# shaunlebron/blinky

Measured on AMD Instinct MI355X. Metric: warped Mpixels/s (lensmap apply), higher is better.
Workload: dtype u8; 1 GPU; 3840x2160 cube/panini f_fov 180, 64 frames/step from a resident ring of 64 distinct globes (1.80 GB, advanced every step), one lensmap; value / ms_per_step = the job with steps alternating between 2 HIP stream(s), value_one_stream = the same on one stream, roofline.kernel_ms_per_launch = the kernel alone under HIP events; 64 frames/step since r5 (r1-r4 ran 16: compare those with value_at_16_frames; ring_globes=64, parallelism=row-stripes x1, streams=2

## Files before the change

### blinky_amd/csrc/bk_api.cpp

```cpp
#include "bk_internal.h"

#include <algorithm>
#include <cstdlib>
#include <cstring>
#include <ctime>
#include <vector>

#include <dlfcn.h>

static thread_local std::string g_create_error;

static bool g_hwq_late = false;
__attribute__((constructor)) static void bk_more_hardware_queues()
{
    const char *keep = getenv("BLINKY_HIP_KEEP_HW_QUEUES");
    if (keep && *keep && *keep != '0') return;
    if (getenv("GPU_MAX_HW_QUEUES")) return;
    if (void *h = dlopen("libamdhip64.so", RTLD_NOW | RTLD_NOLOAD)) { g_hwq_late = true; (void)dlclose(h); }
    (void)setenv("GPU_MAX_HW_QUEUES", "16", 0);
}
void bk::hw_queue_note()
{
    static bool said = false;
    if (said) return;
// ... 238 lines not shown
    if (int r = alloc_maps(ctx)) return fail_empty(r);
    if (int r = alloc_globe(ctx)) return fail_empty(r);
    return BK_OK;
}

extern "C" int bk_set_rows(bk_ctx *ctx, int row0, int row1)
{
    if (!ctx) return BK_E_INVALID;
    if (row0 < 0 || row1 > ctx->H || row0 > row1)
        return ctx->fail(BK_E_INVALID, "bk_set_rows: [%d,%d) outside 0..%d", row0, row1, ctx->H);
    if (ctx->device < 0) {
        ctx->row0 = row0; ctx->row1 = row1;
        return BK_OK;
    }
    if (int r = ensure_device(ctx)) return r;
    if (row0 == ctx->row0 && row1 == ctx->row1) return BK_OK;
    ctx->row0 = row0; ctx->row1 = row1;
    ctx->lensmap_valid = false;
    ctx->spans_valid = false;
    bk::footprint_invalidate(ctx);
    return alloc_maps(ctx);
}

extern "C" int bk_set_frames(bk_ctx *ctx, int nframes)
{
    if (!ctx || nframes < 1) return BK_E_INVALID;
    if (int r = ensure_device(ctx)) return r;
    ctx->nframes = nframes;
    if (!ctx->ps) return BK_OK;
    return alloc_globe(ctx);
}

extern "C" int bk_get_size(const bk_ctx *ctx, int *width, int *height, int *platesize, int *row0, int *row1)
{
    if (!ctx) return BK_E_INVALID;
    if (width) *width = ctx->W;
    if (height) *height = ctx->H;
    if (platesize) *platesize = ctx->ps;
    if (row0) *row0 = ctx->row0;
    if (row1) *row1 = ctx->row1;
    return BK_OK;
}

extern "C" int bk_set_rubixgrid(bk_ctx *ctx, int numcells, double cell_size, double pad_size)
{
    if (!ctx) return BK_E_INVALID;
    ctx->rubix.numcells = numcells; ctx->rubix.cell = cell_size; ctx->rubix.pad = pad_size;
    return BK_OK;
}

extern "C" int bk_set_zoom(bk_ctx *ctx, int zoom_type, int fov_degrees)
{
    if (!ctx || zoom_type < BK_ZOOM_NONE || zoom_type > BK_ZOOM_CONTAIN) return BK_E_INVALID;
    ctx->zoom_type = zoom_type;
    ctx->zoom_fov = (zoom_type == BK_ZOOM_FOV || zoom_type == BK_ZOOM_VFOV) ? fov_degrees : 0;
    return BK_OK;
}

extern "C" int bk_set_apply_variant(bk_ctx *ctx, int variant)
{
    if (!ctx) return BK_E_INVALID;
    ctx->apply_variant = variant;
    return BK_OK;
}

extern "C" int bk_set_blockmap_tuning(bk_ctx *ctx, int measured)
{
    if (!ctx) return BK_E_INVALID;
    ctx->blockmap_tuning = measured != 0;
    bk::coopmap_invalidate(ctx);
    return BK_OK;
}

bk::DebugOptions bk::g_debug;
#if BK_DEBUG_API
extern "C" int bk_debug_set_option(const char *name, int value)
{
    if (!name) return BK_E_INVALID;
    if (!strcmp(name, "no_memcache")) bk::g_debug.no_memcache = value;
    else if (!strcmp(name, "libm_rel_log2")) bk::g_debug.libm_rel_log2 = value;
    else if (!strcmp(name, "print_model")) bk::g_debug.print_model = value;
    else if (!strcmp(name, "host_module")) bk::g_debug.host_module = value;
    else if (!strcmp(name, "no_direct_submit")) bk::g_debug.no_direct_submit = value;
    else if (!strcmp(name, "forward_careful")) bk::g_debug.forward_careful = value;
    else return BK_E_INVALID;
    return BK_OK;
}
#endif
#if BK_DEBUG_API
extern "C" int bk_debug_set_ablation(bk_ctx *ctx, int bits)
{
    if (!ctx) return BK_E_INVALID;
    ctx->apply_flags = bits;
    return BK_OK;
}
#endif

#if BK_DEBUG_API
extern "C" int bk_debug_set_tile_shape(bk_ctx *ctx, int lw)
{
    if (!ctx) return BK_E_INVALID;
    if (lw >= 600) { ctx->apply_block_cost = lw == 600 ? -1 : lw - 601; bk::coopmap_invalidate(ctx); return BK_OK; }
    if (lw >= 400) { ctx->apply_lds_kb = lw - 400; bk::coopmap_invalidate(ctx); return BK_OK; }
    if (lw >= 300) { ctx->apply_fchunk = lw - 300; return BK_OK; }
    if (lw >= 100) { ctx->apply_wgs_per_cu = lw - 100; return BK_OK; }
    if (lw != 0 && lw != 1 && lw != 2 && lw != 4) return BK_E_INVALID;
    ctx->tile_shape = lw;
    bk::coopmap_invalidate(ctx);
    return BK_OK;
}
#endif

#if BK_DEBUG_API
extern "C" int bk_debug_tile_stats(bk_ctx *ctx, int out[6])
{
    if (!ctx || !out) return BK_E_INVALID;
    if (!ctx->lensmap_valid) return ctx->fail(BK_E_STATE, "no lensmap");
    if (int r = ensure_device(ctx)) return r;
    return bk::coopmap_stats(ctx, out);
}
#endif

#if BK_DEBUG_API
extern "C" int bk_debug_traffic_model(bk_ctx *ctx, uint64_t out[8])
{
    if (!ctx || !out) return BK_E_INVALID;
    if (!ctx->lensmap_valid) return ctx->fail(BK_E_STATE, "no lensmap");
    if (int r = ensure_device(ctx)) return r;
    return bk::coopmap_traffic_model(ctx, out);
}
#endif

#if BK_DEBUG_API
extern "C" int bk_debug_band_balance(bk_ctx *ctx, uint32_t out[18])
{
    if (!ctx || !out) return BK_E_INVALID;
    if (!ctx->lensmap_valid) return ctx->fail(BK_E_STATE, "no lensmap");
    if (int r = ensure_device(ctx)) return r;
    return bk::coopmap_band_balance(ctx, out);
}
#endif

#if BK_DEBUG_API
extern "C" int bk_debug_xcd_of_workgroups(bk_ctx *ctx, int *out, int nworkgroups)
{
    if (!ctx || !out || nworkgroups < 1) return BK_E_INVALID;
    if (int r = ensure_device(ctx)) return r;
    return bk::coopmap_xcd_probe(ctx, out, nworkgroups);
}
#endif

extern "C" double bk_last_build_ms(const bk_ctx *ctx) { return ctx ? ctx->last_build_ms : 0; }


extern "C" int bk_set_lensmap(bk_ctx *ctx, const uint32_t *offsets, const uint8_t *tints)
{
    if (!ctx || !offsets) return BK_E_INVALID;
    if (!ctx->d_offsets) return ctx->fail(BK_E_STATE, "bk_set_lensmap: call bk_resize first");
    if (int r = ensure_device(ctx)) return r;
    const size_t px = (size_t)ctx->W * ctx->rows();
    BK_HIP(ctx, hipMemcpyAsync(ctx->d_offsets, offsets, px * 4, hipMemcpyHostToDevice, ctx->stream));
    if (int r = bk::launch_convert_offsets(ctx, ctx->d_offsets, px, 1)) return r;
    if (tints) BK_HIP(ctx, hipMemcpyAsync(ctx->d_tints, tints, px, hipMemcpyHostToDevice, ctx->stream));
    else BK_HIP(ctx, hipMemsetAsync(ctx->d_tints, 255, px, ctx->stream));
    BK_HIP(ctx, hipStreamSynchronize(ctx->stream));
    ctx->lensmap_valid = true;
// ... 618 lines not shown
```

### blinky_amd/csrc/bk_build.cpp

```cpp
#include <algorithm>
#include <chrono>
#include <cstring>
#include <memory>

#include "bk_build_params.h"
#include "bk_emit.h"
#include "bk_hostpool.h"
#include "bk_lens_priv.h"
#include "bkm.h"

using namespace bklua;
using bk::LensProgram;


static void fill_params(bk_ctx *ctx, BkBuildParams *bp)
{
    memset(bp, 0, sizeof *bp);
    bp->W = ctx->W; bp->H = ctx->H;
    bp->row0 = ctx->row0; bp->rows = ctx->rows();
    bp->ps = ctx->ps; bp->gp = ctx->gp; bp->ph = ctx->ph;
    bp->numplates = ctx->numplates;
    bp->has_globe_plate = ctx->prog->globe_plate.is_function();
    bp->scale = ctx->scale;
    bp->inv_scale_up = 1.0 / __builtin_fabs(ctx->scale) * (1.0 + 0x1p-50);
// ... 519 lines not shown
    bk::EmitRequest rq;
    rq.interp = &P->interp; rq.lens_inverse = P->lens_inverse; rq.lens_forward = P->lens_forward; rq.globe_plate = P->globe_plate;
    std::string which;
    bool carries = true;
    try { carries = bk::callbacks_carry_state(rq, &which); } catch (const LuaError &) { carries = true; which = "(callbacks not analysable)"; }
    const bool sequential = ctx->sequential_build >= 2 || (ctx->sequential_build == 1 && carries);
    ctx->last_build_path = sequential ? 2 : 1;
    ctx->last_build_why = why + (sequential ? (carries ? "; state carried in '" + which + "': one sequential scan on the host" : "; one sequential scan on the host (bk_set_sequential_build 2)")
                                            : "; callbacks carry no state: evaluated on the host's worker pool");
    if (P->info.map_type == BK_MAP_INVERSE) {
        if (!P->lens_inverse.is_function()) return ctx->fail(BK_E_STATE, "lens has no lens_inverse (map = \"lens_inverse\" without the function)");
        return sequential ? build_sequential(ctx, P, std::string(), bp, display_out) : build_inverse_pool(ctx, P, bp, display_out);
    }
    if (!P->lens_forward.is_function()) return ctx->fail(BK_E_STATE, "lens has no lens_forward");
    return build_forward_host(ctx, P, bp, sequential, display_out);
}

extern "C" int bk_last_build_path(const bk_ctx *ctx, char *why, size_t cap)
{
    if (!ctx) return BK_E_INVALID;
    if (why && cap) snprintf(why, cap, "%s", ctx->last_build_why.c_str());
    return ctx->last_build_path;
}

#if BK_DEBUG_API
extern "C" int bk_debug_host_build(bk_ctx *ctx, int mode, uint32_t *offsets, uint8_t *tints, int display_out[BK_MAX_PLATES], double *scale_out)
{
    if (!ctx || !offsets || !tints || mode < 0 || mode > 2) return BK_E_INVALID;
    LensProgram *P = ctx->prog;
    if (!P || !P->lens_valid) return ctx->fail(BK_E_STATE, "not a valid lens");
    if (!ctx->globe_valid) return ctx->fail(BK_E_STATE, "not a valid globe");
    if (ctx->W <= 0 || ctx->rows() <= 0) return ctx->fail(BK_E_STATE, "bk_debug_host_build: call bk_resize first");
    const size_t px = (size_t)ctx->W * ctx->rows();
    memset(offsets, 0xFF, px * 4);
    memset(tints, 255, px);
    for (int i = 0; i < BK_MAX_PLATES; ++i) { ctx->display[i] = 0; if (display_out) display_out[i] = 0; }
    ctx->last_bad_key = 0;
    if (int r = bk_calc_zoom(ctx, scale_out)) return r;
    if (P->info.map_type == BK_MAP_NONE) return ctx->fail(BK_E_STATE, "no inverse or forward map being used");
    BkBuildParams bp;
    fill_params(ctx, &bp);
    ctx->host_sink_off = offsets; ctx->host_sink_tint = tints;
    int rc;
    if (mode == 0) rc = build_on_host(ctx, P, "bk_debug_host_build", display_out);
    else if (P->info.map_type == BK_MAP_INVERSE) {
        if (!P->lens_inverse.is_function()) rc = ctx->fail(BK_E_STATE, "lens has no lens_inverse");
        else rc = mode == 2 ? build_sequential(ctx, P, std::string(), bp, display_out) : build_inverse_pool(ctx, P, bp, display_out);
    } else {
        if (!P->lens_forward.is_function()) rc = ctx->fail(BK_E_STATE, "lens has no lens_forward");
        else rc = build_forward_host(ctx, P, bp, mode == 2, display_out);
    }
    ctx->host_sink_off = nullptr; ctx->host_sink_tint = nullptr;
    for (size_t i = 0; i < px; ++i) {
        if (offsets[i] == BK_NULL_OFFSET) continue;
        unsigned plate, x, y;
        bk_texel_coords((unsigned)ctx->gp, (unsigned)ctx->ph, offsets[i], &plate, &x, &y);
        offsets[i] = plate * (unsigned)(ctx->ps * ctx->ps) + y * (unsigned)ctx->ps + x;
    }
    return rc;
}
#endif

extern "C" int bk_set_sequential_build(bk_ctx *ctx, int mode)
{
    if (!ctx || mode < 0 || mode > 2) return BK_E_INVALID;
    ctx->sequential_build = mode;
    return BK_OK;
}

extern "C" int bk_lens_carries_state(bk_ctx *ctx, char *global_name, size_t cap)
{
    if (!ctx) return BK_E_INVALID;
    LensProgram *P = ctx->prog;
    if (!P || !P->lens_valid) return ctx->fail(BK_E_STATE, "not a valid lens");
    bk::EmitRequest rq;
    rq.interp = &P->interp; rq.lens_inverse = P->lens_inverse; rq.lens_forward = P->lens_forward; rq.globe_plate = P->globe_plate;
    std::string which;
    bool carries = false;
    try { carries = bk::callbacks_carry_state(rq, &which); } catch (const LuaError &e) { return ctx->fail(BK_E_SCRIPT, "%s", e.what()); }
    if (global_name && cap) snprintf(global_name, cap, "%s", which.c_str());
    return carries ? 1 : 0;
}

struct HipFree { void operator()(void *p) const { (void)hipFree(p); } };
using DeviceMem = std::unique_ptr<void, HipFree>;

static int build_inverse_device(bk_ctx *ctx, LensProgram *P, const std::string &src, BkBuildParams &bp, int counters[kNumCounters])
{
    if (!P->k_inverse) return ctx->fail(BK_E_STATE, "lens has no lens_inverse (map = \"lens_inverse\" without the function)");
    for (int k = 0; k < 4; ++k) {
        (void)hipFree(ctx->fwd_scratch[k]);
        ctx->fwd_scratch[k] = nullptr; ctx->fwd_scratch_bytes[k] = 0;
    }
    void *args[] = {&bp};
    BK_HIP(ctx, hipEventRecord(ctx->build_time_ev[0], ctx->stream));
    const auto tk0 = std::chrono::steady_clock::now();
    std::vector<uint32_t> flagged;
    if (int r = flagged_pass(ctx, "bk_build_inverse launch", bp, false, [&] {
            return hipModuleLaunchKernel(P->k_inverse, (unsigned)((ctx->W + 255) / 256), (unsigned)ctx->rows(), 1, 256, 1, 1, 0, ctx->stream, args, nullptr);
        }, counters, &flagged, &ctx->last_kernel_retries)) return r;
    ctx->last_kernel_wall_ms = std::chrono::duration<double, std::milli>(std::chrono::steady_clock::now() - tk0).count();
    const size_t nfl = flagged.size() / 4;
    std::vector<uint32_t> roff(nfl);
    std::vector<uint8_t> rtint(nfl);
    std::vector<int> rshown(nfl), rerr(nfl, 0);
    rederive(ctx, P, src, flagged.data(), 4, nfl, true,
             [&](const HostModule &hm, const uint32_t *id, int stride, unsigned long cnt, size_t i) { hm.inverse(&bp, id, stride, cnt, &roff[i], &rtint[i], &rshown[i], &rerr[i]); },
             [&](HostEval &E, uint32_t id, size_t i) { h_inverse_entry(E, bp, id, &roff[i], &rtint[i], &rshown[i], &rerr[i]); });
    unsigned int bad_key = (unsigned)counters[BK_MAX_PLATES + 2];
    for (size_t i = 0; i < nfl; ++i) {
        counters[BK_MAX_PLATES] |= rerr[i];
        if (rerr[i] & BK_ERR_RESULT) {
            const uint32_t o = flagged[4 * i], lyl = o / (uint32_t)ctx->W, lx = o - lyl * (uint32_t)ctx->W;
            bad_key = std::max(bad_key, (uint32_t)(((uint32_t)ctx->row0 + lyl) * (uint32_t)ctx->W + ((uint32_t)ctx->W - 1u - lx)) + 1u);
        }
        if (rshown[i] >= 0) counters[rshown[i]] |= 1;
    }
    counters[BK_MAX_PLATES + 2] = (int)bad_key;
    if (int r = patch_changed(ctx, flagged, {roff.data()}, rtint.data(), ctx->d_offsets, ctx->d_tints)) return r;
    BK_HIP(ctx, hipEventRecord(ctx->build_time_ev[1], ctx->stream));
    return BK_OK;
}

static int build_forward_device(bk_ctx *ctx, LensProgram *P, const std::string &src, BkBuildParams &bp, int counters[kNumCounters])
{
    if (!P->k_corners || !P->k_quads || !P->k_resolve) return ctx->fail(BK_E_STATE, "lens has no lens_forward");
    const size_t px = (size_t)ctx->W * ctx->rows();
    const size_t n1 = (size_t)ctx->ps + 1;
    const size_t ncorner = (size_t)ctx->numplates * n1 * n1;
    const bool given = ctx->debug_corners_set();
    (void)given;
#if BK_DEBUG_API
    if (given && ctx->dbg_corner_ok.size() != ncorner)
        return ctx->fail(BK_E_INVALID, "bk_debug_set_forward_corners: the table has %zu corners, this build has %zu (plates * (platesize + 1)^2)", ctx->dbg_corner_ok.size(), ncorner);
#endif
    const size_t want[4] = {ncorner * 2 * sizeof(int), ncorner, px * 4, px * 4};
    for (int k = 0; k < 4; ++k)
        if (ctx->fwd_scratch_bytes[k] < want[k]) {
            (void)hipFree(ctx->fwd_scratch[k]);
            ctx->fwd_scratch[k] = nullptr; ctx->fwd_scratch_bytes[k] = 0;
            BK_HIP(ctx, hipMalloc(&ctx->fwd_scratch[k], want[k]));
            ctx->fwd_scratch_bytes[k] = want[k];
        }
    bp.corner_xy = (int *)ctx->fwd_scratch[0];
    bp.corner_ok = (unsigned char *)ctx->fwd_scratch[1];
    bp.fwd_key_px = (unsigned int *)ctx->fwd_scratch[2];
    bp.fwd_key_tint = (unsigned int *)ctx->fwd_scratch[3];
    constexpr size_t NQ = 21 * 21;
    const size_t ntile = ((size_t)ctx->ps + 15) / 16;
    if (ctx->fwd_tables_ps != ctx->ps) {
        (void)hipFree(ctx->fwd_tables);
        ctx->fwd_tables = nullptr; ctx->fwd_tables_ps = -1;
        std::vector<double> q(NQ, 0.0);
        for (int a = 0; a <= 20; ++a)
            for (int d = 1; d <= 20; ++d) q[(size_t)a * 21 + d] = (double)a / (double)d;
        std::vector<float> uv(2 * n1);
        for (size_t i = 0; i < n1; ++i) {
            uv[i] = (float)(((double)i - 0.5) / ctx->ps - 0.5);
            uv[n1 + i] = (float)((double)i / ctx->ps - 0.5);
        }
        BK_HIP(ctx, hipMalloc(&ctx->fwd_tables, NQ * sizeof(double) + uv.size() * sizeof(float) + (size_t)BK_MAX_PLATES * ntile * ntile));
        BK_HIP(ctx, hipMemcpy(ctx->fwd_tables, q.data(), NQ * sizeof(double), hipMemcpyHostToDevice));
        BK_HIP(ctx, hipMemcpy((char *)ctx->fwd_tables + NQ * sizeof(double), uv.data(), uv.size() * sizeof(float), hipMemcpyHostToDevice));
        ctx->fwd_tables_ps = ctx->ps;
    }
    bp.fwd_quot = (const double *)ctx->fwd_tables;
    bp.fwd_uv = (const float *)((const char *)ctx->fwd_tables + NQ * sizeof(double));
    unsigned char *const tile_own = (unsigned char *)ctx->fwd_tables + NQ * sizeof(double) + 2 * n1 * sizeof(float);
    const hipEvent_t e0 = ctx->build_time_ev[0], e1 = ctx->build_time_ev[1];
    void *args[] = {&bp};
    const auto clear_keys = [&](hipStream_t st) -> hipError_t {
        hipError_t e = hipMemsetAsync(ctx->fwd_scratch[2], 0, px * 4, st);
        return e == hipSuccess ? hipMemsetAsync(ctx->fwd_scratch[3], 0, px * 4, st) : e;
    };
    const auto launch_corners = [&]() -> hipError_t {
#if BK_DEBUG_API
        if (given) {
            hipError_t e = hipMemcpyAsync(bp.corner_xy, ctx->dbg_corner_xy.data(), ncorner * 2 * sizeof(int), hipMemcpyHostToDevice, ctx->stream);
            return e == hipSuccess ? hipMemcpyAsync(bp.corner_ok, ctx->dbg_corner_ok.data(), ncorner, hipMemcpyHostToDevice, ctx->stream) : e;
        }
#endif
// ... 473 lines not shown
```

### blinky_amd/csrc/bk_build_kernels.h

```cpp

BK_DEV void bk_state_init(BkState &S, const BkBuildParams *P)
{
    S.P = P;
    S.err = 0;
    S.steps = 0;
    S.flag = 0;
    BK_INIT_GLOBALS(S)
}

BK_DEV int bk_ray_to_plate_index(BkState &S, const float *ray)
{
    const BkBuildParams &P = *S.P;
#ifdef BK_HAS_GLOBE_PLATE
    bkv a[3] = {bk_num((double)ray[0]), bk_num((double)ray[1]), bk_num((double)ray[2])};
    bkv r[BK_MAXRET];
    int n = LF_globe_plate(S, a, 3, r);
    if (n < 1 || !bk_isnum(r[n - 1])) return -1;
    double d = r[n - 1].n;
    if (r[n - 1].e != 0.0 && !(bkm_rint(d - r[n - 1].e) == bkm_rint(d + r[n - 1].e))) S.flag = 1;
    if (!(d > -2147483648.0 && d < 2147483647.0)) return -1;
    int plate = (int)bkm_rint(d);
    if (plate < 0 || plate >= P.numplates) return -1;
    return plate;
#else
    int plate_index = 0;
    float max_dp = -2.0f;
#pragma unroll
    for (int i = 0; i < 6; ++i) {
        if (i < P.numplates) {
            const float dp = bk_dot3(ray, P.plates[i].forward);
            if (dp > max_dp) { max_dp = dp; plate_index = i; }
        }
    }
    return plate_index;
#endif
}

BK_DEV bool bk_offgrid(const BkBuildParams &P, int px, int py)
{
    if (P.grid_n)
        return !(((P.grid_bits[px >> 5] >> (px & 31)) | (P.grid_bits[py >> 5] >> (py & 31))) & 1u);
    double ux = (double)px / P.rubix_unit_px;
    double uy = (double)py / P.rubix_unit_px;
    bool ongrid = bkm_fmod(ux, P.rubix_block) < P.rubix_pad || bkm_fmod(uy, P.rubix_block) < P.rubix_pad;
    return !ongrid;
}

BK_DEV unsigned int bk_padded_offset(const BkBuildParams &P, int plate, int px, int py)
{
    return bk_texel_offset((unsigned int)P.gp, (unsigned int)P.ph, (unsigned int)plate, (unsigned int)px, (unsigned int)py);
}

#ifndef BK_HOST_MODULE
__device__ __forceinline__ void bk_push_flagged(const BkBuildParams &P, unsigned int id, unsigned int a, unsigned int b, unsigned int c)
{
    const unsigned int k = atomicAdd(P.flag_count, 1u);
    if (k < P.flag_cap) {
        P.flag_list[4 * k] = id; P.flag_list[4 * k + 1] = a; P.flag_list[4 * k + 2] = b; P.flag_list[4 * k + 3] = c;
    }
}

__device__ __forceinline__ void bk_push_flagged_wave(const BkBuildParams &P, bool flag, unsigned int id, unsigned int a, unsigned int b, unsigned int c)
{
    const unsigned long long m = __ballot(flag);
    if (!m) return;
    const int lane = (int)(threadIdx.x & 63u), leader = __ffsll((long long)m) - 1;
    unsigned int base = 0;
    if (lane == leader) base = atomicAdd(P.flag_count, (unsigned int)__popcll(m));
    base = (unsigned int)__shfl((int)base, leader);
    if (flag) {
        const unsigned int k = base + (unsigned int)__popcll(m & ((1ull << lane) - 1ull));
        if (k < P.flag_cap) {
            P.flag_list[4 * k] = id; P.flag_list[4 * k + 1] = a; P.flag_list[4 * k + 2] = b; P.flag_list[4 * k + 3] = c;
        }
    }
}

__device__ __forceinline__ void bk_publish_flags(const int *s_disp, int *display, int serr, int *err)
{
    if (threadIdx.x < 6 && s_disp[threadIdx.x]) {
        if (__hip_atomic_load(&display[threadIdx.x], __ATOMIC_RELAXED, __HIP_MEMORY_SCOPE_AGENT) == 0)
            atomicOr(&display[threadIdx.x], 1);
    }
    if (serr) atomicOr(err, serr);
}
#endif

#ifdef BK_HAS_INVERSE
BK_DEV void bk_inverse_entry(const BkBuildParams &P, BkState &S, int lx, int ly, unsigned int *off_out, unsigned char *tint_out, int *plate_out)
{
    unsigned int off = 0xFFFFFFFFu;
    unsigned char tint = 255;
    int shown = -1;
    const double y = (double)(-(ly - P.H / 2)) * P.scale;
    const double x = (double)(lx - P.W / 2) * P.scale;
    bkv a[2] = {bk_num(x), bk_num(y)};
    bkv r[BK_MAXRET];
    const int n = LF_lens_inverse(S, a, 2, r);
    if (n == 3 && bk_isnum(r[0]) && bk_isnum(r[1]) && bk_isnum(r[2])) {
        float ray[3] = {bk_narrow(S, r[0].n, r[0].e), bk_narrow(S, r[1].n, r[1].e), bk_narrow(S, r[2].n, r[2].e)};
        bk_vector_normalize(ray);
        const int plate = bk_ray_to_plate_index(S, ray);
        if (plate >= 0) {
            const BkPlateDev &p = P.plates[plate];
            const double px_ = (double)bk_dot3(p.right, ray);
            const double py_ = (double)bk_dot3(p.up, ray);
            const double pz_ = (double)bk_dot3(p.forward, ray);
            const double u = px_ / pz_ * p.dist64 + 0.5;
            const double v = -py_ / pz_ * p.dist64 + 0.5;
            if (u >= 0 && u <= 1 && v >= 0 && v <= 1) {
                const int px = bk_trunc_to_int(u * P.ps);
                const int py = bk_trunc_to_int(v * P.ps);
                if (px >= 0 && px < P.ps && py >= 0 && py < P.ps) {
                    shown = plate;
                    off = bk_padded_offset(P, plate, px, py);
                    if (bk_offgrid(P, px, py)) tint = (unsigned char)plate;
                }
            }
        }
    } else if (!(n == 1 && r[0].t == BK_TNIL)) {
        S.err |= BK_ERR_RESULT;
    }
    *off_out = off;
    *tint_out = tint;
    *plate_out = shown;
}

#ifndef BK_HOST_MODULE
extern "C" __global__ __launch_bounds__(256) void bk_build_inverse(BkBuildParams P)
{
    __shared__ int s_disp[6];
    if (threadIdx.x < 6) s_disp[threadIdx.x] = 0;
    __syncthreads();
    const int lx = blockIdx.x * blockDim.x + threadIdx.x;
    const int lyl = blockIdx.y;
    const int ly = P.row0 + lyl;
    int err = 0;
    bool flagged = false;
    unsigned int off = 0xFFFFFFFFu;
    unsigned char tint = 255;
    const size_t o = (size_t)lyl * P.W + lx;
    if (lx < P.W) {
        int plate;
        BkState S;
        bk_state_init(S, &P);
        bk_inverse_entry(P, S, lx, ly, &off, &tint, &plate);
        if (plate >= 0 && !S.flag) s_disp[plate] = 1;
        err = S.err;
        P.offsets[o] = off;
        P.tints[o] = tint;
        flagged = S.flag != 0;
        if ((err & BK_ERR_RESULT) && P.first_bad) atomicMax(P.first_bad, (unsigned int)(ly * P.W + (P.W - 1 - lx)) + 1u);
    }
    bk_push_flagged_wave(P, flagged, (unsigned int)o, off, tint, 0u);
    __syncthreads();
    bk_publish_flags(s_disp, P.display, err, P.err);
}
#endif
#endif

#ifdef BK_HAS_FORWARD
BK_DEV int bk_to_screen(const BkBuildParams &P, BkState &S, double v, double e, int half)
{
#ifndef BK_HOST_MODULE
    {
        const double fa = __builtin_fma(v, P.inv_scale_up, (double)half);
        const double ea = __builtin_fma(__builtin_fma(bk_abs(v), P.inv_scale_up, (double)half), 0x1p-47, e * P.inv_scale_up);
        const double lo = bkm_trunc(fa - ea);
        if (lo == bkm_trunc(fa + ea) && lo > -2147483649.0 && lo < 2147483648.0) return (int)lo;
    }
#endif
    const double f = v / P.scale + (double)half;
    bk_need_same_trunc(S, f, bk_eop(S, f, e * P.inv_scale_up));
    return bk_trunc_to_int(f);
}

BK_DEV void bk_corner_at(const BkBuildParams &P, BkState &S, int plate, int j, int i, int *sx_out, int *sy_out, unsigned char *ok_out)
{
    float ray[3];
#ifdef BK_HOST_MODULE
    const double u = ((double)i - 0.5) / P.ps;
    const double v = ((double)j - 0.5) / P.ps;
    bk_plate_uv_to_ray(P, plate, u, v, ray);
#else
    bk_plate_fuv_to_ray(P, plate, P.fwd_uv[i], -P.fwd_uv[j], ray);
#endif
    bkv a[3] = {bk_num((double)ray[0]), bk_num((double)ray[1]), bk_num((double)ray[2])};
    bkv r[BK_MAXRET];
    const int n = LF_lens_forward(S, a, 3, r);
    unsigned char ok = 0;
    int sx = 0, sy = 0;
    if (n == 2 && bk_isnum(r[0]) && bk_isnum(r[1])) {
        sx = bk_to_screen(P, S, r[0].n, r[0].e, P.W / 2);
        sy = bk_to_screen(P, S, -r[1].n, r[1].e, P.H / 2);
        ok = 1;
    } else if (!(n == 1 && r[0].t == BK_TNIL)) {
        S.err |= BK_ERR_RESULT;
    }
    *sx_out = sx;
    *sy_out = sy;
    *ok_out = ok;
}
BK_DEV void bk_corner_entry(const BkBuildParams &P, BkState &S, long long id, int *sx_out, int *sy_out, unsigned char *ok_out)
{
    const int n1 = P.ps + 1;
    const int plate = (int)(id / ((long long)n1 * n1));
    const int rem = (int)(id - (long long)plate * n1 * n1);
    const int j = rem / n1, i = rem - j * n1;
    bk_corner_at(P, S, plate, j, i, sx_out, sy_out, ok_out);
}

BK_DEV bool bk_texel_owns_at(const BkBuildParams &P, BkState &S, int plate, int py, int px)
{
    float ray[3];
#ifdef BK_HOST_MODULE
    bk_plate_uv_to_ray(P, plate, (double)px / P.ps, (double)py / P.ps, ray);
#else
    bk_plate_fuv_to_ray(P, plate, P.fwd_uv[P.ps + 1 + px], -P.fwd_uv[P.ps + 1 + py], ray);
#endif
    return plate == bk_ray_to_plate_index(S, ray);
}
BK_DEV bool bk_texel_owns(const BkBuildParams &P, BkState &S, long long id)
{
    const int plate = (int)(id / ((long long)P.ps * P.ps));
    const int rem = (int)(id - (long long)plate * P.ps * P.ps);
    const int py = rem / P.ps, px = rem - py * P.ps;
    return bk_texel_owns_at(P, S, plate, py, px);
}

#endif

#ifndef BK_HOST_MODULE
#ifdef BK_HAS_FORWARD
extern "C" __global__ __launch_bounds__(256) void bk_forward_corners(BkBuildParams P)
{
    const int n1 = P.ps + 1;
    const int i = (int)(blockIdx.x * blockDim.x + threadIdx.x), j = (int)blockIdx.y, plate = (int)blockIdx.z;
    const bool live = i < n1;
    const unsigned int id = ((unsigned int)plate * (unsigned int)n1 + (unsigned int)j) * (unsigned int)n1 + (unsigned int)i;
    BkState S;
// ... 324 lines not shown
```

### blinky_amd/csrc/bk_device_rt.h

```cpp
typedef struct { double n; double e; int t; } bkv;
#define BK_TNIL 0
#define BK_TFALSE 1
#define BK_TTRUE 2
#define BK_TNUM 3
#define BK_TSTR 4
#define BK_MAXRET 8
#define BK_LOOP_BUDGET (1 << 22)
#define BK_DEV static __device__ __forceinline__
#ifndef BK_LIBM_REL
#define BK_LIBM_REL 0x1p-50
#endif
#define BK_ROUND_REL 0x1p-51
#define BK_TINY 0x1p-960

struct BkState {
    const BkBuildParams *P;
    int err;
    int steps;
    int flag;
    BK_MUTABLE_GLOBALS
};

BK_DEV bkv bk_num(double d) { bkv v; v.n = d; v.e = 0.0; v.t = BK_TNUM; return v; }
BK_DEV bkv bk_nume(double d, double e) { bkv v; v.n = d; v.e = e; v.t = BK_TNUM; return v; }
// ... 201 lines not shown
BK_DEV double bk_e_log(BkState &S, double x, double e)
{
    if (e == 0.0) return 0.0;
    if (!(x - 2.0 * e > 0.0)) { S.flag = 1; return 0.0; }
    return e / (x - e);
}
BK_DEV bkv bk_f_log(BkState &S, bkv a) { const double x = bk_tonum(S, a), z = bkm_log(x); return bk_nume(z, bk_elibm(S, z, bk_e_log(S, x, a.e))); }
BK_DEV bkv bk_f_log10(BkState &S, bkv a) { const double x = bk_tonum(S, a), z = bkm_log10(x); return bk_nume(z, bk_elibm(S, z, bk_e_log(S, x, a.e))); }
BK_DEV bkv bk_f_sqrt(BkState &S, bkv a)
{
    const double x = bk_tonum(S, a), z = bkm_sqrt(x);
    if (a.e == 0.0) return bk_num(z);
    if (!(x - 2.0 * a.e > 0.0)) { S.flag = 1; return bk_num(z); }
    return bk_nume(z, bk_eop_inexact(S, z, a.e / (2.0 * bkm_sqrt(x - a.e))));
}
BK_DEV bkv bk_f_abs(BkState &S, bkv a) { return bk_nume(bkm_fabs(bk_tonum(S, a)), a.e); }
BK_DEV bkv bk_f_floor(BkState &S, bkv a) { const double x = bk_tonum(S, a); bk_need_same_floor(S, x, a.e); return bk_num(bkm_floor(x)); }
BK_DEV bkv bk_f_ceil(BkState &S, bkv a) { const double x = bk_tonum(S, a); bk_need_same_floor(S, -x, a.e); return bk_num(bkm_ceil(x)); }
BK_DEV double bk_e_atan2(BkState &S, double y, double ey, double x, double ex)
{
    if (ex == 0.0 && ey == 0.0) return 0.0;
    const double d = x * x + y * y, w = bk_eprod(S, bk_abs(x), ey) + bk_eprod(S, bk_abs(y), ex), s = ex + ey;
    if (!(d > 16.0 * s * s) || (x < 0.0 && !(bk_abs(y) > ey)) || !(d >= 0x1p-1022 && d < BKM_INF)) { S.flag = 1; return 0.0; }
    return 2.0 * w / d;
}
BK_DEV bkv bk_f_atan2(BkState &S, bkv a, bkv b)
{
    const double y = bk_tonum(S, a), x = bk_tonum(S, b), z = bkm_atan2(y, x);
    if (a.e == 0.0 && b.e == 0.0 && (x == 0.0 || y == 0.0)) return bk_num(z);
    return bk_nume(z, bk_elibm(S, z, bk_e_atan2(S, y, a.e, x, b.e)));
}
BK_DEV bkv bk_f_fmod(BkState &S, bkv a, bkv b)
{
    const double x = bk_tonum(S, a), y = bk_tonum(S, b), z = bkm_fmod(x, y);
    if (a.e == 0.0 && b.e == 0.0) return bk_num(z);
    const double q = x / y;
    bk_need_same_trunc(S, q, bk_ediv(S, x, a.e, y, b.e, q));
    return bk_nume(z, bk_eop_inexact(S, z, a.e + bk_abs(bkm_trunc(q)) * b.e));
}
BK_DEV bkv bk_f_scale(BkState &S, bkv a, double c, bool divide)
{
    const double x = bk_tonum(S, a), z = divide ? x / c : x * c;
    return bk_nume(z, bk_eop(S, z, divide ? a.e / c : a.e * c));
}
BK_DEV bkv bk_f_logb(BkState &S, bkv a, bkv b)
{
    if (b.t == BK_TNIL) return bk_f_log(S, a);
    bk_need_exact(S, b);
    if (bk_tonum(S, b) == 10.0) return bk_f_log10(S, a);
    return bk_div(S, bk_f_log(S, a), bk_f_log(S, b));
}
BK_DEV bkv bk_f_pick(BkState &S, bkv m, bkv d, bool want_max)
{
    const double dn = bk_tonum(S, d);
    const bool take = want_max ? dn > m.n : dn < m.n;
    return bk_nume(take ? dn : m.n, m.e > d.e ? m.e : d.e);
}
BK_DEV void bk_f_modf(BkState &S, bkv a, bkv *r)
{
    const double x = bk_tonum(S, a), ip = bkm_trunc(x);
    bk_need_same_trunc(S, x, a.e);
    r[0] = bk_num(ip);
    r[1] = bk_nume(bkm_copysign(bkm_isinf(x) ? 0.0 : x - ip, x), a.e);
}

BK_DEV float bk_dot3(const float *a, const float *b) { return a[0] * b[0] + a[1] * b[1] + a[2] * b[2]; }
BK_DEV void bk_vector_ma(const float *a, float scale, const float *b, float *c)
{
    c[0] = a[0] + scale * b[0];
    c[1] = a[1] + scale * b[1];
    c[2] = a[2] + scale * b[2];
}
BK_DEV void bk_vector_normalize(float *v)
{
    float length = v[0] * v[0] + v[1] * v[1] + v[2] * v[2];
    length = (float)__builtin_sqrt((double)length);
    if (length) {
        float ilength = 1 / length;
        v[0] *= ilength;
        v[1] *= ilength;
        v[2] *= ilength;
    }
}
BK_DEV void bk_latlon_to_ray(BkState &S, double lat, double elat, double lon, double elon, float *ray)
{
    double slat, clat, slon, clon;
    bkm_sincos(lat, &slat, &clat);
    bkm_sincos(lon, &slon, &clon);
    const double ec = bk_elibm(S, clat, elat), es = bk_elibm(S, slon, elon), ek = bk_elibm(S, clon, elon);
    const double p0 = slon * clat, p2 = clon * clat;
    ray[0] = bk_narrow(S, p0, bk_eop(S, p0, bk_abs(slon) * ec + bk_abs(clat) * es + ec * es));
    ray[1] = bk_narrow(S, slat, bk_elibm(S, slat, elat));
    ray[2] = bk_narrow(S, p2, bk_eop(S, p2, bk_abs(clon) * ec + bk_abs(clat) * ek + ec * ek));
}
BK_DEV void bk_plate_fuv_to_ray(const BkBuildParams &P, int plate, float fu, float fv, float *ray)
{
    const BkPlateDev &p = P.plates[plate];
    ray[0] = ray[1] = ray[2] = 0;
    bk_vector_ma(ray, p.dist, p.forward, ray);
    bk_vector_ma(ray, fu, p.right, ray);
    bk_vector_ma(ray, fv, p.up, ray);
    bk_vector_normalize(ray);
}
BK_DEV void bk_plate_uv_to_ray(const BkBuildParams &P, int plate, double u, double v, float *ray)
{
    u -= 0.5;
    v -= 0.5;
    v = -v;
    bk_plate_fuv_to_ray(P, plate, (float)u, (float)v, ray);
}
BK_DEV int bk_trunc_to_int(double v)
{
    if (!(v > -2147483649.0 && v < 2147483648.0)) return (int)0x80000000;
    return (int)v;
}

BK_DEV int bk_host_latlon_to_ray(BkState &S, bkv lat, bkv lon, bkv *r)
{
    float ray[3];
    bk_latlon_to_ray(S, bk_tonum(S, lat), lat.e, bk_tonum(S, lon), lon.e, ray);
    r[0] = bk_num((double)ray[0]); r[1] = bk_num((double)ray[1]); r[2] = bk_num((double)ray[2]);
    return 3;
}
BK_DEV int bk_host_ray_to_latlon(BkState &S, bkv x, bkv y, bkv z, bkv *r)
{
    const float ray[3] = {bk_narrow(S, bk_tonum(S, x), x.e), bk_narrow(S, bk_tonum(S, y), y.e), bk_narrow(S, bk_tonum(S, z), z.e)};
    const double lon = bkm_atan2((double)ray[0], (double)ray[2]);
    const double lat = bkm_atan2((double)ray[1], bkm_sqrt((double)(ray[0] * ray[0] + ray[2] * ray[2])));
    r[0] = bk_nume(lat, bk_elibm(S, lat, 0.0)); r[1] = bk_nume(lon, bk_elibm(S, lon, 0.0));
    return 2;
}
BK_DEV int bk_host_plate_to_ray(BkState &S, bkv plate, bkv u, bkv v, bkv *r)
{
    bk_need_same_trunc(S, bk_tonum(S, plate), plate.e);
    int pi = bk_trunc_to_int(bk_tonum(S, plate));
    float ray[3];
    if (pi < 0 || pi >= S.P->numplates) { r[0] = bk_nil(); return 1; }
    (void)bk_narrow(S, bk_tonum(S, u) - 0.5, u.e);
    (void)bk_narrow(S, -(bk_tonum(S, v) - 0.5), v.e);
    bk_plate_uv_to_ray(*S.P, pi, u.n, v.n, ray);
    r[0] = bk_num((double)ray[0]); r[1] = bk_num((double)ray[1]); r[2] = bk_num((double)ray[2]);
    return 3;
}
```

### blinky_amd/csrc/bk_emit.cpp

```cpp
#include "bk_emit.h"

#include <cmath>
#include <cstdio>
#include <map>
#include <set>
#include <sstream>

namespace bk {
using namespace bklua;

namespace {

[[noreturn]] void unsupported(const std::string &chunk, int line, const std::string &what)
{
    throw LuaError(chunk + ":" + std::to_string(line) + ": not supported in a GPU callback: " + what);
}

std::string sanitize(const std::string &s)
{
    std::string o;
    for (char c : s) o += (isalnum((unsigned char)c) ? c : '_');
    return o;
}

std::string num_literal(double d)
{
    if (d != d) return "bk_num(__builtin_nan(\"\"))";
    if (std::isinf(d)) return d > 0 ? "bk_num(__builtin_inf())" : "bk_num(-__builtin_inf())";
    char buf[64];
    snprintf(buf, sizeof buf, "bk_num(%a)", d);
    return buf;
}

struct FnInfo {
    const FuncProto *proto = nullptr;
    const Closure *cl = nullptr;
    std::string cname;
    bool emitting = false, done = false;
};

struct Emitter {
    Interp &I;
    std::map<std::pair<const FuncProto *, std::string>, FnInfo> fns;
    std::vector<std::string> fn_code;
    std::set<std::string> mutable_globals;
    std::map<const Table *, std::pair<std::string, int>> const_tables;
    std::ostringstream table_code;
    int uid = 0;
    struct SinCos { std::string s, c; long epoch; };
    std::map<std::string, SinCos> sincos;
    long epoch = 0;
    struct Pure { std::string name; long epoch; };
    std::map<std::string, Pure> pure;
    std::string last_single, last_single_of;
    static bool is_name(const std::string &v)
    {
        if (v.empty() || (v[0] >= '0' && v[0] <= '9')) return false;
        for (char c : v) if (!(c == '_' || c == '.' || (c >= '0' && c <= '9') || (c >= 'a' && c <= 'z') || (c >= 'A' && c <= 'Z'))) return false;
        return true;
    }
    static bool mentions(const std::string &key, const std::string &var)
    {
        auto word = [](char c) { return c == '_' || c == '.' || (c >= '0' && c <= '9') || (c >= 'a' && c <= 'z') || (c >= 'A' && c <= 'Z'); };
        for (size_t at = key.find(var); at != std::string::npos; at = key.find(var, at + 1)) {
            const bool left = at == 0 || !word(key[at - 1]), right = at + var.size() >= key.size() || !word(key[at + var.size()]);
            if (left && right) return true;
        }
        return false;
    }
    void forget(const std::string &var)
    {
        sincos.erase(var);
        for (auto it = pure.begin(); it != pure.end();) it = mentions(it->first, var) ? pure.erase(it) : std::next(it);
    }
    std::map<std::string, int> strings{{"nil", 1}, {"boolean", 2}, {"number", 3}, {"string", 4}};
    std::string str_literal(const std::string &v)
    {
        auto it = strings.find(v);
        if (it == strings.end()) it = strings.emplace(v, (int)strings.size() + 1).first;
        return "bk_str(" + std::to_string(it->second) + ")";
    }

    explicit Emitter(Interp &i) : I(i) {}

    struct Scope {
        const FuncProto *proto = nullptr;
        const Closure *cl = nullptr;
        const Scope *parent = nullptr;
    };
    struct Fn : Scope {
        std::ostringstream out;
        int indent = 1;
        std::map<int, int> array_slots;
        std::map<int, std::string> fn_slots;
        std::set<int> fn_open;
        std::map<int, Value> static_slots;
        std::map<int, std::vector<std::string>> record_slots;
        std::map<int, std::pair<int, int>> matrix_slots;
        std::string lp = "l", ap = "A", rp = "R";
        std::string field_var(int slot, const std::string &name) const { return rp + std::to_string(slot) + "_" + name; }
        bool is_table(int slot) const { return array_slots.count(slot) || record_slots.count(slot) || matrix_slots.count(slot); }
        std::string chunk;
    };
    static const Value *upvalue_of(const Scope *s, int idx, const Scope **owner, int *slot)
    {
        while (!s->cl) {
            const UpvalDesc &d = s->proto->upvals[(size_t)idx];
            if (d.from_parent_local) { *owner = s->parent; *slot = d.index; return nullptr; }
            idx = d.index;
            s = s->parent;
        }
        *owner = nullptr;
        return s->cl->upvals[(size_t)idx].get();
    }
    bool ad_active = false;
    Fn *ad_fn = nullptr;
    std::map<int, std::string> ad_slot;
    std::map<std::string, std::string> ad_d;
    std::string ad_call;
    std::string d_of(const std::string &v) const { auto it = ad_d.find(v); return it == ad_d.end() ? std::string("0.0") : it->second; }
    void ad_note(Fn &f, const std::string &value, const std::string &dexpr)
    {
        const std::string dn = tmp("dd");
        line(f, "const double " + dn + " = " + dexpr + ";");
        ad_d[value] = dn;
    }
    static Fn *local_of(Fn &f, const Expr &e, int *slot)
    {
        if (e.kind != Expr::Name) return nullptr;
        if (e.var == VarKind::Local) { *slot = e.slot; return &f; }
        if (e.var == VarKind::Upvalue) {
            const Scope *owner = nullptr;
            if (!upvalue_of(&f, e.slot, &owner, slot)) return const_cast<Fn *>(static_cast<const Fn *>(owner));
        }
        return nullptr;
    }
    std::vector<std::pair<const Value *, std::string>> mutable_cells;
    const std::string *cell_field(const Value *cell) const
    {
        for (auto &c : mutable_cells) if (c.first == cell) return &c.second;
        return nullptr;
    }
    std::string tmp(const char *p = "t") { return std::string(p) + std::to_string(++uid); }
    static void line(Fn &f, const std::string &s) { f.out << std::string((size_t)f.indent * 4, ' ') << s << "\n"; }
    std::string pure_value(Fn &f, const std::string &call)
    {
        auto hit = pure.find(call);
        if (hit != pure.end() && hit->second.epoch == epoch) return hit->second.name;
        const std::string t = tmp();
        line(f, "bkv " + t + " = " + call + ";");
        pure.insert_or_assign(call, Pure{t, epoch});
        return t;
    }

    static Value static_field(const Value &t, const Value &key)
    {
        Value cur = t;
        for (int depth = 0; depth < 32 && cur.t == Value::TABLE; ++depth) {
            Value v = cur.tab()->get(key);
            if (v.t != Value::NIL || !cur.tab()->meta) return v;
            cur = cur.tab()->meta->get(Value::string("__index"));
        }
        return Value();
    }

    bool static_value(Fn &f, const Expr &e, Value *v)
    {
        if (e.kind == Expr::Name) {
            int lslot = 0;
            if (Fn *o = local_of(f, e, &lslot)) {
                auto it = o->static_slots.find(lslot);
                if (it == o->static_slots.end()) return false;
                *v = it->second;
                return true;
            }
            if (e.var == VarKind::Global) {
                if (mutable_globals.count(e.str)) return false;
                *v = I.get_global(e.str);
                return true;
            }
            if (e.var == VarKind::Upvalue) {
                const Scope *owner = nullptr;
                int slot = 0;
                const Value *cell = upvalue_of(&f, e.slot, &owner, &slot);
                if (!cell || cell_field(cell)) return false;
                *v = *cell;
                return true;
            }
            return false;
        }
        if (e.kind == Expr::Index && e.b->kind == Expr::String) {
            Value o;
            if (static_value(f, *e.a, &o) && o.t == Value::TABLE) { *v = static_field(o, Value::string(e.b->str)); return true; }
        }
        return false;
    }

    static bool assigned_in(const Block &b, int slot)
    {
        for (const StmtP &sp : b) {
            const Stmt &s = *sp;
            for (auto &t : s.targets) if (t->kind == Expr::Name && t->var == VarKind::Local && t->slot == slot) return true;
            if (assigned_in(s.body, slot)) return true;
            for (auto &c : s.clauses) if (assigned_in(c.second, slot)) return true;
        }
        return false;
    }
    static bool slot_is_constant(const FuncProto *p, int slot) { return !p->is_captured(slot) && !assigned_in(p->body, slot); }

    void scan_closure(const Closure *cl, std::set<const FuncProto *> &seen)
    {
        Scope sc;
        sc.proto = cl->proto;
        sc.cl = cl;
        scan_block(cl->proto->body, sc, seen);
    }
    void scan_block(const Block &b, const Scope &sc, std::set<const FuncProto *> &seen)
    {
        for (const StmtP &s : b) scan_stmt(*s, sc, seen);
    }
    void scan_expr(const Expr *e, const Scope &sc, std::set<const FuncProto *> &seen)
    {
        if (!e) return;
        if (e->kind == Expr::Call && e->str.empty()) {
            Value callee;
            bool known = false;
            if (e->a->kind == Expr::Name && e->a->var == VarKind::Global) { callee = I.get_global(e->a->str); known = true; }
            else if (e->a->kind == Expr::Name && e->a->var == VarKind::Upvalue) {
                const Scope *owner = nullptr;
                int slot = 0;
                if (const Value *cell = upvalue_of(&sc, e->a->slot, &owner, &slot)) { callee = *cell; known = true; }
            }
            if (known && callee.t == Value::FUNC && !seen.count(callee.fn()->proto)) {
                seen.insert(callee.fn()->proto);
                scan_closure(callee.fn(), seen);
            }
        }
        if (e->kind == Expr::Call && !e->str.empty() && e->a->kind == Expr::Name) {
            Value obj;
            if (e->a->var == VarKind::Global) obj = I.get_global(e->a->str);
            else if (e->a->var == VarKind::Upvalue) {
                const Scope *owner = nullptr;
                int slot = 0;
                if (const Value *cell = upvalue_of(&sc, e->a->slot, &owner, &slot)) obj = *cell;
            }
            const Value m = static_field(obj, Value::string(e->str));
            if (m.t == Value::FUNC && !seen.count(m.fn()->proto)) {
                seen.insert(m.fn()->proto);
                scan_closure(m.fn(), seen);
            }
        }
        if (e->kind == Expr::Function && e->proto) {
            Scope inner;
            inner.proto = e->proto;
            inner.parent = &sc;
            scan_block(e->proto->body, inner, seen);
        }
        scan_expr(e->a.get(), sc, seen);
        scan_expr(e->b.get(), sc, seen);
        for (auto &x : e->args) scan_expr(x.get(), sc, seen);
        for (auto &x : e->fields) { scan_expr(x.first.get(), sc, seen); scan_expr(x.second.get(), sc, seen); }
    }
    void scan_stmt(const Stmt &s, const Scope &sc, std::set<const FuncProto *> &seen)
    {
        for (auto &t : s.targets) {
            if (t->kind == Expr::Name && t->var == VarKind::Global) mutable_globals.insert(t->str);
            if (t->kind == Expr::Name && t->var == VarKind::Upvalue) {
                const Scope *owner = nullptr;
                int slot = 0;
                const Value *cell = upvalue_of(&sc, t->slot, &owner, &slot);
                if (cell && !cell_field(cell)) mutable_cells.emplace_back(cell, "u" + std::to_string(mutable_cells.size() + 1) + "_" + sanitize(t->str));
            }
            scan_expr(t.get(), sc, seen);
        }
        for (auto &x : s.exprs) scan_expr(x.get(), sc, seen);
        scan_expr(s.call.get(), sc, seen);
        scan_expr(s.cond.get(), sc, seen);
        scan_block(s.body, sc, seen);
        for (auto &c : s.clauses) { scan_expr(c.first.get(), sc, seen); scan_block(c.second, sc, seen); }
    }

    std::pair<std::string, int> const_table(Fn &f, const Expr &at, const std::shared_ptr<Table> &t, const std::string &hint)
    {
        auto it = const_tables.find(t.get());
        if (it != const_tables.end()) return it->second;
        if (!t->nhash.empty() || !t->shash.empty())
            unsupported(f.chunk, at.line, "table '" + hint + "' with non-array keys");
        std::string name = "GT" + std::to_string(++uid) + "_" + sanitize(hint);
        int n = (int)t->arr.size();
        table_code << "static __device__ const bkv " << name << "[" << n + 1 << "] = {{0.0, 0.0, BK_TNIL}";
        for (const Value &v : t->arr) {
            char buf[80];
            switch (v.t) {
            case Value::NUM:
                if (v.n != v.n || std::isinf(v.n)) unsupported(f.chunk, at.line, "non-finite number in table '" + hint + "'");
                snprintf(buf, sizeof buf, ", {%a, 0.0, BK_TNUM}", v.n);
                break;
            case Value::BOOL: snprintf(buf, sizeof buf, ", {0.0, 0.0, %s}", v.b ? "BK_TTRUE" : "BK_TFALSE"); break;
            case Value::NIL: snprintf(buf, sizeof buf, ", {0.0, 0.0, BK_TNIL}"); break;
            case Value::STR: {
                const std::string lit = str_literal(v.str());
                snprintf(buf, sizeof buf, ", {%s.0, 0.0, BK_TSTR}", lit.substr(7, lit.size() - 8).c_str());
                break;
            }
            default: unsupported(f.chunk, at.line, std::string("table '") + hint + "' holding a " + v.type_name());
            }
            table_code << buf;
        }
        table_code << "};\n";
        return const_tables[t.get()] = {name, n};
    }

    std::string const_value(Fn &f, const Expr &e, const Value &v, const std::string &what)
    {
        switch (v.t) {
        case Value::NIL: return "bk_nil()";
        case Value::BOOL: return v.b ? "bk_bool(true)" : "bk_bool(false)";
        case Value::NUM: return num_literal(v.n);
        case Value::STR: return str_literal(v.str());
        default: unsupported(f.chunk, e.line, what + " (a " + v.type_name() + ") used as a value");
        }
    }

    std::string emit_expr(Fn &f, const Expr &e)
    {
        switch (e.kind) {
        case Expr::Nil: return "bk_nil()";
        case Expr::True: return "bk_bool(true)";
        case Expr::False: return "bk_bool(false)";
        case Expr::Number: return num_literal(e.num);
        case Expr::String: return str_literal(e.str);
        case Expr::Vararg: {
            const std::string np = std::to_string(f.proto->nparams);
            return "(na > " + np + " ? a[" + np + "] : bk_nil())";
        }
        case Expr::Function: unsupported(f.chunk, e.line, "function values / closures");
        case Expr::Table: unsupported(f.chunk, e.line, "table constructors other than 'local t = {a, b, ...}'");
        case Expr::Name: {
            int slot = 0;
            if (Fn *o = local_of(f, e, &slot)) {
                if (o->is_table(slot)) unsupported(f.chunk, e.line, "table '" + e.str + "' used as a value");
                if (o->fn_slots.count(slot)) unsupported(f.chunk, e.line, "function '" + e.str + "' used as a value (a function defined inside a callback can only be called)");
                if (o->static_slots.count(slot))
                    unsupported(f.chunk, e.line, std::string(o->static_slots[slot].t == Value::TABLE ? "table" : "function") + " '" + e.str +
                                                     "' used as a value (it can be " + (o->static_slots[slot].t == Value::TABLE ? "indexed" : "called") + ", and passed on to script functions)");
                return o->lp + std::to_string(slot);
            }
            if (e.var == VarKind::Global && mutable_globals.count(e.str)) return "S.g_" + sanitize(e.str);
            if (e.var == VarKind::Upvalue) {
                const Scope *owner = nullptr;
                if (const std::string *field = cell_field(upvalue_of(&f, e.slot, &owner, &slot))) return "S." + *field;
            }
            {
                Value v;
                static_value(f, e, &v);
                return const_value(f, e, v, "'" + e.str + "'");
            }
        }
        case Expr::Index: {
            int aslot = 0;
            Fn *ao = local_of(f, *e.a, &aslot);
            if (ao && ao->record_slots.count(aslot)) {
                if (e.b->kind != Expr::String) unsupported(f.chunk, e.line, "indexing record '" + e.a->str + "' with a computed key");
                const auto &names = ao->record_slots[aslot];
                for (const std::string &n : names) if (n == e.b->str) return ao->field_var(aslot, n);
                return "bk_nil()";
            }
            if (ao && ao->matrix_slots.count(aslot)) unsupported(f.chunk, e.line, "a row of table '" + e.a->str + "' used as a value");
            if (e.a->kind == Expr::Index) {
                int mslot = 0;
                Fn *mo = local_of(f, *e.a->a, &mslot);
                if (mo && mo->matrix_slots.count(mslot)) {
                    const std::string row = matrix_row(f, *mo, mslot, *e.a->b);
                    const std::string k = emit_expr(f, *e.b), t = tmp();
                    line(f, "bkv " + t + " = bk_aget(S, " + row + ", " + std::to_string(mo->matrix_slots[mslot].second) + ", " + k + ");");
                    return t;
                }
            }
            if (ao && ao->array_slots.count(aslot)) {
                std::string k = emit_expr(f, *e.b), t = tmp();
                line(f, "bkv " + t + " = bk_aget(S, " + ao->ap + std::to_string(aslot) + ", " + std::to_string(ao->array_slots[aslot]) + ", " + k + ");");
                return t;
            }
            Value sv;
            if (static_value(f, e, &sv)) return const_value(f, e, sv, "field '" + e.b->str + "'");
            Value o;
            if (static_value(f, *e.a, &o) && o.t == Value::TABLE) {
                auto ct = const_table(f, e, o.tab_ptr(), e.a->kind == Expr::Name ? e.a->str : "table");
                std::string k = emit_expr(f, *e.b), t = tmp();
                line(f, "bkv " + t + " = bk_aget(S, " + ct.first + ", " + std::to_string(ct.second) + ", " + k + ");");
                return t;
            }
            unsupported(f.chunk, e.line, "indexing this expression");
        }
        case Expr::Call: {
            std::string arr, cnt;
            emit_call(f, e, &arr, &cnt);
            if (!ad_active && last_single_of == arr && is_name(last_single)) return last_single;
            std::string t = tmp();
            line(f, "bkv " + t + " = " + cnt + " > 0 ? " + arr + "[0] : bk_nil();");
            if (ad_active && !ad_call.empty()) ad_note(f, t, ad_call);
            ad_call.clear();
            return t;
        }
        case Expr::Unop: {
            if (e.str == "()") return emit_expr(f, *e.a);
            if (e.str == "#") {
                int aslot = 0;
                Fn *ao = local_of(f, *e.a, &aslot);
                if (ao && ao->array_slots.count(aslot)) return num_literal((double)ao->array_slots[aslot]);
                if (ao && ao->matrix_slots.count(aslot)) return num_literal((double)ao->matrix_slots[aslot].first);
                if (ao && ao->record_slots.count(aslot)) return num_literal(0.0);
                if (e.a->kind == Expr::Index) {
                    int mslot = 0;
                    Fn *mo = local_of(f, *e.a->a, &mslot);
                    if (mo && mo->matrix_slots.count(mslot)) { (void)matrix_row(f, *mo, mslot, *e.a->b); return num_literal((double)mo->matrix_slots[mslot].second); }
                }
                Value sv;
                if (static_value(f, *e.a, &sv) && sv.t == Value::TABLE && sv.tab()->nhash.empty() && sv.tab()->shash.empty() && !sv.tab()->meta)
                    return num_literal((double)sv.tab()->length());
                if (static_value(f, *e.a, &sv) && sv.t == Value::STR) return num_literal((double)sv.str().size());
                if (e.a->kind == Expr::String) return num_literal((double)e.a->str.size());
                unsupported(f.chunk, e.line, "the length operator on this expression");
            }
            std::string a = emit_expr(f, *e.a), t = tmp();
            if (e.str == "not") line(f, "bkv " + t + " = bk_not(" + a + ");");
            else {
                line(f, "bkv " + t + " = bk_unm(S, " + a + ");");
                if (ad_active && d_of(a) != "0.0") ad_note(f, t, "-" + d_of(a));
            }
            return t;
        }
        case Expr::Binop: {
            const std::string &op = e.str;
            if (op == "and" || op == "or") {
                std::string a = emit_expr(f, *e.a), t = tmp();
                line(f, "bkv " + t + " = " + a + ";");
                line(f, std::string("if (") + (op == "and" ? "" : "!") + "bk_truthy(" + t + ")) {");
                f.indent++;
                ++epoch;
                std::string b = emit_expr(f, *e.b);
                line(f, t + " = " + b + ";");
                f.indent--;
                line(f, "}");
                ++epoch;
                return t;
            }
            if (op == "..") unsupported(f.chunk, e.line, "string concatenation");
            std::string a = emit_expr(f, *e.a);
            std::string b = emit_expr(f, *e.b);
            std::string t = tmp(), call;
            if (op == "+") call = "bk_add(S, " + a + ", " + b + ")";
            else if (op == "-") call = "bk_sub(S, " + a + ", " + b + ")";
            else if (op == "*") call = "bk_mul(S, " + a + ", " + b + ")";
            else if (op == "/") call = "bk_div(S, " + a + ", " + b + ")";
            else if (op == "%") call = "bk_mod(S, " + a + ", " + b + ")";
            else if (op == "^") call = "bk_pow(S, " + a + ", " + b + ")";
            else if (op == "==") call = "bk_eq(S, " + a + ", " + b + ")";
            else if (op == "~=") call = "bk_ne(S, " + a + ", " + b + ")";
            else if (op == "<") call = "bk_lt(S, " + a + ", " + b + ")";
            else if (op == "<=") call = "bk_le(S, " + a + ", " + b + ")";
            else if (op == ">") call = "bk_lt(S, " + b + ", " + a + ")";
            else if (op == ">=") call = "bk_le(S, " + b + ", " + a + ")";
            else unsupported(f.chunk, e.line, "operator '" + op + "'");
            if (!ad_active) return pure_value(f, call);
            line(f, "bkv " + t + " = " + call + ";");
            if (ad_active && (d_of(a) != "0.0" || d_of(b) != "0.0")) {
                const std::string da = d_of(a), db = d_of(b);
                const bool za = da == "0.0", zb = db == "0.0";
                if (op == "+") ad_note(f, t, za ? db : zb ? da : da + " + " + db);
                else if (op == "-") ad_note(f, t, za ? "-" + db : zb ? da : da + " - " + db);
                else if (op == "*") ad_note(f, t, za ? a + ".n * " + db : zb ? b + ".n * " + da : a + ".n * " + db + " + " + b + ".n * " + da);
                else if (op == "/") ad_note(f, t, zb ? da + " / " + b + ".n" : za ? "-" + t + ".n * " + db + " / " + b + ".n" : "(" + da + " - " + t + ".n * " + db + ") / " + b + ".n");
            }
            return t;
        }
        }
        return "bk_nil()";
    }

    struct Args {
        std::vector<std::string> fixed;
        bool multi = false;
        std::string marr, mcnt;
    };
    Args emit_args(Fn &f, const std::vector<ExprP> &list)
    {
        std::vector<const Expr *> ptrs;
        for (const ExprP &x : list) ptrs.push_back(x.get());
        return emit_args(f, ptrs);
    }
    Args emit_args(Fn &f, const std::vector<const Expr *> &list)
    {
        Args a;
        for (size_t i = 0; i < list.size(); ++i) {
            const Expr &x = *list[i];
            if (i + 1 == list.size() && x.kind == Expr::Call && !(ad_active && single_valued_call(f, x))) {
                a.multi = true;
                emit_call(f, x, &a.marr, &a.mcnt);
                if (!ad_active && last_single_of == a.marr && is_name(last_single)) {
                    a.multi = false;
                    a.fixed.push_back(last_single);
                    a.marr.clear(); a.mcnt.clear();
                }
            } else if (i + 1 == list.size() && x.kind == Expr::Vararg) {
                const std::string np = std::to_string(f.proto->nparams), vc = tmp("va");
                line(f, "int " + vc + " = na > " + np + " ? na - " + np + " : 0;");
                line(f, "if (" + vc + " > BK_MAXRET) { S.err |= BK_ERR_INDEX; " + vc + " = BK_MAXRET; }");
                a.multi = true;
                a.marr = "(a + " + np + ")";
                a.mcnt = vc;
            } else a.fixed.push_back(emit_expr(f, x));
        }
        return a;
    }
    static std::string arg_at(const Args &a, size_t i)
    {
        if (i < a.fixed.size()) return a.fixed[i];
        if (a.multi) {
            size_t k = i - a.fixed.size();
            return "(" + a.mcnt + " > " + std::to_string(k) + " ? " + a.marr + "[" + std::to_string(k) + "] : bk_nil())";
        }
        return "bk_nil()";
    }
    std::pair<std::string, std::string> pack(Fn &f, const Args &a, int min_size)
    {
        std::string arr = tmp("v"), cnt = tmp("n");
        int cap = (int)a.fixed.size() + (a.multi ? 8 : 0);
        if (cap < min_size) cap = min_size;
        if (cap < 1) cap = 1;
        line(f, "bkv " + arr + "[" + std::to_string(cap) + "];");
        for (size_t i = 0; i < a.fixed.size(); ++i) line(f, arr + "[" + std::to_string(i) + "] = " + a.fixed[i] + ";");
        if (a.multi) {
            line(f, "int " + cnt + " = " + std::to_string(a.fixed.size()) + " + " + a.mcnt + ";");
            line(f, "for (int q = 0; q < " + a.mcnt + "; ++q) " + arr + "[" + std::to_string(a.fixed.size()) + " + q] = " + a.marr + "[q];");
        } else {
            line(f, "const int " + cnt + " = " + std::to_string(a.fixed.size()) + ";");
        }
        return {arr, cnt};
    }

    bool single_valued_call(Fn &f, const Expr &e)
    {
        Value callee;
        if (e.kind != Expr::Call || !e.str.empty() || !static_value(f, *e.a, &callee) || callee.t != Value::BUILTIN) return false;
        const std::string &bn = callee.bi()->name;
        return bn.compare(0, 5, "math.") == 0 && bn != "math.modf" && bn != "math.frexp";
    }
// ... 2 lines not shown
    {
        ad_call.clear();
        Value callee, self_obj;
        const bool method = !e.str.empty();
        if (method) {
            if (!static_value(f, *e.a, &self_obj) || self_obj.t != Value::TABLE)
                unsupported(f.chunk, e.line, "method calls (a:" + e.str + "(..)) on a value that is not a constant table of the script");
            callee = static_field(self_obj, Value::string(e.str));
            if (callee.t != Value::FUNC) unsupported(f.chunk, e.line, "method '" + e.str + "' is not a script function");
        } else {
            int slot = 0;
            Fn *o = local_of(f, *e.a, &slot);
            if (o && o->fn_slots.count(slot)) {
                if (o->fn_open.count(slot)) unsupported(f.chunk, e.line, "recursion ('" + e.a->str + "')");
                *arr = tmp("r");
                *cnt = tmp("n");
                Args a = emit_args(f, e.args);
                auto packed = pack(f, a, 1);
                line(f, "bkv " + *arr + "[BK_MAXRET];");
                line(f, "const int " + *cnt + " = " + o->fn_slots[slot] + "(" + packed.first + ", " + packed.second + ", " + *arr + ");");
                ++epoch;
                return;
            }
        }
        if (!method && !static_value(f, *e.a, &callee)) {
            std::string n = e.a->kind == Expr::Name ? "'" + e.a->str + "'" : "this expression";
            unsupported(f.chunk, e.line, "calling " + n + " (callee must be a script function or builtin known at build time)");
        }
        *arr = tmp("r");
        *cnt = tmp("n");
        if (callee.t == Value::FUNC) {
            std::vector<std::pair<int, Value>> bound;
            std::vector<const Expr *> plain;
            static const Expr nil_expr = [] { Expr x; x.kind = Expr::Nil; return x; }();
            const int shift = method ? 1 : 0;
            if (method) {
                if (callee.fn()->proto->nparams < 1) unsupported(f.chunk, e.line, "method '" + e.str + "' takes no self");
                bound.emplace_back(0, self_obj);
                plain.push_back(&nil_expr);
            }
            for (size_t i = 0; i < e.args.size(); ++i) {
                Value av;
                const Expr &x = *e.args[i];
                if ((int)i + shift < callee.fn()->proto->nparams && (x.kind == Expr::Name || x.kind == Expr::Index) && static_value(f, x, &av) &&
                    (av.is_function() || av.t == Value::TABLE)) {
                    bound.emplace_back((int)i + shift, av);
                    plain.push_back(&nil_expr);
                } else plain.push_back(&x);
            }
            const FnInfo &fi = ensure_function(callee.fn(), e.line, f.chunk, bound);
            Args a = emit_args(f, plain);
            auto packed = pack(f, a, 1);
            line(f, "bkv " + *arr + "[BK_MAXRET];");
            line(f, "const int " + *cnt + " = " + fi.cname + "(S, " + packed.first + ", " + packed.second + ", " + *arr + ");");
            ++epoch;
            return;
        }
        if (callee.t != Value::BUILTIN) {
            std::string n = e.a->kind == Expr::Name ? e.a->str : "?";
            unsupported(f.chunk, e.line, "attempt to call '" + n + "' (a " + callee.type_name() + " value)");
        }
        const std::string &bn = callee.bi()->name;
        if (bn == "print") {
            line(f, "bkv " + *arr + "[1]; const int " + *cnt + " = 0; (void)" + *arr + ";");
            return;
        }
        Args a = emit_args(f, e.args);
        auto A = [&](size_t i) { return arg_at(a, i); };
        auto single = [&](const std::string &expr) {
            line(f, "bkv " + *arr + "[1] = {" + expr + "}; const int " + *cnt + " = 1;");
            last_single = expr;
            last_single_of = *arr;
        };
        static const std::map<std::string, std::string> unary = {
            {"math.sin", "bk_f_sin"}, {"math.cos", "bk_f_cos"}, {"math.tan", "bk_f_tan"}, {"math.asin", "bk_f_asin"},
            {"math.acos", "bk_f_acos"}, {"math.atan", "bk_f_atan"}, {"math.sinh", "bk_f_sinh"}, {"math.cosh", "bk_f_cosh"},
            {"math.tanh", "bk_f_tanh"}, {"math.exp", "bk_f_exp"}, {"math.log10", "bk_f_log10"}, {"math.sqrt", "bk_f_sqrt"},
            {"math.abs", "bk_f_abs"}, {"math.floor", "bk_f_floor"}, {"math.ceil", "bk_f_ceil"}};
        if (bn == "math.sin" || bn == "math.cos") {
            const std::string operand = A(0);
            auto hit = sincos.find(operand);
            if (hit == sincos.end() || hit->second.epoch != epoch) {
                SinCos sc{tmp("sn"), tmp("cs"), epoch};
                line(f, "bkv " + sc.s + ", " + sc.c + "; bk_f_sincos(S, " + operand + ", &" + sc.s + ", &" + sc.c + ");");
                hit = sincos.insert_or_assign(operand, sc).first;
            }
            single(bn == "math.sin" ? hit->second.s : hit->second.c);
            if (ad_active && d_of(operand) != "0.0")
                ad_call = bn == "math.sin" ? hit->second.c + ".n * " + d_of(operand) : "-" + hit->second.s + ".n * " + d_of(operand);
            return;
        }
        auto u = unary.find(bn);
        if (u != unary.end()) {
            if (!ad_active) { single(pure_value(f, u->second + "(S, " + A(0) + ")")); return; }
            single(u->second + "(S, " + A(0) + ")");
            if (ad_active && d_of(A(0)) != "0.0") {
                const std::string x = A(0) + ".n", r = *arr + "[0].n", d = d_of(A(0));
                if (bn == "math.tan") ad_call = "(1.0 + " + r + " * " + r + ") * " + d;
                else if (bn == "math.asin") ad_call = d + " / bkm_sqrt((1.0 - " + x + ") * (1.0 + " + x + "))";
                else if (bn == "math.acos") ad_call = "-" + d + " / bkm_sqrt((1.0 - " + x + ") * (1.0 + " + x + "))";
                else if (bn == "math.atan") ad_call = d + " / (1.0 + " + x + " * " + x + ")";
                else if (bn == "math.sqrt") ad_call = d + " / (2.0 * " + r + ")";
                else if (bn == "math.exp") ad_call = r + " * " + d;
                else if (bn == "math.tanh") ad_call = "(1.0 - " + r + " * " + r + ") * " + d;
                else if (bn == "math.sinh") ad_call = "bkm_cosh(" + x + ") * " + d;
                else if (bn == "math.cosh") ad_call = "bkm_sinh(" + x + ") * " + d;
            }
            return;
        }
        if (bn == "math.atan2") {
            if (!ad_active) { single(pure_value(f, "bk_f_atan2(S, " + A(0) + ", " + A(1) + ")")); return; }
            single("bk_f_atan2(S, " + A(0) + ", " + A(1) + ")");
            if (ad_active && (d_of(A(0)) != "0.0" || d_of(A(1)) != "0.0")) {
                const std::string y = A(0) + ".n", x = A(1) + ".n";
                ad_call = "(" + x + " * " + d_of(A(0)) + " - " + y + " * " + d_of(A(1)) + ") / (" + x + " * " + x + " + " + y + " * " + y + ")";
            }
            return;
        }
        if (bn == "math.pow") { single("bk_powv(S, " + A(0) + ", " + A(1) + ")"); return; }
        if (bn == "math.fmod") { single("bk_f_fmod(S, " + A(0) + ", " + A(1) + ")"); return; }
        if (bn == "math.deg") { single("bk_f_scale(S, " + A(0) + ", 0x1.921fb54442d18p+1 / 180.0, true)"); return; }
        if (bn == "math.rad") { single("bk_f_scale(S, " + A(0) + ", 0x1.921fb54442d18p+1 / 180.0, false)"); return; }
        if (bn == "math.log") {
            if (a.fixed.size() < 2 && !a.multi) { single("bk_f_log(S, " + A(0) + ")"); return; }
            single("bk_f_logb(S, " + A(0) + ", " + A(1) + ")");
            return;
        }
        if (bn == "math.max" || bn == "math.min") {
            if (a.fixed.empty() && !a.multi) unsupported(f.chunk, e.line, bn + " without arguments");
            const std::string want = bn == "math.max" ? "true" : "false";
            std::string m = tmp("m");
            line(f, "bkv " + m + " = " + A(0) + "; (void)bk_tonum(S, " + m + ");");
            for (size_t i = 1; i < a.fixed.size(); ++i) line(f, m + " = bk_f_pick(S, " + m + ", " + A(i) + ", " + want + ");");
            if (a.multi)
                line(f, "for (int q = " + std::string(a.fixed.empty() ? "1" : "0") + "; q < " + a.mcnt + "; ++q) " + m + " = bk_f_pick(S, " + m + ", " +
                            a.marr + "[q], " + want + ");");
            single(m);
            return;
        }
        if (bn == "math.modf") {
            line(f, "bkv " + *arr + "[2]; bk_f_modf(S, " + A(0) + ", " + *arr + "); const int " + *cnt + " = 2;");
            return;
        }
        if (bn == "select") {
            if (e.args.empty()) unsupported(f.chunk, e.line, "select without arguments");
            std::vector<const Expr *> rest;
            for (size_t i = 1; i < e.args.size(); ++i) rest.push_back(e.args[i].get());
            Args ra = emit_args(f, rest);
            auto packed = pack(f, ra, 1);
            if (e.args[0]->kind == Expr::String && e.args[0]->str == "#") {
                line(f, "bkv " + *arr + "[1] = {bk_num((double)" + packed.second + ")}; const int " + *cnt + " = 1; (void)" + packed.first + ";");
                return;
            }
            const std::string n = emit_expr(f, *e.args[0]), tn = tmp(), k = tmp("k");
            line(f, "const bkv " + tn + " = " + n + "; bk_need_exact(S, " + tn + ");");
            line(f, "int " + k + " = (" + tn + ".t == BK_TNUM && " + tn + ".n > -65.0 && " + tn + ".n < 65.0) ? (int)" + tn + ".n : 0;");
            line(f, "if (" + k + " < 0) " + k + " = " + packed.second + " + " + k + " + 1;");
            line(f, "if (" + k + " < 1) { S.err |= BK_ERR_INDEX; " + k + " = " + packed.second + " + 1; }");
            line(f, "if (" + k + " > " + packed.second + ") " + k + " = " + packed.second + " + 1;");
            line(f, "bkv *" + *arr + " = " + packed.first + " + (" + k + " - 1); const int " + *cnt + " = " + packed.second + " - (" + k + " - 1);");
            return;
        }
        if (bn == "type") { single("bk_typeof(" + A(0) + ")"); return; }
        if (bn == "latlon_to_ray") {
            line(f, "bkv " + *arr + "[3]; const int " + *cnt + " = bk_host_latlon_to_ray(S, " + A(0) + ", " + A(1) + ", " + *arr + ");");
            return;
        }
        if (bn == "ray_to_latlon") {
            line(f, "bkv " + *arr + "[2]; const int " + *cnt + " = bk_host_ray_to_latlon(S, " + A(0) + ", " + A(1) + ", " + A(2) + ", " + *arr + ");");
            return;
        }
        if (bn == "plate_to_ray") {
            line(f, "bkv " + *arr + "[3]; const int " + *cnt + " = bk_host_plate_to_ray(S, " + A(0) + ", " + A(1) + ", " + A(2) + ", " + *arr + ");");
            return;
        }
        unsupported(f.chunk, e.line, "builtin '" + bn + "'");
    }

    bool ad_expr_ok(Fn &f, const Expr &e, std::vector<int> *reads)
    {
        switch (e.kind) {
        case Expr::Number: return true;
        case Expr::Name: {
            int slot = 0;
            if (Fn *o = local_of(f, e, &slot)) {
                if (o != &f || o->is_table(slot) || o->fn_slots.count(slot) || o->static_slots.count(slot) || f.proto->is_captured(slot)) return false;
                reads->push_back(slot);
                return true;
            }
            if (e.var == VarKind::Global && mutable_globals.count(e.str)) return false;
            if (e.var == VarKind::Upvalue) {
                const Scope *owner = nullptr;
                if (cell_field(upvalue_of(&f, e.slot, &owner, &slot))) return false;
            }
            Value v;
            return static_value(f, e, &v) && v.t == Value::NUM;
        }
        case Expr::Unop: return (e.str == "-" || e.str == "()") && ad_expr_ok(f, *e.a, reads);
        case Expr::Binop: return (e.str == "+" || e.str == "-" || e.str == "*" || e.str == "/") && ad_expr_ok(f, *e.a, reads) && ad_expr_ok(f, *e.b, reads);
        case Expr::Call: {
            Value callee;
            if (!e.str.empty() || !static_value(f, *e.a, &callee) || callee.t != Value::BUILTIN) return false;
            static const std::set<std::string> one = {"math.sin", "math.cos", "math.tan", "math.asin", "math.acos", "math.atan", "math.sqrt",
                                                      "math.exp", "math.sinh", "math.cosh", "math.tanh"};
            const std::string &bn = callee.bi()->name;
            const size_t want = one.count(bn) ? 1 : bn == "math.atan2" ? 2 : 0;
            if (!want || e.args.size() != want) return false;
            for (const ExprP &x : e.args)
                if (x->kind == Expr::Vararg || !ad_expr_ok(f, *x, reads)) return false;
            return true;
        }
        default: return false;
        }
    }
    bool contraction_pattern(Fn &f, const Stmt &loop, int *carried, std::vector<int> *assigned)
    {
        std::set<int> all;
        for (const StmtP &sp : loop.body) {
            const Stmt &s = *sp;
            if (s.kind == Stmt::Local) {
                if (s.exprs.size() != s.slots.size()) return false;
                for (int slot : s.slots) all.insert(slot);
            } else if (s.kind == Stmt::Assign) {
                if (s.exprs.size() != s.targets.size()) return false;
                for (const ExprP &t : s.targets) {
                    int slot = 0;
                    if (t->kind != Expr::Name || local_of(f, *t, &slot) != &f || f.is_table(slot) || f.fn_slots.count(slot) || f.static_slots.count(slot) ||
                        f.proto->is_captured(slot)) return false;
                    all.insert(slot);
                }
            } else return false;
        }
        if (all.count(loop.slots[0])) return false;
        std::set<int> done, live;
        for (const StmtP &sp : loop.body) {
            const Stmt &s = *sp;
            std::vector<int> reads;
            for (const ExprP &x : s.exprs)
                if (!ad_expr_ok(f, *x, &reads)) return false;
            for (int r : reads) if (all.count(r) && !done.count(r)) live.insert(r);
            if (s.kind == Stmt::Local) for (int slot : s.slots) done.insert(slot);
            else for (const ExprP &t : s.targets) { int slot = 0; (void)local_of(f, *t, &slot); done.insert(slot); }
        }
        if (live.size() != 1) return false;
        *carried = *live.begin();
        assigned->assign(all.begin(), all.end());
        return true;
    }

    void emit_block(Fn &f, const Block &b)
    {
        ++epoch;
        for (const StmtP &s : b) emit_stmt(f, *s);
        ++epoch;
    }

    std::vector<std::string> emit_values(Fn &f, const std::vector<ExprP> &exprs, size_t want)
    {
        Args a = emit_args(f, exprs);
        std::vector<std::string> v;
        for (size_t i = 0; i < want; ++i) {
            std::string t = tmp();
            line(f, "const bkv " + t + " = " + arg_at(a, i) + ";");
            if (ad_active && d_of(arg_at(a, i)) != "0.0") ad_note(f, t, d_of(arg_at(a, i)));
            v.push_back(t);
        }
        return v;
    }

    std::string matrix_row(Fn &f, Fn &owner, int slot, const Expr &index)
    {
        const int rows = owner.matrix_slots[slot].first, cols = owner.matrix_slots[slot].second;
        const std::string i = emit_expr(f, index), ti = tmp(), r = tmp("row");
        line(f, "const bkv " + ti + " = " + i + "; bk_need_exact(S, " + ti + ");");
        line(f, "const int " + r + " = (" + ti + ".t == BK_TNUM && " + ti + ".n >= 1.0 && " + ti + ".n <= " + std::to_string(rows) + ".0 && " + ti + ".n == bkm_trunc(" + ti + ".n)) ? (int)" + ti + ".n : 0;");
        line(f, "if (!" + r + ") S.err |= BK_ERR_INDEX;");
        return "(" + owner.ap + std::to_string(slot) + " + (" + r + " ? " + r + " - 1 : 0) * " + std::to_string(cols) + ")";
    }

    void store(Fn &f, const Expr &target, const std::string &val)
    {
        int slot = 0;
        if (target.kind == Expr::Name) {
            if (Fn *o = local_of(f, target, &slot)) {
                if (o->is_table(slot)) unsupported(f.chunk, target.line, "re-assigning table '" + target.str + "'");
                if (o->fn_slots.count(slot)) unsupported(f.chunk, target.line, "re-assigning function '" + target.str + "'");
                line(f, o->lp + std::to_string(slot) + " = " + val + ";");
                forget(o->lp + std::to_string(slot));
                if (ad_active && o == ad_fn && ad_slot.count(slot)) line(f, ad_slot[slot] + " = " + d_of(val) + ";");
            } else if (target.var == VarKind::Global) {
                line(f, "S.g_" + sanitize(target.str) + " = " + val + ";");
                forget("S.g_" + sanitize(target.str));
            } else {
                const Scope *owner = nullptr;
                const std::string *field = cell_field(upvalue_of(&f, target.slot, &owner, &slot));
                if (!field) unsupported(f.chunk, target.line, "assigning to the enclosing function's local '" + target.str + "'");
                line(f, "S." + *field + " = " + val + ";");
                forget("S." + *field);
            }
            return;
        }
        Fn *ao = local_of(f, *target.a, &slot);
        if (ao && ao->record_slots.count(slot)) {
            if (target.b->kind != Expr::String) unsupported(f.chunk, target.line, "indexing record '" + target.a->str + "' with a computed key");
            for (const std::string &n : ao->record_slots[slot]) if (n == target.b->str) { line(f, ao->field_var(slot, n) + " = " + val + ";"); forget(ao->field_var(slot, n)); return; }
            unsupported(f.chunk, target.line, "adding field '" + target.b->str + "' to '" + target.a->str + "' (name it in the constructor)");
        }
        if (target.a->kind == Expr::Index) {
            int mslot = 0;
            Fn *mo = local_of(f, *target.a->a, &mslot);
            if (mo && mo->matrix_slots.count(mslot)) {
                const std::string row = matrix_row(f, *mo, mslot, *target.a->b);
                const std::string k = emit_expr(f, *target.b);
                line(f, "bk_aset(S, " + row + ", " + std::to_string(mo->matrix_slots[mslot].second) + ", " + k + ", " + val + ");");
                return;
            }
        }
        if (ao && ao->array_slots.count(slot)) {
            std::string k = emit_expr(f, *target.b);
            line(f, "bk_aset(S, " + ao->ap + std::to_string(slot) + ", " + std::to_string(ao->array_slots[slot]) + ", " + k + ", " + val + ");");
            return;
        }
        unsupported(f.chunk, target.line, "storing into this table (only tables created by 'local t = {..}' in the same function are writable)");
    }

    static void declare_locals(std::ostream &o, const Fn &f, const std::string &pad)
    {
        const FuncProto *p = f.proto;
        for (int i = 0; i < p->nslots; ++i) {
            if (f.fn_slots.count(i)) continue;
            if (f.record_slots.count(i)) {
                for (const std::string &name : f.record_slots.at(i)) o << pad << "bkv " << f.field_var(i, name) << " = bk_nil();   /* " << p->slot_names[i] << "." << name << " */\n";
            } else if (f.matrix_slots.count(i)) {
                const int cells = f.matrix_slots.at(i).first * f.matrix_slots.at(i).second;
                o << pad << "bkv " << f.ap << i << "[" << cells + 1 << "];   /* " << p->slot_names[i] << " */\n";
                o << pad << "for (int q = 0; q <= " << cells << "; ++q) " << f.ap << i << "[q] = bk_nil();\n";
            } else if (f.array_slots.count(i)) {
                o << pad << "bkv " << f.ap << i << "[" << f.array_slots.at(i) + 1 << "];   /* " << p->slot_names[i] << " */\n";
            } else if (i < p->nparams) {
                o << pad << "bkv " << f.lp << i << " = na > " << i << " ? a[" << i << "] : bk_nil();   /* " << p->slot_names[i] << " */\n";
            } else {
                o << pad << "bkv " << f.lp << i << " = bk_nil();   /* " << p->slot_names[i] << " */\n";
            }
        }
    }

    void emit_local_function(Fn &f, const Stmt &s)
    {
        const FuncProto *p = s.exprs[0]->proto;
        const int slot = s.slots[0];
        if (f.fn_slots.count(slot) || f.is_table(slot)) unsupported(f.chunk, s.line, "re-declaring '" + s.names[0] + "'");
        const std::string id = std::to_string(++uid);
        Fn g;
        g.proto = p;
        g.parent = &f;
        g.chunk = f.chunk;
        g.lp = "n" + id + "_l";
        g.ap = "n" + id + "_A";
        g.rp = "n" + id + "_R";
        g.indent = f.indent + 1;
        const std::string name = "NF" + id + "_" + sanitize(s.names[0]);
        f.fn_slots[slot] = name;
        f.fn_open.insert(slot);
        emit_block(g, p->body);
        f.fn_open.erase(slot);
        line(f, "/* " + f.chunk + ":" + std::to_string(p->line) + "  function " + s.names[0] + " */");
        line(f, "auto " + name + " = [&](const bkv *a, int na, bkv *r) -> int {");
        std::ostringstream decl;
        declare_locals(decl, g, std::string((size_t)(f.indent + 1) * 4, ' '));
        f.out << decl.str();
        line(f, "    (void)a; (void)na; (void)r;");
        f.out << g.out.str();
        line(f, "    return 0;");
        line(f, "};");
    }

    void emit_stmt(Fn &f, const Stmt &s)
    {
        const bool plain = s.kind == Stmt::Local || s.kind == Stmt::Assign;
        if (!plain) ++epoch;
        emit_stmt_body(f, s);
        if (!plain) ++epoch;
    }
    void emit_stmt_body(Fn &f, const Stmt &s)
    {
        switch (s.kind) {
        case Stmt::Local: {
            if (s.slots.size() == 1 && s.exprs.size() == 1 && s.exprs[0]->kind == Expr::Function) { emit_local_function(f, s); return; }
            if (s.slots.size() == 1 && s.exprs.size() == 1 && (s.exprs[0]->kind == Expr::Name || s.exprs[0]->kind == Expr::Index)) {
                Value fv;
                if (static_value(f, *s.exprs[0], &fv) && (fv.is_function() || fv.t == Value::TABLE)) {
                    if (!slot_is_constant(f.proto, s.slots[0])) unsupported(f.chunk, s.line, std::string(fv.t == Value::TABLE ? "table" : "function") + " '" + s.names[0] + "' used as a value (the local is assigned or captured later)");
                    f.static_slots[s.slots[0]] = fv;
                    return;
                }
            }
            if (s.slots.size() == 1 && s.exprs.size() == 1 && s.exprs[0]->kind == Expr::Table && !s.exprs[0]->fields.empty() && s.exprs[0]->args.empty()) {
                const Expr &t = *s.exprs[0];
                const int slot = s.slots[0];
                if (f.fn_slots.count(slot) || f.is_table(slot)) unsupported(f.chunk, s.line, "re-declaring a table");
                std::vector<std::string> names, vals;
                for (auto &fld : t.fields) {
                    if (fld.first->kind != Expr::String || fld.first->str.empty() || !(isalpha((unsigned char)fld.first->str[0]) || fld.first->str[0] == '_'))
                        unsupported(f.chunk, s.line, "table constructors with computed keys");
                    for (const std::string &n : names) if (n == fld.first->str) unsupported(f.chunk, s.line, "field '" + n + "' named twice in a table constructor");
                    names.push_back(fld.first->str);
                    vals.push_back(emit_expr(f, *fld.second));
                }
                f.record_slots[slot] = names;
                for (size_t i = 0; i < names.size(); ++i) { line(f, f.field_var(slot, names[i]) + " = " + vals[i] + ";"); forget(f.field_var(slot, names[i])); }
                return;
            }
            if (s.slots.size() == 1 && s.exprs.size() == 1 && s.exprs[0]->kind == Expr::Table && s.exprs[0]->fields.empty() && !s.exprs[0]->args.empty() &&
                s.exprs[0]->args[0]->kind == Expr::Table) {
                const Expr &t = *s.exprs[0];
                const int slot = s.slots[0];
                if (f.fn_slots.count(slot) || f.is_table(slot)) unsupported(f.chunk, s.line, "re-declaring a table");
                const int rows = (int)t.args.size(), cols = (int)t.args[0]->args.size();
                std::vector<std::string> vals;
                for (auto &row : t.args) {
                    if (row->kind != Expr::Table || !row->fields.empty() || (int)row->args.size() != cols || cols == 0)
                        unsupported(f.chunk, s.line, "nested table constructors other than rows of one length ({{a, b}, {c, d}})");
                    if (row->args.back()->kind == Expr::Call && !single_valued_call(f, *row->args.back()))
                        unsupported(f.chunk, s.line, "call expansion inside a table constructor (write '(f(...))' to keep one value)");
                    if (row->args.back()->kind == Expr::Vararg)
                        unsupported(f.chunk, s.line, "'...' at the end of a table constructor (a table of a size only known at run time)");
                    for (auto &x : row->args) vals.push_back(emit_expr(f, *x));
                }
                f.matrix_slots[slot] = {rows, cols};
                for (size_t i = 0; i < vals.size(); ++i) line(f, f.ap + std::to_string(slot) + "[" + std::to_string(i + 1) + "] = " + vals[i] + ";");
                return;
            }
            if (s.slots.size() == 1 && s.exprs.size() == 1 && s.exprs[0]->kind == Expr::Table) {
                const Expr &t = *s.exprs[0];
                if (!t.fields.empty()) unsupported(f.chunk, s.line, "table constructors mixing positional and named fields");
                if (!t.args.empty() && t.args.back()->kind == Expr::Call && !single_valued_call(f, *t.args.back()))
                    unsupported(f.chunk, s.line, "call expansion inside a table constructor (write '(f(...))' to keep one value)");
                if (!t.args.empty() && t.args.back()->kind == Expr::Vararg)
                    unsupported(f.chunk, s.line, "'...' at the end of a table constructor (a table of a size only known at run time)");
                std::vector<std::string> vals;
                for (auto &x : t.args) vals.push_back(emit_expr(f, *x));
                int n = (int)vals.size();
                if (f.array_slots.count(s.slots[0]) && f.array_slots[s.slots[0]] != n) unsupported(f.chunk, s.line, "re-declaring a table with a different size");
                if (f.record_slots.count(s.slots[0]) || f.matrix_slots.count(s.slots[0])) unsupported(f.chunk, s.line, "re-declaring a table");
                f.array_slots[s.slots[0]] = n;
                for (int i = 0; i < n; ++i) line(f, f.ap + std::to_string(s.slots[0]) + "[" + std::to_string(i + 1) + "] = " + vals[i] + ";");
                return;
            }
            auto v = emit_values(f, s.exprs, s.slots.size());
            for (size_t i = 0; i < s.slots.size(); ++i) {
                line(f, f.lp + std::to_string(s.slots[i]) + " = " + v[i] + ";");
                forget(f.lp + std::to_string(s.slots[i]));
                if (ad_active && &f == ad_fn && ad_slot.count(s.slots[i])) line(f, ad_slot[s.slots[i]] + " = " + d_of(v[i]) + ";");
            }
            return;
        }
        case Stmt::LocalFunction: emit_local_function(f, s); return;
        case Stmt::Assign: {
            auto v = emit_values(f, s.exprs, s.targets.size());
            for (size_t i = 0; i < s.targets.size(); ++i) store(f, *s.targets[i], v[i]);
            return;
        }
        case Stmt::CallStmt: {
            std::string arr, cnt;
            line(f, "{");
            f.indent++;
            emit_call(f, *s.call, &arr, &cnt);
            line(f, "(void)" + cnt + ";");
            f.indent--;
            line(f, "}");
            return;
        }
        case Stmt::Do:
            line(f, "{");
            f.indent++;
            emit_block(f, s.body);
            f.indent--;
            line(f, "}");
            return;
        case Stmt::While: {
            line(f, "for (;;) {");
            f.indent++;
            line(f, "if (!bk_tick(S)) break;");
            std::string c = emit_expr(f, *s.cond);
            line(f, "if (!bk_truthy(" + c + ")) break;");
            emit_block(f, s.body);
            f.indent--;
            line(f, "}");
            return;
        }
        case Stmt::Repeat: {
            line(f, "for (;;) {");
            f.indent++;
            line(f, "if (!bk_tick(S)) break;");
            emit_block(f, s.body);
            std::string c = emit_expr(f, *s.cond);
            line(f, "if (bk_truthy(" + c + ")) break;");
            f.indent--;
            line(f, "}");
            return;
        }
        case Stmt::If: {
            int opened = 0;
            for (size_t i = 0; i < s.clauses.size(); ++i) {
                const auto &c = s.clauses[i];
                if (!c.first) {
                    emit_block(f, c.second);
                    break;
                }
                std::string cv = emit_expr(f, *c.first);
                line(f, "if (bk_truthy(" + cv + ")) {");
                f.indent++;
                emit_block(f, c.second);
                f.indent--;
                if (i + 1 < s.clauses.size()) {
                    line(f, "} else {");
                    f.indent++;
                    opened++;
                } else line(f, "}");
            }
            for (int k = 0; k < opened; ++k) { f.indent--; line(f, "}"); }
            return;
        }
        case Stmt::NumFor: {
            std::string start = emit_expr(f, *s.exprs[0]), stop = emit_expr(f, *s.exprs[1]);
            std::string step = s.exprs.size() > 2 ? emit_expr(f, *s.exprs[2]) : "bk_num(1.0)";
            std::string st = tmp("step"), lim = tmp("lim"), idx = tmp("idx");
            line(f, "bk_need_exact(S, " + start + "); bk_need_exact(S, " + stop + "); bk_need_exact(S, " + step + ");");
            line(f, "const double " + st + " = bk_tonum(S, " + step + "), " + lim + " = bk_tonum(S, " + stop + ");");
            line(f, "double " + idx + " = bk_tonum(S, " + start + ") - " + st + ";");
            line(f, "for (;;) {");
            f.indent++;
            line(f, idx + " = " + idx + " + " + st + ";");
            line(f, "if (!(0 < " + st + " ? " + idx + " <= " + lim + " : " + lim + " <= " + idx + ")) break;");
            line(f, "if (!bk_tick(S)) break;");
            line(f, f.lp + std::to_string(s.slots[0]) + " = bk_num(" + idx + ");");
            int carried = -1;
            std::vector<int> assigned;
            const bool contract = !ad_active && contraction_pattern(f, s, &carried, &assigned);
            std::string e0;
            if (contract) {
                const std::string k = std::to_string(++uid), cv = f.lp + std::to_string(carried);
                e0 = "ce" + k;
                line(f, "const double " + e0 + " = " + cv + ".e; " + cv + ".e = 0.0;     /* " + f.proto->slot_names[(size_t)carried] + " enters the step as exact (bk_contract below) */");
                for (int slot : assigned) {
                    const std::string dn = "cd" + k + "_" + std::to_string(slot);
                    line(f, "double " + dn + " = " + (slot == carried ? "1.0" : "0.0") + ";");
                    ad_slot[slot] = dn;
                    ad_d[f.lp + std::to_string(slot)] = dn;
                }
                ad_active = true;
                ad_fn = &f;
            }
            emit_block(f, s.body);
            if (contract) {
                ad_active = false;
                for (int slot : assigned)
                    line(f, f.lp + std::to_string(slot) + ".e = bk_contract(S, " + ad_slot[slot] + ", " + e0 + ", " + f.lp + std::to_string(slot) + ".e);");
                ad_slot.clear();
                ad_d.clear();
                ad_fn = nullptr;
            }
            f.indent--;
            line(f, "}");
            return;
        }
        case Stmt::GenFor: {
            const Expr *call = s.exprs.size() == 1 && s.exprs[0]->kind == Expr::Call ? s.exprs[0].get() : nullptr;
            Value callee;
            if (!call || !static_value(f, *call->a, &callee) || callee.t != Value::BUILTIN ||
                (callee.bi()->name != "ipairs" && callee.bi()->name != "pairs") || call->args.size() != 1)
                unsupported(f.chunk, s.line, "generic 'for ... in' other than ipairs(t) / pairs(t)");
            const bool is_ipairs = callee.bi()->name == "ipairs";
            const Expr &targ = *call->args[0];
            std::string arr;
            int n = 0;
            int tslot = 0;
            Fn *to = local_of(f, targ, &tslot);
            if (to && to->array_slots.count(tslot)) {
                arr = to->ap + std::to_string(tslot);
                n = to->array_slots[tslot];
            } else {
                Value tv;
                if (!static_value(f, targ, &tv) || tv.t != Value::TABLE) unsupported(f.chunk, s.line, "iterating a table that is not known when the kernel is generated");
                auto ct = const_table(f, targ, tv.tab_ptr(), targ.kind == Expr::Name ? targ.str : "table");
                arr = ct.first;
                n = ct.second;
            }
            std::string gi = tmp("gi"), gv = tmp("gv");
            line(f, "for (int " + gi + " = 1; " + gi + " <= " + std::to_string(n) + "; ++" + gi + ") {");
            f.indent++;
            line(f, "if (!bk_tick(S)) break;");
            line(f, "const bkv " + gv + " = " + arr + "[" + gi + "];");
            line(f, std::string("if (") + gv + ".t == BK_TNIL) " + (is_ipairs ? "break;" : "continue;"));
            for (size_t i = 0; i < s.slots.size(); ++i)
                line(f, f.lp + std::to_string(s.slots[i]) + " = " + (i == 0 ? "bk_num((double)" + gi + ")" : i == 1 ? gv : std::string("bk_nil()")) + ";");
            emit_block(f, s.body);
            f.indent--;
            line(f, "}");
            return;
        }
        case Stmt::Return: {
            if (s.exprs.size() == 1 && s.exprs[0]->kind == Expr::Call) {
                std::string arr, cnt;
                line(f, "{");
                f.indent++;
                emit_call(f, *s.exprs[0], &arr, &cnt);
                line(f, "for (int q = 0; q < " + cnt + "; ++q) r[q] = " + arr + "[q];");
                line(f, "return " + cnt + ";");
                f.indent--;
                line(f, "}");
                return;
            }
            line(f, "{");
            f.indent++;
            Args a = emit_args(f, s.exprs);
            if (a.fixed.size() > 8) unsupported(f.chunk, s.line, "more than 8 return values");
            if (a.multi && a.fixed.size() > 4) unsupported(f.chunk, s.line, "more than 4 return values in front of a trailing call or `...`");
            for (size_t i = 0; i < a.fixed.size(); ++i) line(f, "r[" + std::to_string(i) + "] = " + a.fixed[i] + ";");
            if (a.multi) {
                line(f, "for (int q = 0; q < " + a.mcnt + " && " + std::to_string(a.fixed.size()) + " + q < BK_MAXRET; ++q) r[" + std::to_string(a.fixed.size()) + " + q] = " + a.marr + "[q];");
                line(f, "return " + std::to_string(a.fixed.size()) + " + " + a.mcnt + ";");
            } else line(f, "return " + std::to_string(a.fixed.size()) + ";");
            f.indent--;
            line(f, "}");
            return;
        }
        case Stmt::Break: line(f, "break;"); return;
        case Stmt::Goto: case Stmt::Label: unsupported(f.chunk, s.line, "goto");
        }
    }

    const FnInfo &ensure_function(const Closure *cl, int line_no, const std::string &from_chunk, const std::vector<std::pair<int, Value>> &bound = {})
    {
        std::string signature;
        for (auto &b : bound) {
            char id[48];
            snprintf(id, sizeof id, "%d=%p;", b.first, b.second.p.get());
            signature += id;
        }
        FnInfo &fi = fns[{cl->proto, signature}];
        if (fi.done) {
            if (fi.cl != cl) unsupported(from_chunk, line_no, "two closures of the same function body");
            return fi;
        }
        if (fi.emitting) unsupported(from_chunk, line_no, "recursion ('" + cl->proto->name + "')");
        fi.proto = cl->proto;
        fi.cl = cl;
        fi.cname = "LF" + std::to_string(++uid) + "_" + sanitize(cl->proto->name);
        fi.emitting = true;

        Fn f;
        f.proto = cl->proto;
        f.cl = cl;
        f.chunk = cl->chunk->name;
        for (auto &b : bound) {
            if (!slot_is_constant(cl->proto, b.first))
                unsupported(from_chunk, line_no, std::string(b.second.t == Value::TABLE ? "a table" : "a function") + " passed as '" + cl->proto->slot_names[(size_t)b.first] + "' of '" + cl->proto->name + "', which assigns or captures that parameter");
            f.static_slots[b.first] = b.second;
        }
        emit_block(f, cl->proto->body);

        std::ostringstream o;
        o << "/* " << f.chunk << ":" << cl->proto->line << "  function " << cl->proto->name << " */\n";
        o << "BK_DEV int " << fi.cname << "(BkState &S, const bkv *a, int na, bkv *r)\n{\n";
        declare_locals(o, f, "    ");
        o << "    (void)a; (void)na; (void)r;\n";
        o << f.out.str();
        o << "    return 0;\n}\n\n";
        fn_code.push_back(o.str());
        fi.emitting = false;
        fi.done = true;
        return fi;
    }
};

}


namespace {

struct StateScan {
    Interp &I;
    const std::set<std::string> &mut;
    std::string culprit;
    std::set<const FuncProto *> active;
    static constexpr uint8_t IMPURE = 0x80;
    struct Val { uint8_t dep = 0; int copy_of = -1; };
    using State = std::map<std::string, Val>;
    struct Frame { std::vector<Val> loc; uint8_t ret = 0; };
    std::map<std::string, std::string> cache_key;
    std::string refresh_key;
    std::vector<std::pair<std::string, std::string>> stores;

    static Val join(Val a, Val b) { Val o; o.dep = (uint8_t)(a.dep | b.dep); o.copy_of = a.copy_of == b.copy_of ? a.copy_of : -1; return o; }
    static State meet(const State &a, const State &b)
    {
        State o;
        for (auto &kv : a) { auto it = b.find(kv.first); if (it != b.end()) o[kv.first] = join(kv.second, it->second); }
        return o;
    }
    Val local_of(Frame &fr, int slot) { if (slot < 0) return Val{IMPURE, -1}; if ((size_t)slot >= fr.loc.size()) fr.loc.resize((size_t)slot + 1); return fr.loc[(size_t)slot]; }
    void set_local(Frame &fr, int slot, Val v, bool fresh)
    {
        if (slot < 0) return;
        if ((size_t)slot >= fr.loc.size()) fr.loc.resize((size_t)slot + 1);
        fr.loc[(size_t)slot] = fresh ? v : join(fr.loc[(size_t)slot], v);
    }
    Val read_global(const std::string &name, const State &st)
    {
        if (!mut.count(name)) return Val{};
        auto it = st.find(name);
        if (it != st.end()) return it->second;
        if (culprit.empty()) culprit = name;
        return Val{IMPURE, -1};
    }
    Val call_script(const Closure *cl, const std::vector<Val> &args, const State &st)
    {
        if (active.count(cl->proto)) return Val{IMPURE, -1};
        active.insert(cl->proto);
        Frame fr;
        fr.loc.resize((size_t)std::max(cl->proto->nslots, cl->proto->nparams));
        for (int i = 0; i < cl->proto->nparams; ++i) fr.loc[(size_t)i] = (size_t)i < args.size() ? args[(size_t)i] : Val{};
        if (cl->proto->is_vararg) for (size_t i = (size_t)cl->proto->nparams; i < args.size(); ++i) fr.ret |= args[i].dep;
        Emitter::Scope callee_scope;
        callee_scope.proto = cl->proto;
        callee_scope.cl = cl;
        State inner = st;
        block(cl->proto->body, &callee_scope, inner, fr);
        active.erase(cl->proto);
        Val out;
        out.dep = fr.ret;
        return out;
    }
    Val expr(const Expr *e, const Emitter::Scope *sc, State &st, Frame &fr)
    {
        if (!e) return Val{};
        switch (e->kind) {
        case Expr::Nil: case Expr::True: case Expr::False: case Expr::Number: case Expr::String: return Val{};
        case Expr::Vararg: return Val{fr.ret, -1};
        case Expr::Name:
            if (e->var == VarKind::Global) return read_global(e->str, st);
            if (e->var == VarKind::Local) return local_of(fr, e->slot);
            return Val{};
        case Expr::Function:
            if (e->proto) {
                Emitter::Scope inner_scope;
                inner_scope.proto = e->proto;
                inner_scope.parent = sc;
                State inner = st;
                Frame ifr;
                ifr.loc.assign((size_t)e->proto->nslots, Val{IMPURE, -1});
                block(e->proto->body, &inner_scope, inner, ifr);
            }
            return Val{IMPURE, -1};
        default: break;
// ... 183 lines not shown
        if (which) *which = em.mutable_cells[0].second.substr(em.mutable_cells[0].second.find('_') + 1);
        return true;
    }
    if (em.mutable_globals.empty()) return false;
    StateScan sc{*req.interp, em.mutable_globals, std::string(), {}, {}, std::string(), {}};
    for (const Value *v : roots)
        if (v->t == Value::FUNC) {
            StateScan::State st;
            StateScan::Frame fr;
            const FuncProto *pr = v->fn()->proto;
            fr.loc.resize((size_t)std::max(pr->nslots, pr->nparams));
            for (int i = 0; i < pr->nparams && i < 3; ++i) fr.loc[(size_t)i] = StateScan::Val{(uint8_t)(1u << i), i};
            for (int i = 3; i < pr->nparams; ++i) fr.loc[(size_t)i] = StateScan::Val{};
            Emitter::Scope root;
            root.proto = pr;
            root.cl = v->fn();
            sc.active.insert(pr);
            sc.block(pr->body, &root, st, fr);
            sc.active.erase(pr);
        }
    sc.check_caches();
    if (which) *which = sc.culprit;
    return !sc.culprit.empty();
}

std::string emit_build_source(const EmitRequest &req)
{
    Emitter em(*req.interp);
    std::set<const FuncProto *> seen;
    const Value *roots[3] = {&req.lens_inverse, &req.lens_forward, &req.globe_plate};
    for (const Value *v : roots)
        if (v->t == Value::FUNC && !seen.count(v->fn()->proto)) {
            seen.insert(v->fn()->proto);
            em.scan_closure(v->fn(), seen);
        }
    for (const Value *v : roots)
        if (v->t != Value::NIL && v->t != Value::FUNC)
            throw LuaError(std::string("a lens / globe callback must be a Lua function, got a ") + v->type_name());

    std::string names[3];
    for (int i = 0; i < 3; ++i)
        if (roots[i]->t == Value::FUNC) names[i] = em.ensure_function(roots[i]->fn(), 0, "callback").cname;

    std::ostringstream src;
    src << "/* generated by libblinkyhip (bk_emit.cpp) */\n";
    src << "#define BK_MUTABLE_GLOBALS";
    for (const std::string &g : em.mutable_globals) src << " bkv g_" << sanitize(g) << ";";
    for (auto &c : em.mutable_cells) src << " bkv " << c.second << ";";
    src << "\n";
    src << "#include \"bkm.h\"\n#include \"bk_build_params.h\"\n#include \"bk_device_rt.h\"\n\n";
    src << em.table_code.str() << "\n";
    for (const std::string &c : em.fn_code) src << c;
    src << "#define BK_INIT_GLOBALS(S)";
    for (const std::string &g : em.mutable_globals) {
        Value v = req.interp->get_global(g);
        std::string init;
        switch (v.t) {
        case Value::NIL: init = "bk_nil()"; break;
        case Value::BOOL: init = v.b ? "bk_bool(true)" : "bk_bool(false)"; break;
        case Value::NUM: init = num_literal(v.n); break;
        case Value::STR: init = em.str_literal(v.str()); break;
        default:
            throw LuaError("global '" + g + "' is assigned inside a GPU callback but holds a " + v.type_name() +
                           " when the lensmap build starts; only nil / boolean / number / string globals can be per-pixel state");
        }
        src << " (S).g_" << sanitize(g) << " = " << init << ";";
    }
    for (auto &c : em.mutable_cells) {
        const Value &v = *c.first;
        std::string init;
        switch (v.t) {
        case Value::NIL: init = "bk_nil()"; break;
        case Value::BOOL: init = v.b ? "bk_bool(true)" : "bk_bool(false)"; break;
        case Value::NUM: init = num_literal(v.n); break;
        case Value::STR: init = em.str_literal(v.str()); break;
        default:
            throw LuaError("local '" + c.second.substr(c.second.find('_') + 1) + "' of the script is assigned inside a GPU callback but holds a " +
                           v.type_name() + " when the lensmap build starts; only nil / boolean / number / string values can be per-pixel state");
        }
        src << " (S)." << c.second << " = " << init << ";";
    }
    src << "\n";
    if (!names[0].empty()) src << "#define BK_HAS_INVERSE 1\n#define LF_lens_inverse " << names[0] << "\n";
    if (!names[1].empty()) src << "#define BK_HAS_FORWARD 1\n#define LF_lens_forward " << names[1] << "\n";
    if (!names[2].empty()) src << "#define BK_HAS_GLOBE_PLATE 1\n#define LF_globe_plate " << names[2] << "\n";
    src << "#include \"bk_build_kernels.h\"\n";
    return src.str();
}

}
```

### blinky_amd/csrc/bk_emit.h

```cpp
#pragma once

#include <string>

#include "bk_lua.h"

namespace bk {

struct EmitRequest {
    bklua::Interp *interp = nullptr;
    bklua::Value lens_inverse;
    bklua::Value lens_forward;
    bklua::Value globe_plate;
};

std::string emit_build_source(const EmitRequest &req);

bool callbacks_carry_state(const EmitRequest &req, std::string *which);

struct EmbeddedHeader { const char *name; const char *text; };
extern const EmbeddedHeader kEmbeddedHeaders[];
extern const int kNumEmbeddedHeaders;

}
```

### blinky_amd/csrc/bk_internal.h

```cpp
#pragma once

#include <hip/hip_runtime.h>

#include <cstdarg>
#include <cstdint>
#include <cstdio>
#include <functional>
#include <string>
#include <vector>

#include "../../include/blinky_hip.h"
#ifndef BK_DEBUG_API
#define BK_DEBUG_API 0
#endif
#if BK_DEBUG_API
#include "../../include/blinky_hip_debug.h"
#endif
#include "bk_build_params.h"

namespace bk {

struct DebugOptions { int no_memcache = 0, libm_rel_log2 = 0, print_model = 0, host_module = 0, no_direct_submit = 0, forward_careful = 0; };
extern DebugOptions g_debug;

struct Range {
    explicit Range(const char *name);
    ~Range();
    Range(const Range &) = delete;
    Range &operator=(const Range &) = delete;
};

struct Span { int row, x0, x1; };

struct Rubix { int numcells = 10; double cell = 4, pad = 1; };

struct LensProgram;
struct CoopMap;
struct Resident;

}

struct bk_ctx {
    int device = 0;
    hipStream_t stream = nullptr;
    std::string err;

    int W = 0, H = 0, ps = 0;
    int gp = 0, ph = 0;
    int row0 = 0, row1 = 0;
    int nframes = 1;

    bk_plate plates[BK_MAX_PLATES] = {};
    int numplates = 0;
    bool globe_valid = false;
    int display[BK_MAX_PLATES] = {};

    int zoom_type = BK_ZOOM_NONE, zoom_fov = 0;
    double scale = -1;
    bk::Rubix rubix;

    uint8_t *d_globe = nullptr;
    uint8_t *d_plate_stage = nullptr;
    uint8_t *d_rgba_stage = nullptr;
    size_t rgba_stage_bytes = 0;
    uint32_t *d_fp_bits = nullptr;
    uint32_t *h_fp = nullptr;
    size_t fp_words = 0;
    bool footprint_valid = false;
    static constexpr int kPlateSlots = 3;
    uint8_t *h_plate[kPlateSlots] = {};
    uint8_t *d_plate_slot[kPlateSlots] = {};
    hipEvent_t plate_ev[kPlateSlots] = {};
    size_t plate_slot_bytes = 0;
    int plate_next = 0;
    uint32_t *d_offsets = nullptr;
    uint32_t *d_convert = nullptr;
    uint8_t *d_tints = nullptr;
    uint8_t *d_frame = nullptr;
    uint8_t *d_pal = nullptr;
    uint8_t *d_lut_rgba = nullptr;
    uint64_t *d_mask = nullptr;
    int *d_display = nullptr;
    unsigned int last_bad_key = 0;
    uint32_t *d_flag_list = nullptr;
    size_t flag_cap = 0;
    void *fwd_scratch[4] = {nullptr, nullptr, nullptr, nullptr};
    size_t fwd_scratch_bytes[4] = {0, 0, 0, 0};
    unsigned int grid_cache[256] = {0};
    double grid_cache_key[4] = {-1, 0, 0, 0};
    hipStream_t build_aux = nullptr;
    hipEvent_t build_ev[2] = {nullptr, nullptr};
    hipEvent_t build_time_ev[2] = {nullptr, nullptr};
    int *h_build_flags = nullptr;
    bool fwd_tiles_used = false;
    void *fwd_tables = nullptr;
    int fwd_tables_ps = -1;
#if BK_DEBUG_API
    std::vector<int32_t> dbg_corner_xy;
    std::vector<uint8_t> dbg_corner_ok;
    bool dbg_corners_set = false;
    void clear_debug_corners() { dbg_corner_xy.clear(); dbg_corner_ok.clear(); dbg_corners_set = false; }
    bool debug_corners_set() const { return dbg_corners_set; }
#else
    void clear_debug_corners() {}
    bool debug_corners_set() const { return false; }
#endif
    int last_flagged = 0, last_changed = 0;
    uint8_t *h_frame = nullptr;
    uint64_t *h_mask = nullptr;
    size_t globe_bytes = 0;
    size_t map_px = 0;

    bool lensmap_valid = false;
    std::vector<bk::Span> spans;
    bool spans_valid = false;
    bool apply_in_flight = false;
    bool fully_mapped = false;

    int apply_variant = -1;
    int num_cus = 256;
    int apply_flags = 0;
    int apply_block_cost = -1;
    int apply_lds_kb = 0;
    int apply_fchunk = 0;
    int apply_wgs_per_cu = 16;
    bool blockmap_tuning = true;
    int tile_shape = 0;
    bk::CoopMap *coopmap = nullptr;
    bk::CoopMap *coopmap_alt = nullptr;
    bk::Resident *resident = nullptr;
    int resident_mode = 0;
    int res_part = 0, res_parts = 1, res_reserve = 0;
    uint64_t apply_ticket = 0;
    uint8_t res_pal[BK_MAX_PLATES * 256] = {};
    uint8_t pal_cache[BK_MAX_PLATES * 256] = {};
    hipStream_t pal_stream = nullptr;
    bool pal_cached = false;
    uint8_t lut_rgba_cache[4 * BK_MAX_PLATES * 256] = {};
    hipStream_t lut_rgba_stream = nullptr;
    bool lut_rgba_cached = false;
    bool res_rubix = false;
    bool apply_was_resident = false;
    bk::LensProgram *prog = nullptr;
    double last_build_ms = 0;
    double last_host_eval_ms = 0;
    double last_kernel_wall_ms = 0;
    int last_kernel_retries = 0;
    bool last_fixup_compiled = false;
    uint32_t *host_sink_off = nullptr; uint8_t *host_sink_tint = nullptr;
    int last_build_path = 0;
    std::string last_build_why;
    int sequential_build = 1;
    bool async_compile = false;

    int fail(int code, const char *fmt, ...) __attribute__((format(printf, 3, 4)))
    {
        char buf[2048];
        va_list ap;
        va_start(ap, fmt);
        vsnprintf(buf, sizeof buf, fmt, ap);
        va_end(ap);
        err = buf;
        return code;
    }
    int rows() const { return row1 - row0; }
    size_t plate_bytes() const { return (size_t)gp * ph; }
    size_t globe_stride() const { return (size_t)BK_MAX_PLATES * gp * ph; }
    size_t plate_tiles() const { return (size_t)(gp >> 4) * (ph >> 3); }
    const int *fp_summary(int plate) const { return reinterpret_cast<const int *>(h_fp + fp_words) + 5 * plate; }
};

#define BK_HIP(ctx, expr)                                                               \
    do {                                                                                \
        hipError_t e_ = (expr);                                                         \
        if (e_ != hipSuccess)                                                           \
            return (ctx)->fail(BK_E_HIP, "%s failed: %s", #expr, hipGetErrorString(e_)); \
    } while (0)

namespace bk {

int launch_apply(bk_ctx *ctx, int frame0, int nframes, uint8_t *dst_first_owned_row, int dst_pitch,
                 size_t frame_stride, int rubix_on);
int launch_mask(bk_ctx *ctx);
int launch_fill_lcg(bk_ctx *ctx, uint8_t *plate_dst, uint32_t seed);
int launch_convert_offsets(bk_ctx *ctx, uint32_t *buf, size_t n, int to_device);
int launch_plate_retile(bk_ctx *ctx, uint8_t *plate_tiled, int to_tiled, uint8_t *rowmajor = nullptr);
int launch_plate_rgba_retile(bk_ctx *ctx, uint8_t *plane0, const uint8_t *src_dev, size_t src_pitch);
int launch_footprint(bk_ctx *ctx);
inline void footprint_invalidate(bk_ctx *ctx) { ctx->footprint_valid = false; }
void footprint_free(bk_ctx *ctx);
int launch_plate_rgba_retile_footprint(bk_ctx *ctx, int plate, uint8_t *plane0, const uint8_t *src_dev, size_t src_pitch);
int launch_scatter32(bk_ctx *ctx, uint32_t *dst, const uint32_t *h_idx, const uint32_t *h_val, size_t n);
int launch_scatter8(bk_ctx *ctx, uint8_t *dst, const uint32_t *h_idx, const uint8_t *h_val, size_t n);
int launch_truncate_scan(bk_ctx *ctx, unsigned int bad_key, int display_out[BK_MAX_PLATES]);
void coopmap_invalidate(bk_ctx *ctx);
int launch_apply_coop(bk_ctx *ctx, int frame0, int nframes, uint8_t *dst_first_owned_row, int dst_pitch,
                      size_t frame_stride, int rubix_on);
int launch_apply_rgba(bk_ctx *ctx, int globe0, int nframes, uint8_t *dst_first_owned_row, int dst_pitch, size_t frame_stride,
                      const uint8_t *d_lut = nullptr, bool ss2 = false);
int coopmap_stats(bk_ctx *ctx, int out[6]);
int coopmap_traffic_model(bk_ctx *ctx, uint64_t out[8]);
int coopmap_xcd_probe(bk_ctx *ctx, int *out, int nwg);
int coopmap_band_balance(bk_ctx *ctx, uint32_t out[18]);
// ... 23 lines not shown
```

### blinky_amd/csrc/bk_lens.cpp

```cpp
#include <chrono>
#include <cstring>
#include <future>

#include "bk_emit.h"
#include "bk_lens_priv.h"

using namespace bklua;

namespace bk {

static double need_num(const Values &a, size_t i, const char *fn)
{
    if (i >= a.size() || a[i].t != Value::NUM)
        throw LuaError(std::string("bad argument #") + std::to_string(i + 1) + " to '" + fn + "' (number expected)");
    return a[i].n;
}

LensProgram::LensProgram(bk_ctx *ctx) : interp(math_platform())
{
    interp.print_sink = [this](const std::string &s) { console += s; };
    static const char *alias[] = {"cos", "sin", "tan", "asin", "acos", "atan", "atan2", "sinh", "cosh", "tanh",
                                  "log", "log10", "abs", "sqrt", "exp", "pow"};
    Value math = interp.get_global("math");
    for (const char *a : alias) interp.set_global(a, math.tab()->get(Value::string(a)));
// ... 199 lines not shown
static int host_lens_forward(bk_ctx *ctx, const float ray[3], double *x, double *y)
{
    LensProgram *P = ctx->prog;
    Values r = P->interp.call(P->lens_forward, Values{Value::number((double)ray[0]), Value::number((double)ray[1]),
                                                      Value::number((double)ray[2])});
    if (r.size() == 2) {
        if (r[0].t == Value::NUM && r[1].t == Value::NUM) { *x = r[0].n; *y = r[1].n; return 1; }
        ctx->fail(BK_E_SCRIPT, "lens_forward returned a non-number value for x,y");
        return -1;
    }
    if (r.size() == 1) {
        if (r[0].t == Value::NIL) return 0;
        ctx->fail(BK_E_SCRIPT, "lens_forward returned a single non-nil value");
        return -1;
    }
    ctx->fail(BK_E_SCRIPT, "lens_forward returned %zu values instead of 2", r.size());
    return -1;
}

extern "C" int bk_calc_zoom(bk_ctx *ctx, double *scale_out)
{
    if (!ctx) return BK_E_INVALID;
    LensProgram *P = ctx->prog;
    if (!P || !P->lens_valid) return ctx->fail(BK_E_STATE, "no valid lens");
    if (ctx->W <= 0 || ctx->H <= 0) return ctx->fail(BK_E_STATE, "bk_calc_zoom: call bk_resize first");
    const bk_lens_info &L = P->info;
    double scale = -1;
    try {
        if (ctx->zoom_type == BK_ZOOM_FOV || ctx->zoom_type == BK_ZOOM_VFOV) {
            if (L.max_fov <= 0 || L.max_vfov <= 0)
                return ctx->fail(BK_E_ZOOM, "max_fov & max_vfov not specified, try \"f_cover\"");
            if (ctx->zoom_type == BK_ZOOM_FOV && ctx->zoom_fov > L.max_fov)
                return ctx->fail(BK_E_ZOOM, "fov must be less than %d", L.max_fov);
            if (ctx->zoom_type == BK_ZOOM_VFOV && ctx->zoom_fov > L.max_vfov)
                return ctx->fail(BK_E_ZOOM, "vfov must be less than %d", L.max_vfov);
            if (!L.has_forward)
                return ctx->fail(BK_E_ZOOM, "Please specify a forward mapping function in your script for FOV scaling");
            float ray[3];
            double x = 0, y = 0;
            const double fovr = ctx->zoom_fov * 3.14159265358979323846 / 180;
            if (ctx->zoom_type == BK_ZOOM_FOV) bk::h_latlon_to_ray(*P->interp.math, 0, fovr * 0.5, ray);
            else bk::h_latlon_to_ray(*P->interp.math, fovr * 0.5, 0, ray);
            const int st = host_lens_forward(ctx, ray, &x, &y);
            if (st == -1) return BK_E_SCRIPT;
            if (st == 0) return ctx->fail(BK_E_ZOOM, "ray_to_xy did not return a valid r value for determining FOV scale");
            scale = ctx->zoom_type == BK_ZOOM_FOV ? x / (ctx->W * 0.5) : y / (ctx->H * 0.5);
        } else if (ctx->zoom_type == BK_ZOOM_CONTAIN || ctx->zoom_type == BK_ZOOM_COVER) {
            const double fit_w = L.lens_width / ctx->W, fit_h = L.lens_height / ctx->H;
            const bool wp = L.lens_width > 0, hp = L.lens_height > 0;
            if (!wp && hp) scale = fit_h;
            else if (wp && !hp) scale = fit_w;
            else if (!wp && !hp)
                return ctx->fail(BK_E_ZOOM, "neither lens_height nor lens_width are valid/specified.  Try f_fov instead.");
            else {
                const double lens_aspect = L.lens_width / L.lens_height;
                const double screen_aspect = (double)ctx->W / ctx->H;
                const bool lens_wider = lens_aspect > screen_aspect;
                if (ctx->zoom_type == BK_ZOOM_CONTAIN) scale = lens_wider ? fit_w : fit_h;
                else scale = lens_wider ? fit_h : fit_w;
            }
        }
    } catch (const LuaError &e) {
        return ctx->fail(BK_E_SCRIPT, "lens_forward failed: %s", e.what());
    }
    if (scale <= 0) return ctx->fail(BK_E_ZOOM, "init returned a scale of %f, which is  <= 0", scale);
    ctx->scale = scale;
    if (scale_out) *scale_out = scale;
    return BK_OK;
}


static std::string target_arch(bk_ctx *ctx)
{
    hipDeviceProp_t prop;
    if (ctx->device >= 0 && hipGetDeviceProperties(&prop, ctx->device) == hipSuccess && prop.gcnArchName[0])
        return std::string("--offload-arch=") + prop.gcnArchName;
    return "--offload-arch=gfx950";
}

static int load_module(bk_ctx *ctx, LensProgram *P, const std::string &source, const CodeResult &cr)
{
    if (cr.rc != BK_OK) return ctx->fail(cr.rc, "%s", cr.log.c_str());
    if (P->module) { (void)hipModuleUnload(P->module); P->module = nullptr; }
    P->k_inverse = P->k_corners = P->k_quads = P->k_resolve = P->k_tiles = nullptr;
    P->module_from_cache = cr.from_disk;
    if (ctx->device < 0) {
        P->module_source = source;
        return BK_OK;
    }
    BK_HIP(ctx, hipModuleLoadData(&P->module, cr.code->data()));
    (void)hipModuleGetFunction(&P->k_inverse, P->module, "bk_build_inverse");
    (void)hipModuleGetFunction(&P->k_corners, P->module, "bk_forward_corners");
    (void)hipModuleGetFunction(&P->k_quads, P->module, "bk_forward_quads");
    (void)hipModuleGetFunction(&P->k_resolve, P->module, "bk_forward_resolve");
    if (hipModuleGetFunction(&P->k_tiles, P->module, "bk_forward_tiles") != hipSuccess) P->k_tiles = nullptr;
    (void)hipGetLastError();
    P->module_source = source;
    return BK_OK;
}

int compile_module(bk_ctx *ctx, LensProgram *P, const std::string &source)
{
    if (P->module_source == source && (P->module || ctx->device < 0)) return BK_OK;
    return load_module(ctx, P, source, compile_code(source, target_arch(ctx)));
}

static int compile_module_async(bk_ctx *ctx, LensProgram *P, const std::string &source)
{
    if (P->module_source == source && P->module) return BK_OK;
    const std::string arch = target_arch(ctx);
    if (P->pending.valid() && P->pending_source == source) {
        if (P->pending.wait_for(std::chrono::seconds(0)) != std::future_status::ready) return BK_PENDING;
        CodeResult cr = P->pending.get();
        P->pending_source.clear();
        P->pending = std::shared_future<::CodeResult>();
        return load_module(ctx, P, source, cr);
    }
    CodeResult cr = cached_code(source, arch);
    if (cr.code) return load_module(ctx, P, source, cr);
    park_compile(P->pending);
    P->pending_source = source;
    P->pending = std::async(std::launch::async, [source, arch]() { return compile_code(source, arch); }).share();
    return BK_PENDING;
}

int bk::build_module_ready(bk_ctx *ctx)
{
    LensProgram *P = ctx->prog;
    if (!(ctx->async_compile && P && P->lens_valid && ctx->globe_valid && P->info.map_type != BK_MAP_NONE)) return BK_OK;
    std::string psrc;
    bk::EmitRequest rq;
    rq.interp = &P->interp; rq.lens_inverse = P->lens_inverse; rq.lens_forward = P->lens_forward; rq.globe_plate = P->globe_plate;
    if (P->emitted.valid && P->emitted.activity == P->interp.activity && P->emitted.libm_rel == bk::g_debug.libm_rel_log2) {
        if (!P->emitted.refused.empty()) return BK_OK;
        psrc = P->emitted.src;
    } else
    try { psrc = bk::emit_build_source(rq); } catch (const LuaError &) { return BK_OK; }
    int prev = -1;
    const bool switched = ctx->device >= 0 && hipGetDevice(&prev) == hipSuccess && prev != ctx->device && hipSetDevice(ctx->device) == hipSuccess;
    const int rc = compile_module_async(ctx, P, psrc) == BK_PENDING ? BK_PENDING : BK_OK;
    if (switched) (void)hipSetDevice(prev);
    return rc;
}

extern "C" int bk_set_async_compile(bk_ctx *ctx, int on)
{
    if (!ctx) return BK_E_INVALID;
    ctx->async_compile = on != 0;
    return BK_OK;
}

int generate_source(bk_ctx *ctx, LensProgram *P, std::string *out, std::string *refused)
{
    bk::EmitRequest rq;
    rq.interp = &P->interp;
    rq.lens_inverse = P->lens_inverse;
    rq.lens_forward = P->lens_forward;
    rq.globe_plate = P->globe_plate;
    if (refused) refused->clear();
    if (P->emitted.valid && P->emitted.activity == P->interp.activity && P->emitted.libm_rel == bk::g_debug.libm_rel_log2 &&
        (refused || P->emitted.refused.empty())) {
        *out = P->emitted.src;
        if (refused) *refused = P->emitted.refused;
        return BK_OK;
    }
    P->emitted.valid = false;
    const auto remember = [&](const std::string &src, const std::string &why) {
        P->emitted.src = src; P->emitted.refused = why;
        P->emitted.activity = P->interp.activity; P->emitted.libm_rel = bk::g_debug.libm_rel_log2;
        try { std::string which; P->emitted.stateless = !bk::callbacks_carry_state(rq, &which); } catch (const LuaError &) { P->emitted.stateless = false; }
        P->emitted.valid = true;
    };
    try {
        *out = bk::emit_build_source(rq);
        if (const int n = bk::g_debug.libm_rel_log2)
            if (n >= 8 && n <= 52) *out = "#define BK_LIBM_REL 0x1p-" + std::to_string(n) + "\n" + *out;
    } catch (const LuaError &e) {
        if (refused && strstr(e.what(), "GPU callback")) {
            out->clear();
            *refused = e.what();
            remember(*out, *refused);
            return BK_OK;
        }
        return ctx->fail(BK_E_SCRIPT, "%s", e.what());
    }
    P->last_source = *out;
    remember(*out, std::string());
    return BK_OK;
}

#if BK_DEBUG_API
extern "C" int bk_debug_kernel_source(bk_ctx *ctx, char *buf, size_t cap, size_t *needed, int compile)
{
    if (!ctx) return BK_E_INVALID;
    LensProgram *P = ctx->prog;
    if (!P || !P->lens_valid) return ctx->fail(BK_E_STATE, "no valid lens");
    std::string src;
    if (int r = generate_source(ctx, P, &src)) return r;
    if (needed) *needed = src.size() + 1;
    if (buf && cap) snprintf(buf, cap, "%s", src.c_str());
    if (compile) return compile_module(ctx, P, src);
    return BK_OK;
}
#endif

#if BK_DEBUG_API
extern "C" int bk_debug_eval(bk_ctx *ctx, int which, const double *args, int nargs, double *out, int *nout)
{
    if (!ctx || !ctx->prog) return BK_E_INVALID;
    LensProgram *P = ctx->prog;
    const Value &f = which == 0 ? P->lens_inverse : which == 1 ? P->lens_forward : P->globe_plate;
    if (!f.is_function()) return ctx->fail(BK_E_STATE, "callback not defined");
    try {
        Values a;
        for (int i = 0; i < nargs; ++i) a.push_back(Value::number(args[i]));
        P->interp.steps = 0;
        Values r = P->interp.call(f, a);
        *nout = (int)r.size();
        for (size_t i = 0; i < r.size() && i < 8; ++i) out[i] = r[i].t == Value::NUM ? r[i].n : __builtin_nan("");
        if (r.size() == 1 && r[0].t == Value::NIL) *nout = -1;
    } catch (const LuaError &e) {
        return ctx->fail(BK_E_SCRIPT, "%s", e.what());
    }
    return BK_OK;
}
#endif

#if BK_DEBUG_API
extern "C" int bk_debug_module_from_cache(const bk_ctx *ctx) { return ctx && ctx->prog && ctx->prog->module_from_cache ? 1 : 0; }
#endif

extern "C" int bk_set_host_math(bk_ctx *ctx, int portable)
{
    if (!ctx) return BK_E_INVALID;
#if BK_DEBUG_API
    if (portable >= 2) {
        bk::prog_of(ctx)->interp.math = &math_perturbed(ldexp(1.0, -(portable & 63)), portable >> 6);
        return BK_OK;
    }
#else
    if (portable >= 2) return ctx->fail(BK_E_INVALID, "bk_set_host_math: %d is a test mode of debug-API builds", portable);
#endif
    bk::prog_of(ctx)->interp.math = portable ? &math_portable() : &math_platform();
    return BK_OK;
}

extern "C" const char *bk_script_console(bk_ctx *ctx) { return ctx && ctx->prog ? ctx->prog->console.c_str() : ""; }
```

### blinky_amd/csrc/bk_lens_priv.h

```cpp
#pragma once

#include <future>
#include <string>

#include "bk_internal.h"
#include "bk_lua.h"
#include "bk_modules.h"

static inline int h_trunc_to_int(double v)
{
    if (!(v > -2147483649.0 && v < 2147483648.0)) return (int)0x80000000;
    return (int)v;
}

namespace bk {

struct LensProgram {
    bklua::Interp interp;
    bool lens_valid = false;
    bk_lens_info info{};
    bklua::Value lens_inverse, lens_forward, globe_plate;
    std::string module_source;
    hipModule_t module = nullptr;
    bool module_from_cache = false;
    hipFunction_t k_inverse = nullptr, k_corners = nullptr, k_quads = nullptr, k_resolve = nullptr, k_tiles = nullptr;
    std::shared_future<::CodeResult> pending;
    std::string pending_source;
    struct { bool valid = false; unsigned long long activity = 0; int libm_rel = 0; bool stateless = false; std::string src, refused; } emitted;
    bool fwd_needs_host = false;
    std::string last_source;
    std::string console;

    explicit LensProgram(bk_ctx *ctx);
};

static inline LensProgram *prog_of(bk_ctx *ctx)
{
    if (!ctx->prog) ctx->prog = new LensProgram(ctx);
    return ctx->prog;
}

static inline void h_vector_ma(const float *a, float scale, const float *b, float *c)
{
    c[0] = a[0] + scale * b[0];
    c[1] = a[1] + scale * b[1];
    c[2] = a[2] + scale * b[2];
}
static inline void h_vector_normalize(float *v)
{
    float length = v[0] * v[0] + v[1] * v[1] + v[2] * v[2];
    length = (float)__builtin_sqrt((double)length);
    if (length) {
        float ilength = 1 / length;
        v[0] *= ilength;
        v[1] *= ilength;
        v[2] *= ilength;
    }
}
static inline void h_latlon_to_ray(const bklua::MathLib &M, double lat, double lon, float *ray)
{
    double clat = M.cos(lat);
    ray[0] = (float)(M.sin(lon) * clat);
    ray[1] = (float)M.sin(lat);
    ray[2] = (float)(M.cos(lon) * clat);
}
static inline void h_ray_to_latlon(const bklua::MathLib &M, const float *ray, double *lat, double *lon)
{
    *lon = M.atan2((double)ray[0], (double)ray[2]);
    *lat = M.atan2((double)ray[1], M.sqrt((double)(ray[0] * ray[0] + ray[2] * ray[2])));
}

static inline void h_plate_uv_to_ray(const bk_plate &p, double u, double v, float *ray)
{
    u -= 0.5;
    v -= 0.5;
    v = -v;
    ray[0] = ray[1] = ray[2] = 0;
    h_vector_ma(ray, p.dist, p.forward, ray);
    h_vector_ma(ray, (float)u, p.right, ray);
    h_vector_ma(ray, (float)v, p.up, ray);
    h_vector_normalize(ray);
}
static inline void h_cross(const float *v1, const float *v2, float *cross)
{
    cross[0] = v1[1] * v2[2] - v1[2] * v2[1];
    cross[1] = v1[2] * v2[0] - v1[0] * v2[2];
    cross[2] = v1[0] * v2[1] - v1[1] * v2[0];
}

}

#pragma GCC visibility push(hidden)
int generate_source(bk_ctx *ctx, bk::LensProgram *P, std::string *out, std::string *refused = nullptr);
int compile_module(bk_ctx *ctx, bk::LensProgram *P, const std::string &source);
#pragma GCC visibility pop
```

### blinky_amd/ffi.py

```python
import ctypes as C
import os

import numpy as np

try:
    import torch
except ImportError:
    torch = None

LIB_PATH = os.environ.get("BLINKY_HIP_LIB") or os.path.join(os.path.dirname(os.path.abspath(__file__)), "libblinkyhip.so")
if not os.path.exists(LIB_PATH):
    raise ImportError(
        f"{LIB_PATH} is missing: build it with `python -c 'import __graft_entry__ as g; g.build()'` "
        "(or `make -C blinky_amd/csrc`).  There is no CPU fallback."
    )
lib = C.CDLL(LIB_PATH)

MAX_PLATES = 6
NULL_OFFSET = 0xFFFFFFFF
DEVICE_NONE = -2
OK = 0
PENDING = 1
MAP_NONE, MAP_INVERSE, MAP_FORWARD = 0, 1, 2
ZOOM_NONE, ZOOM_FOV, ZOOM_VFOV, ZOOM_COVER, ZOOM_CONTAIN = range(5)


class Plate(C.Structure):
    _fields_ = [("forward", C.c_float * 3), ("right", C.c_float * 3), ("up", C.c_float * 3),
                ("fov", C.c_float), ("dist", C.c_float)]


class LensInfo(C.Structure):
    _fields_ = [("map_type", C.c_int), ("has_inverse", C.c_int), ("has_forward", C.c_int),
                ("max_fov", C.c_int), ("max_vfov", C.c_int),
                ("lens_width", C.c_double), ("lens_height", C.c_double), ("onload", C.c_char * 128)]


_vp, _i, _sz, _d = C.c_void_p, C.c_int, C.c_size_t, C.c_double
_SIGS = {
    "bk_create": (_vp, [_i]),
    "bk_destroy": (None, [_vp]),
    "bk_last_error": (C.c_char_p, [_vp]),
    "bk_set_stream": (_i, [_vp, _vp]),
    "bk_synchronize": (_i, [_vp]),
    "bk_load_globe": (_i, [_vp, C.c_char_p, _sz, C.c_char_p]),
    "bk_load_lens": (_i, [_vp, C.c_char_p, _sz, C.c_char_p]),
    "bk_clear_lens": (_i, [_vp]),
    "bk_clear_globe": (_i, [_vp]),
    "bk_get_lens_info": (_i, [_vp, C.POINTER(LensInfo)]),
    "bk_get_globe": (_i, [_vp, C.POINTER(Plate), C.POINTER(_i)]),
    "bk_set_globe_plates": (_i, [_vp, C.POINTER(Plate), _i]),
    "bk_resize": (_i, [_vp, _i, _i]),
    "bk_set_rows": (_i, [_vp, _i, _i]),
    "bk_set_frames": (_i, [_vp, _i]),
    "bk_set_zoom": (_i, [_vp, _i, _i]),
    "bk_set_rubixgrid": (_i, [_vp, _i, _d, _d]),
    "bk_build": (_i, [_vp, C.POINTER(_i), C.POINTER(_d)]),
    "bk_calc_zoom": (_i, [_vp, C.POINTER(_d)]),
    "bk_last_build_fixups": (_i, [_vp, C.POINTER(_i), C.POINTER(_i)]),
    "bk_last_build_bad_key": (C.c_uint, [_vp]),
    "bk_set_sequential_build": (_i, [_vp, _i]),
    "bk_last_build_path": (_i, [_vp, C.c_char_p, _sz]),
    "bk_lens_carries_state": (_i, [_vp, C.c_char_p, _sz]),
    "bk_truncate_build": (_i, [_vp, C.c_uint, C.POINTER(_i)]),
    "bk_set_cache_dir": (_i, [C.c_char_p]),
    "bk_set_async_compile": (_i, [_vp, _i]),
    "bk_set_lensmap": (_i, [_vp, _vp, _vp]),
    "bk_read_lensmap": (_i, [_vp, _vp, _vp]),
    "bk_upload_plate": (_i, [_vp, _i, _i, _vp, _i]),
    "bk_upload_plate_async": (_i, [_vp, _i, _i, _vp, _i]),
    "bk_upload_plate_rgba": (_i, [_vp, _i, _i, _vp, _i]),
    "bk_upload_plate_rgba_device": (_i, [_vp, _i, _i, _vp, _i]),
    "bk_plate_footprint": (_i, [_vp, _i, C.POINTER(_i), C.POINTER(_i), _vp]),
    "bk_upload_plate_rgba_footprint": (_i, [_vp, _i, _i, _vp, _i]),
    "bk_upload_plate_rgba_footprint_device": (_i, [_vp, _i, _i, _vp, _i]),
    "bk_apply_rgba_device": (_i, [_vp, _i, _i, _vp, _i, _sz, _i, _i]),
    "bk_apply_rgba_tinted_device": (_i, [_vp, _i, _i, _vp, _i, _sz, _i, _i, _vp]),
    "bk_apply_rgba_ss2_device": (_i, [_vp, _i, _i, _vp, _i, _sz, _i, _i, _vp]),
    "bk_globe_device_ptr": (_vp, [_vp, _i]),
    "bk_fill_plate_lcg": (_i, [_vp, _i, _i, C.c_uint32]),
    "bk_apply": (_i, [_vp, _i, _vp, _i, _i, _i, _i, _vp]),
    "bk_apply_device": (_i, [_vp, _i, _i, _vp, _i, _sz, _i, _i, _i, _vp]),
    "bk_apply_begin": (_i, [_vp, _i, _i, _vp]),
    "bk_apply_resident_begin": (_i, [_vp, _i, _vp, _d]),
    "bk_apply_resident_submit": (_i, [_vp, _i, _vp, _i, _i, _i, C.POINTER(C.c_uint64)]),
    "bk_apply_resident_submit_batch": (_i, [_vp, _i, _i, _vp, _i, _sz, _i, _i, C.POINTER(C.c_uint64)]),
    "bk_apply_resident_wait": (_i, [_vp, C.c_uint64, C.POINTER(_d)]),
    "bk_apply_resident_end": (_i, [_vp]),
    "bk_apply_resident_info": (_i, [_vp, C.POINTER(_i)]),
    "bk_apply_end": (_i, [_vp, _vp, _i, _i, _i]),
    "bk_create_palmap": (None, [_vp, _vp]),
    "bk_create_tintmap_rgba": (None, [_vp, _vp]),
    "bk_get_size": (_i, [_vp] + [C.POINTER(_i)] * 5),
    "bk_version": (C.c_char_p, []),
    "bk_set_apply_variant": (_i, [_vp, _i]),
    "bk_set_resident_share": (_i, [_vp, _i, _i, _i]),
    "bk_set_resident_apply": (_i, [_vp, _i]),
    "bk_multi_set_resident_apply": (_i, [_vp, _i]),
    "bk_set_blockmap_tuning": (_i, [_vp, _i]),
    "bk_set_host_compile": (_i, [_i]),
    "bk_host_module_ready": (_i, [_vp, _i]),
    "bk_debug_module_from_cache": (_i, [_vp]),
    "bk_debug_forward_tiles": (_i, [_vp, C.POINTER(_i), C.POINTER(_i)]),
    "bk_debug_set_option": (_i, [C.c_char_p, _i]),
    "bk_debug_build_breakdown": (_i, [_vp, C.POINTER(_d)]),
    "bk_multi_lensmap_valid": (_i, [_vp]),
    "bk_last_build_ms": (_d, [_vp]),
    "bk_globe_pitch": (_i, [_vp]),
    "bk_globe_rows": (_i, [_vp]),
    "bk_globe_texel_offset": (C.c_uint32, [_vp, _i, _i, _i]),
    "bk_download_plate": (_i, [_vp, _i, _i, _vp, _i]),
    "bk_save_plate": (_i, [_vp, _i, _i, _i, _vp, _i]),
    "bk_debug_tile_stats": (_i, [_vp, C.POINTER(_i)]),
    "bk_debug_traffic_model": (_i, [_vp, C.POINTER(C.c_uint64)]),
    "bk_debug_band_balance": (_i, [_vp, C.POINTER(C.c_uint32)]),
    "bk_debug_stream_mix": (_i, [_vp, _sz, _i, _i, C.POINTER(_d)]),
    "bk_debug_fnv1a64": (_i, [_vp, _sz, C.POINTER(C.c_uint64)]),
    "bk_debug_host_build": (_i, [_vp, _i, _vp, _vp, C.POINTER(_i), C.POINTER(_d)]),
    "bk_debug_resident_latency": (_i, [_vp, _i, _vp, _i, _i, C.POINTER(_d), C.POINTER(_d)]),
    "bk_debug_build_params": (_i, [_vp, _vp, _sz, C.POINTER(_sz)]),
    "bk_debug_host_entries": (_i, [_vp, _vp, _sz, _vp, _vp]),
    "bk_debug_host_corners": (_i, [_vp, _vp, _sz, _vp, _vp, _vp]),
    "bk_debug_set_forward_corners": (_i, [_vp, _vp, _vp, _sz]),
    "bk_debug_xcd_of_workgroups": (_i, [_vp, C.POINTER(_i), _i]),
    "bk_debug_set_ablation": (_i, [_vp, _i]),
    "bk_debug_set_tile_shape": (_i, [_vp, _i]),
    "bk_debug_kernel_source": (_i, [_vp, C.c_char_p, _sz, C.POINTER(_sz), _i]),
    "bk_debug_eval": (_i, [_vp, _i, C.POINTER(_d), _i, C.POINTER(_d), C.POINTER(_i)]),
    "bk_script_console": (C.c_char_p, [_vp]),
    "bk_set_host_math": (_i, [_vp, _i]),
    "bk_debug_eval_device": (_i, [_vp, _i, _vp, _i, _i, _vp, _vp]),
    "bk_debug_eval_device_bounds": (_i, [_vp, _i, _vp, _i, _i, _vp, _vp, _vp, _vp]),
    "bk_dev_alloc": (_vp, [_vp, _sz]),
    "bk_dev_free": (None, [_vp, _vp]),
    "bk_dev_read": (_i, [_vp, _vp, _vp, _sz]),
    "bk_comm_unique_id": (_i, [_vp]),
    "bk_comm_create": (_vp, [_vp, _i, _i, _vp]),
    "bk_comm_destroy": (None, [_vp]),
    "bk_comm_last_error": (C.c_char_p, [_vp]),
    "bk_comm_stripe": (_i, [_vp, _i, C.POINTER(_i), C.POINTER(_i)]),
    "bk_comm_restripe": (_i, [_vp]),
    "bk_comm_rebalance": (_i, [_vp]),
    "bk_debug_stripe_bounds": (_i, [C.POINTER(C.c_uint32), _i, _i, _i, C.POINTER(_i)]),
    "bk_debug_row_costs": (_i, [_vp, C.POINTER(C.c_uint32)]),
    "bk_multi_rebalance": (_i, [_vp, C.POINTER(_i)]),
# ... 100 lines not shown
        n = _i()
        self._chk(lib.bk_get_globe(self._h, plates, C.byref(n)))
        return list(plates)[: n.value]

    def set_globe_plates(self, plates):
        arr = (Plate * len(plates))(*plates)
        self._chk(lib.bk_set_globe_plates(self._h, arr, len(plates)))

    def resize(self, w, h):
        self._chk(lib.bk_resize(self._h, w, h))

    def set_rows(self, r0, r1):
        self._chk(lib.bk_set_rows(self._h, r0, r1))

    def set_frames(self, n):
        self._chk(lib.bk_set_frames(self._h, n))

    def set_zoom(self, ztype, fov=0):
        self._chk(lib.bk_set_zoom(self._h, ztype, fov))

    def set_rubixgrid(self, numcells, cell, pad):
        self._chk(lib.bk_set_rubixgrid(self._h, numcells, cell, pad))

    def size(self):
        v = [_i() for _ in range(5)]
        self._chk(lib.bk_get_size(self._h, *[C.byref(x) for x in v]))
        return tuple(x.value for x in v)

    def build(self):
        disp = (_i * MAX_PLATES)()
        scale = _d()
        self._chk(lib.bk_build(self._h, disp, C.byref(scale)))
        return list(disp), scale.value

    def set_async_compile(self, on):
        self._chk(lib.bk_set_async_compile(self._h, int(on)))

    def build_nowait(self):
        disp = (_i * MAX_PLATES)()
        scale = _d()
        rc = lib.bk_build(self._h, disp, C.byref(scale))
        if rc == PENDING:
            return None
        self._chk(rc)
        return list(disp), scale.value

    def calc_zoom(self):
        scale = _d()
        self._chk(lib.bk_calc_zoom(self._h, C.byref(scale)))
        return scale.value

    def last_build_fixups(self):
        a, b = _i(), _i()
        self._chk(lib.bk_last_build_fixups(self._h, C.byref(a), C.byref(b)))
        return a.value, b.value

    def build_breakdown(self):
        out = (_d * 6)()
        self._chk(lib.bk_debug_build_breakdown(self._h, out))
        return dict(build_ms=out[0], host_eval_ms=out[1], flagged=int(out[2]), pool_threads=int(out[3]), kernel_wall_ms=out[4],
                    retries=int(out[5]) % 1000, compiled_host_module=out[5] >= 1000)

    def host_build(self, mode=0):
        W, H, ps, r0, r1 = self.size()
        off = np.empty((r1 - r0) * W, np.uint32)
        tin = np.empty((r1 - r0) * W, np.uint8)
        disp = (_i * MAX_PLATES)()
        scale = _d()
        rc = lib.bk_debug_host_build(self._h, int(mode), _ptr(off), _ptr(tin), disp, C.byref(scale))
        err = None
        if rc != OK:
            err = lib.bk_last_error(self._h).decode(errors="replace")
            if rc != -3:
                raise BlinkyError(f"[{rc}] {err}")
        return off, tin, list(disp), scale.value, err

    def last_build_path(self):
        buf = C.create_string_buffer(1024)
        rc = lib.bk_last_build_path(self._h, buf, 1024)
        if rc < 0:
            self._chk(rc)
        return rc, buf.value.decode(errors="replace")

    def set_sequential_build(self, mode):
        self._chk(lib.bk_set_sequential_build(self._h, int(mode)))

    def lens_carries_state(self):
        buf = C.create_string_buffer(128)
        rc = lib.bk_lens_carries_state(self._h, buf, 128)
        if rc < 0:
            self._chk(rc)
        return bool(rc), buf.value.decode()

    def last_build_bad_key(self):
        return int(lib.bk_last_build_bad_key(self._h))

    def truncate_build(self, bad_key):
        out = (_i * MAX_PLATES)()
        self._chk(lib.bk_truncate_build(self._h, bad_key, out))
        return list(out)

    def last_build_ms(self):
        return lib.bk_last_build_ms(self._h)

    def set_lensmap(self, offsets, tints=None):
        offsets = np.ascontiguousarray(offsets, dtype=np.uint32)
        if tints is not None:
            tints = np.ascontiguousarray(tints, dtype=np.uint8)
        self._chk(lib.bk_set_lensmap(self._h, _ptr(offsets), _ptr(tints)))

    def read_lensmap(self):
        w, h, ps, r0, r1 = self.size()
        off = np.empty((r1 - r0) * w, np.uint32)
        tin = np.empty((r1 - r0) * w, np.uint8)
        self._chk(lib.bk_read_lensmap(self._h, _ptr(off), _ptr(tin)))
        return off, tin

    def upload_plate(self, frame, plate, src, pitch=None):
        src = np.ascontiguousarray(src, dtype=np.uint8)
        if pitch is None:
            pitch = src.shape[-1]
        self._chk(lib.bk_upload_plate(self._h, frame, plate, _ptr(src), pitch))

    def upload_plate_async(self, frame, plate, src, pitch=None):
        src = np.ascontiguousarray(src, dtype=np.uint8)
        self._chk(lib.bk_upload_plate_async(self._h, frame, plate, _ptr(src), src.shape[-1] if pitch is None else pitch))

    def upload_plate_rgba(self, globe, plate, src, pitch=None):
        src = np.ascontiguousarray(src, dtype=np.uint8)
        if pitch is None:
            pitch = src.shape[-1] * (src.shape[-2] if src.ndim == 3 else 1)
        self._chk(lib.bk_upload_plate_rgba(self._h, globe, plate, _ptr(src), pitch))

    def upload_plate_rgba_device(self, globe, plate, ptr, pitch):
        self._chk(lib.bk_upload_plate_rgba_device(self._h, globe, plate, ptr, pitch))

    def plate_footprint(self, plate, tiles=False):
        rect, n = (_i * 4)(), _i()
        mask = np.zeros((self.globe_rows() // 8, self.globe_pitch() // 16), np.uint8) if tiles else None
        self._chk(lib.bk_plate_footprint(self._h, plate, rect, C.byref(n), _ptr(mask)))
        return (tuple(rect), n.value, mask) if tiles else (tuple(rect), n.value)

    def upload_plate_rgba_footprint(self, globe, plate, src, pitch=None):
        src = np.ascontiguousarray(src, dtype=np.uint8)
        if pitch is None:
            pitch = src.shape[-1] * (src.shape[-2] if src.ndim == 3 else 1)
        self._chk(lib.bk_upload_plate_rgba_footprint(self._h, globe, plate, _ptr(src), pitch))

    def upload_plate_rgba_footprint_device(self, globe, plate, ptr, pitch):
        self._chk(lib.bk_upload_plate_rgba_footprint_device(self._h, globe, plate, ptr, pitch))

    def globe_device_ptr(self, frame=0):
        return lib.bk_globe_device_ptr(self._h, frame)

    def fill_plate_lcg(self, frame, plate, seed_frame=None):
        self._chk(lib.bk_fill_plate_lcg(self._h, frame, plate, frame if seed_frame is None else seed_frame))

    def apply(self, dst, frame=0, pitch=None, x0=0, y0=0, rubix_on=False, pal=None):
        assert dst.dtype == np.uint8 and dst.flags.c_contiguous
        if pitch is None:
            pitch = dst.shape[-1]
        if pal is not None:
            pal = np.ascontiguousarray(pal, dtype=np.uint8)
        self._chk(lib.bk_apply(self._h, frame, _ptr(dst), pitch, x0, y0, int(rubix_on), _ptr(pal)))
        return dst

# ... 431 lines not shown
```

### include/blinky_hip.h

```cpp
#ifndef BLINKY_HIP_H
#define BLINKY_HIP_H

#include <stddef.h>
#include <stdint.h>

#ifdef __cplusplus
extern "C" {
#endif

#define BK_MAX_PLATES   6
#define BK_NULL_OFFSET  0xFFFFFFFFu
#define BK_DEVICE_NONE  (-2)

enum {
    BK_PENDING = 1,
    BK_OK = 0,
    BK_E_INVALID = -1,
    BK_E_HIP = -2,
    BK_E_SCRIPT = -3,
    BK_E_ZOOM = -4,
    BK_E_NOMEM = -5,
    BK_E_STATE = -6
};

enum { BK_MAP_NONE = 0, BK_MAP_INVERSE = 1, BK_MAP_FORWARD = 2 };
enum { BK_ZOOM_NONE = 0, BK_ZOOM_FOV, BK_ZOOM_VFOV, BK_ZOOM_COVER, BK_ZOOM_CONTAIN };

typedef struct bk_ctx bk_ctx;

typedef struct {
    float forward[3], right[3], up[3];
    float fov;
    float dist;
} bk_plate;

typedef struct {
    int    map_type;
    int    has_inverse, has_forward;
    int    max_fov, max_vfov;
    double lens_width, lens_height;
    char   onload[128];
} bk_lens_info;

bk_ctx     *bk_create(int device);
void        bk_destroy(bk_ctx *ctx);
const char *bk_last_error(const bk_ctx *ctx);
int         bk_set_stream(bk_ctx *ctx, void *hip_stream);
int         bk_synchronize(bk_ctx *ctx);

int bk_load_globe(bk_ctx *ctx, const char *src, size_t len, const char *chunkname);
int bk_load_lens(bk_ctx *ctx, const char *src, size_t len, const char *chunkname);
int bk_clear_lens(bk_ctx *ctx);
int bk_clear_globe(bk_ctx *ctx);
int bk_get_lens_info(const bk_ctx *ctx, bk_lens_info *out);
int bk_get_globe(const bk_ctx *ctx, bk_plate plates[BK_MAX_PLATES], int *numplates);
int bk_set_globe_plates(bk_ctx *ctx, const bk_plate *plates, int numplates);

int bk_resize(bk_ctx *ctx, int width, int height);
int bk_set_rows(bk_ctx *ctx, int row0, int row1);
int bk_set_frames(bk_ctx *ctx, int nframes);
int bk_set_zoom(bk_ctx *ctx, int zoom_type, int fov_degrees);
int bk_set_rubixgrid(bk_ctx *ctx, int numcells, double cell_size, double pad_size);

int bk_build(bk_ctx *ctx, int display_out[BK_MAX_PLATES], double *scale_out);
int bk_last_build_path(const bk_ctx *ctx, char *why , size_t cap);
int bk_set_sequential_build(bk_ctx *ctx, int mode);
int bk_lens_carries_state(bk_ctx *ctx, char *global_name , size_t cap);
unsigned int bk_last_build_bad_key(const bk_ctx *ctx);
int bk_truncate_build(bk_ctx *ctx, unsigned int bad_key, int display_out[BK_MAX_PLATES]);
int bk_calc_zoom(bk_ctx *ctx, double *scale_out);
int bk_set_cache_dir(const char *dir);
int bk_set_async_compile(bk_ctx *ctx, int on);
int bk_last_build_fixups(const bk_ctx *ctx, int *flagged, int *changed);
int bk_set_lensmap(bk_ctx *ctx, const uint32_t *offsets, const uint8_t *tints);
int bk_read_lensmap(bk_ctx *ctx, uint32_t *offsets, uint8_t *tints);

int   bk_upload_plate(bk_ctx *ctx, int frame, int plate, const uint8_t *src, int src_pitch);
int   bk_upload_plate_async(bk_ctx *ctx, int frame, int plate, const uint8_t *src, int src_pitch);
int   bk_download_plate(bk_ctx *ctx, int frame, int plate, uint8_t *dst_host, int dst_pitch);
int   bk_save_plate(bk_ctx *ctx, int frame, int plate, int with_margins, uint8_t *dst_host, int dst_pitch);
void    *bk_globe_device_ptr(bk_ctx *ctx, int frame);
int      bk_globe_pitch(const bk_ctx *ctx);
int      bk_globe_rows(const bk_ctx *ctx);
uint32_t bk_globe_texel_offset(const bk_ctx *ctx, int plate, int px, int py);
int   bk_fill_plate_lcg(bk_ctx *ctx, int frame, int plate, uint32_t seed_frame);
int   bk_upload_plate_rgba(bk_ctx *ctx, int globe, int plate, const uint8_t *src_host, int src_pitch_bytes);
int   bk_upload_plate_rgba_device(bk_ctx *ctx, int globe, int plate, const void *src_dev, int src_pitch_bytes);
int   bk_plate_footprint(bk_ctx *ctx, int plate, int rect[4], int *ntiles, uint8_t *tiles);
int   bk_upload_plate_rgba_footprint_device(bk_ctx *ctx, int globe, int plate, const void *src_dev, int src_pitch_bytes);
int   bk_upload_plate_rgba_footprint(bk_ctx *ctx, int globe, int plate, const uint8_t *src_host, int src_pitch_bytes);

int bk_apply(bk_ctx *ctx, int frame, uint8_t *dst, int dst_pitch, int x0, int y0,
             int rubix_on, const uint8_t pal[BK_MAX_PLATES][256]);
int bk_apply_begin(bk_ctx *ctx, int frame, int rubix_on, const uint8_t pal[BK_MAX_PLATES][256]);
int bk_apply_end(bk_ctx *ctx, uint8_t *dst, int dst_pitch, int x0, int y0);
int bk_apply_device(bk_ctx *ctx, int frame0, int nframes, void *dst_dev, int dst_pitch,
                    size_t frame_stride, int x0, int y0, int rubix_on,
                    const uint8_t pal[BK_MAX_PLATES][256]);
int bk_apply_rgba_device(bk_ctx *ctx, int globe0, int nframes, void *dst_dev, int dst_pitch,
                         size_t frame_stride, int x0, int y0);
int bk_apply_rgba_tinted_device(bk_ctx *ctx, int globe0, int nframes, void *dst_dev, int dst_pitch,
                                size_t frame_stride, int x0, int y0, const uint8_t lut[4][BK_MAX_PLATES][256]);
int bk_apply_rgba_ss2_device(bk_ctx *ctx, int globe0, int nframes, void *dst_dev, int dst_pitch,
                             size_t frame_stride, int x0, int y0,
                             const uint8_t lut[4][BK_MAX_PLATES][256] );

int bk_apply_resident_begin(bk_ctx *ctx, int rubix_on, const uint8_t pal[BK_MAX_PLATES][256], double idle_ms);
int bk_apply_resident_submit(bk_ctx *ctx, int frame, void *dst_dev, int dst_pitch, int x0, int y0, uint64_t *ticket);
int bk_apply_resident_submit_batch(bk_ctx *ctx, int frame0, int nframes, void *dst_dev, int dst_pitch, size_t frame_stride,
                                   int x0, int y0, uint64_t *last_ticket);
int bk_apply_resident_wait(bk_ctx *ctx, uint64_t ticket, double *gpu_us);
int bk_apply_resident_end(bk_ctx *ctx);
int bk_apply_resident_info(bk_ctx *ctx, int out[12]);
int bk_set_resident_share(bk_ctx *ctx, int part, int parts, int reserve_slots_per_cu);
int bk_set_resident_apply(bk_ctx *ctx, int on);

#define BK_COMM_ID_BYTES 128
#define BK_COMM_SLOTS 4
typedef struct bk_comm bk_comm;
int         bk_comm_unique_id(uint8_t id[BK_COMM_ID_BYTES]);
bk_comm    *bk_comm_create(bk_ctx *ctx, int nranks, int rank, const uint8_t id[BK_COMM_ID_BYTES]);
void        bk_comm_destroy(bk_comm *c);
const char *bk_comm_last_error(const bk_comm *c);
int         bk_comm_stripe(const bk_comm *c, int rank, int *row0, int *row1);
int         bk_comm_restripe(bk_comm *c);
int         bk_comm_rebalance(bk_comm *c);
int         bk_comm_or_display(bk_comm *c, int display[BK_MAX_PLATES]);
int         bk_comm_gather(bk_comm *c, const void *stripe_dev, int nframes, int root, void *frames_dev, size_t frame_stride, int slot);
int         bk_comm_exchange_rotating(bk_comm *c, const void *stripe_dev, int nframes, void *frames_dev, size_t frame_stride, int slot);
int         bk_comm_wait(bk_comm *c, int slot);
int         bk_comm_synchronize(bk_comm *c);

typedef struct bk_multi bk_multi;
bk_multi   *bk_create_multi(int ndev, const int *devices);
void        bk_destroy_multi(bk_multi *m);
const char *bk_multi_last_error(const bk_multi *m);
int         bk_multi_size(const bk_multi *m);
bk_ctx     *bk_multi_ctx(bk_multi *m, int i);
bk_comm    *bk_multi_comm(bk_multi *m, int i);
int         bk_multi_uses_rccl(const bk_multi *m);
int         bk_multi_lensmap_valid(const bk_multi *m);
int bk_multi_load_globe(bk_multi *m, const char *src, size_t len, const char *chunkname);
int bk_multi_load_lens(bk_multi *m, const char *src, size_t len, const char *chunkname);
int bk_multi_clear_lens(bk_multi *m);
int bk_multi_clear_globe(bk_multi *m);
int bk_multi_resize(bk_multi *m, int width, int height);
int bk_multi_rebalance(bk_multi *m, int *bounds_out );
int bk_multi_set_frames(bk_multi *m, int nframes);
// ... 37 lines not shown
```

Measured before the change: 2.629 million Mpixels/s.

## Hoist x-only lens_inverse subexpressions into per-column pass with row-strip build kernel

The Lua-to-HIP emitter now tracks whether each value depends only on the screen x coordinate. Those values are hoisted into a per-column function that runs once per thread, and a strip kernel then evaluates several rows reusing them, with latlon_to_ray split into per-angle sincos halves. This removes repeated transcendental work in the lensmap build. The metric, however, measures only lensmap apply, which this change does not touch, so throughput should stay about the same. It adds a second emitted program and extra compile complexity.

```diff
diff --git a/blinky_amd/csrc/bk_api.cpp b/blinky_amd/csrc/bk_api.cpp
--- a/blinky_amd/csrc/bk_api.cpp
+++ b/blinky_amd/csrc/bk_api.cpp
@@ -344,6 +344,8 @@
     else if (!strcmp(name, "print_model")) bk::g_debug.print_model = value;
     else if (!strcmp(name, "host_module")) bk::g_debug.host_module = value;
     else if (!strcmp(name, "no_direct_submit")) bk::g_debug.no_direct_submit = value;
+    else if (!strcmp(name, "no_axis_split")) bk::g_debug.no_axis_split = value;
+    else if (!strcmp(name, "axis_strip_rows")) bk::g_debug.axis_strip_rows = value;
     else if (!strcmp(name, "forward_careful")) bk::g_debug.forward_careful = value;
     else return BK_E_INVALID;
     return BK_OK;
diff --git a/blinky_amd/csrc/bk_build.cpp b/blinky_amd/csrc/bk_build.cpp
--- a/blinky_amd/csrc/bk_build.cpp
+++ b/blinky_amd/csrc/bk_build.cpp
@@ -625,6 +625,15 @@
     return carries ? 1 : 0;
 }
 
+static constexpr int kStripRows = 8;
+
+extern "C" int bk_last_build_axis_split(const bk_ctx *ctx, int *rows)
+{
+    if (!ctx) return BK_E_INVALID;
+    if (rows) *rows = ctx->last_strip_rows ? ctx->last_strip_rows : 1;
+    return ctx->last_strip_rows ? 1 : 0;
+}
+
 struct HipFree { void operator()(void *p) const { (void)hipFree(p); } };
 using DeviceMem = std::unique_ptr<void, HipFree>;
 
@@ -639,7 +648,19 @@
     BK_HIP(ctx, hipEventRecord(ctx->build_time_ev[0], ctx->stream));
     const auto tk0 = std::chrono::steady_clock::now();
     std::vector<uint32_t> flagged;
+    int strip = 1;
+    if (P->k_inverse_strip) {
+        const long long waves_per_row = 4LL * ((ctx->W + 255) / 256), want = 16LL * ctx->num_cus;
+        for (int r : {kStripRows, kStripRows / 2})
+            if (strip == 1 && waves_per_row * ((ctx->rows() + r - 1) / r) >= want) strip = r;
+        const int forced = bk::g_debug.axis_strip_rows;
+        if (forced >= 1 && forced <= 64) strip = forced;
+    }
+    ctx->last_strip_rows = strip > 1 ? strip : 0;
+    void *strip_args[] = {&bp, &strip};
     if (int r = flagged_pass(ctx, "bk_build_inverse launch", bp, false, [&] {
+            if (strip > 1)
+                return hipModuleLaunchKernel(P->k_inverse_strip, (unsigned)((ctx->W + 255) / 256), (unsigned)((ctx->rows() + strip - 1) / strip), 1, 256, 1, 1, 0, ctx->stream, strip_args, nullptr);
             return hipModuleLaunchKernel(P->k_inverse, (unsigned)((ctx->W + 255) / 256), (unsigned)ctx->rows(), 1, 256, 1, 1, 0, ctx->stream, args, nullptr);
         }, counters, &flagged, &ctx->last_kernel_retries)) return r;
     ctx->last_kernel_wall_ms = std::chrono::duration<double, std::milli>(std::chrono::steady_clock::now() - tk0).count();
diff --git a/blinky_amd/csrc/bk_build_kernels.h b/blinky_amd/csrc/bk_build_kernels.h
--- a/blinky_amd/csrc/bk_build_kernels.h
+++ b/blinky_amd/csrc/bk_build_kernels.h
@@ -87,16 +87,11 @@
 #endif
 
 #ifdef BK_HAS_INVERSE
-BK_DEV void bk_inverse_entry(const BkBuildParams &P, BkState &S, int lx, int ly, unsigned int *off_out, unsigned char *tint_out, int *plate_out)
+BK_DEV void bk_inverse_result(const BkBuildParams &P, BkState &S, int n, const bkv *r, unsigned int *off_out, unsigned char *tint_out, int *plate_out)
 {
     unsigned int off = 0xFFFFFFFFu;
     unsigned char tint = 255;
     int shown = -1;
-    const double y = (double)(-(ly - P.H / 2)) * P.scale;
-    const double x = (double)(lx - P.W / 2) * P.scale;
-    bkv a[2] = {bk_num(x), bk_num(y)};
-    bkv r[BK_MAXRET];
-    const int n = LF_lens_inverse(S, a, 2, r);
     if (n == 3 && bk_isnum(r[0]) && bk_isnum(r[1]) && bk_isnum(r[2])) {
         float ray[3] = {bk_narrow(S, r[0].n, r[0].e), bk_narrow(S, r[1].n, r[1].e), bk_narrow(S, r[2].n, r[2].e)};
         bk_vector_normalize(ray);
@@ -125,6 +120,15 @@
     *tint_out = tint;
     *plate_out = shown;
 }
+BK_DEV double bk_screen_x(const BkBuildParams &P, int lx) { return (double)(lx - P.W / 2) * P.scale; }
+BK_DEV double bk_screen_y(const BkBuildParams &P, int ly) { return (double)(-(ly - P.H / 2)) * P.scale; }
+BK_DEV void bk_inverse_entry(const BkBuildParams &P, BkState &S, int lx, int ly, unsigned int *off_out, unsigned char *tint_out, int *plate_out)
+{
+    bkv a[2] = {bk_num(bk_screen_x(P, lx)), bk_num(bk_screen_y(P, ly))};
+    bkv r[BK_MAXRET];
+    const int n = LF_lens_inverse(S, a, 2, r);
+    bk_inverse_result(P, S, n, r, off_out, tint_out, plate_out);
+}
 
 #ifndef BK_HOST_MODULE
 extern "C" __global__ __launch_bounds__(256) void bk_build_inverse(BkBuildParams P)
@@ -156,6 +160,48 @@
     __syncthreads();
     bk_publish_flags(s_disp, P.display, err, P.err);
 }
+
+#ifdef BK_HAS_INVERSE_SPLIT
+extern "C" __global__ __launch_bounds__(256) void bk_build_inverse_strip(BkBuildParams P, int strip)
+{
+    __shared__ int s_disp[6];
+    if (threadIdx.x < 6) s_disp[threadIdx.x] = 0;
+    __syncthreads();
+    const int lx = blockIdx.x * blockDim.x + threadIdx.x;
+    const bool live = lx < P.W;
+    int err = 0;
+    BkState S0;
+    BkCol C;
+    bk_state_init(S0, &P);
+    if (live) LF_lens_inverse_col(S0, bk_num(bk_screen_x(P, lx)), C);
+    for (int k = 0; k < strip; ++k) {
+        const int lyl = (int)blockIdx.y * strip + k;
+        if (lyl >= P.rows) break;
+        const int ly = P.row0 + lyl;
+        bool flagged = false;
+        unsigned int off = 0xFFFFFFFFu;
+        unsigned char tint = 255;
+        const size_t o = (size_t)lyl * P.W + lx;
+        if (live) {
+            int plate;
+            BkState S = S0;
+            bkv a[2] = {bk_num(bk_screen_x(P, lx)), bk_num(bk_screen_y(P, ly))};
+            bkv r[BK_MAXRET];
+            const int n = LF_lens_inverse_px(S, a, 2, r, C);
+            bk_inverse_result(P, S, n, r, &off, &tint, &plate);
+            if (plate >= 0 && !S.flag) s_disp[plate] = 1;
+            err |= S.err;
+            P.offsets[o] = off;
+            P.tints[o] = tint;
+            flagged = S.flag != 0;
+            if ((S.err & BK_ERR_RESULT) && P.first_bad) atomicMax(P.first_bad, (unsigned int)(ly * P.W + (P.W - 1 - lx)) + 1u);
+        }
+        bk_push_flagged_wave(P, flagged, (unsigned int)o, off, tint, 0u);
+    }
+    __syncthreads();
+    bk_publish_flags(s_disp, P.display, err, P.err);
+}
+#endif
 #endif
 #endif
 
diff --git a/blinky_amd/csrc/bk_device_rt.h b/blinky_amd/csrc/bk_device_rt.h
--- a/blinky_amd/csrc/bk_device_rt.h
+++ b/blinky_amd/csrc/bk_device_rt.h
@@ -307,16 +307,26 @@
         v[2] *= ilength;
     }
 }
+typedef struct { double s, c, es, ec; } BkHalf;
+BK_DEV void bk_angle_half(BkState &S, double a, double ea, BkHalf *h)
+{
+    bkm_sincos(a, &h->s, &h->c);
+    h->es = bk_elibm(S, h->s, ea);
+    h->ec = bk_elibm(S, h->c, ea);
+}
+BK_DEV void bk_ray_from_halves(BkState &S, const BkHalf &lat, const BkHalf &lon, float *ray)
+{
+    const double p0 = lon.s * lat.c, p2 = lon.c * lat.c;
+    ray[0] = bk_narrow(S, p0, bk_eop(S, p0, bk_abs(lon.s) * lat.ec + bk_abs(lat.c) * lon.es + lat.ec * lon.es));
+    ray[1] = bk_narrow(S, lat.s, lat.es);
+    ray[2] = bk_narrow(S, p2, bk_eop(S, p2, bk_abs(lon.c) * lat.ec + bk_abs(lat.c) * lon.ec + lat.ec * lon.ec));
+}
 BK_DEV void bk_latlon_to_ray(BkState &S, double lat, double elat, double lon, double elon, float *ray)
 {
-    double slat, clat, slon, clon;
-    bkm_sincos(lat, &slat, &clat);
-    bkm_sincos(lon, &slon, &clon);
-    const double ec = bk_elibm(S, clat, elat), es = bk_elibm(S, slon, elon), ek = bk_elibm(S, clon, elon);
-    const double p0 = slon * clat, p2 = clon * clat;
-    ray[0] = bk_narrow(S, p0, bk_eop(S, p0, bk_abs(slon) * ec + bk_abs(clat) * es + ec * es));
-    ray[1] = bk_narrow(S, slat, bk_elibm(S, slat, elat));
-    ray[2] = bk_narrow(S, p2, bk_eop(S, p2, bk_abs(clon) * ec + bk_abs(clat) * ek + ec * ek));
+    BkHalf hlat, hlon;
+    bk_angle_half(S, lat, elat, &hlat);
+    bk_angle_half(S, lon, elon, &hlon);
+    bk_ray_from_halves(S, hlat, hlon, ray);
 }
 BK_DEV void bk_plate_fuv_to_ray(const BkBuildParams &P, int plate, float fu, float fv, float *ray)
 {
@@ -344,6 +354,14 @@
 {
     float ray[3];
     bk_latlon_to_ray(S, bk_tonum(S, lat), lat.e, bk_tonum(S, lon), lon.e, ray);
+    r[0] = bk_num((double)ray[0]); r[1] = bk_num((double)ray[1]); r[2] = bk_num((double)ray[2]);
+    return 3;
+}
+BK_DEV void bk_host_angle_half(BkState &S, bkv a, BkHalf *h) { bk_angle_half(S, bk_tonum(S, a), a.e, h); }
+BK_DEV int bk_host_ray_from_halves(BkState &S, const BkHalf &lat, const BkHalf &lon, bkv *r)
+{
+    float ray[3];
+    bk_ray_from_halves(S, lat, lon, ray);
     r[0] = bk_num((double)ray[0]); r[1] = bk_num((double)ray[1]); r[2] = bk_num((double)ray[2]);
     return 3;
 }
diff --git a/blinky_amd/csrc/bk_emit.cpp b/blinky_amd/csrc/bk_emit.cpp
--- a/blinky_amd/csrc/bk_emit.cpp
+++ b/blinky_amd/csrc/bk_emit.cpp
@@ -2,6 +2,7 @@
 
 #include <cmath>
 #include <cstdio>
+#include <cstring>
 #include <map>
 #include <set>
 #include <sstream>
@@ -47,6 +48,7 @@
     std::map<const Table *, std::pair<std::string, int>> const_tables;
     std::ostringstream table_code;
     int uid = 0;
+    std::string gp;
     struct SinCos { std::string s, c; long epoch; };
     std::map<std::string, SinCos> sincos;
     long epoch = 0;
@@ -143,12 +145,53 @@
     }
     std::string tmp(const char *p = "t") { return std::string(p) + std::to_string(++uid); }
     static void line(Fn &f, const std::string &s) { f.out << std::string((size_t)f.indent * 4, ' ') << s << "\n"; }
-    std::string pure_value(Fn &f, const std::string &call)
+
+    enum { AX_CONST = 0, AX_X = 1, AX_Y = 2, AX_MIXED = 3 };
+    struct Split {
+        bool on = false;
+        Fn *fn = nullptr;
+        int depth = 0;
+        bool open = true;
+        bool worth = false;
+        std::string declined;
+        std::map<std::string, int> axis;
+        std::ostringstream col;
+        std::vector<std::pair<std::string, std::string>> fields;
+        int if_axis = AX_CONST;
+    } sp;
+    struct Nest { Split &s; explicit Nest(Split &x) : s(x) { ++s.depth; } ~Nest() { --s.depth; } };
+    bool hoist_ok(const Fn &f) const { return sp.on && &f == sp.fn && sp.depth == 0 && sp.open && !ad_active; }
+    int axis_of(const std::string &v) const
+    {
+        auto it = sp.axis.find(v);
+        if (it != sp.axis.end()) return it->second;
+        for (const char *lit : {"bk_num(", "bk_nil()", "bk_bool(", "bk_str("})
+            if (v.compare(0, strlen(lit), lit) == 0 && v.find("(double)") == std::string::npos && v.find('?') == std::string::npos) return AX_CONST;
+        return AX_MIXED;
+    }
+    void define(Fn &f, const std::string &text, const std::vector<std::string> &defs, int ax, const char *type = "bkv")
+    {
+        if (!hoist_ok(f) || ax > AX_X) { line(f, text); return; }
+        sp.col << "    " << text << "\n";
+        for (const std::string &d : defs) sp.axis[d] = ax;
+        if (ax == AX_CONST) { line(f, text); return; }
+        for (const std::string &d : defs) sp.fields.emplace_back(type, d);
+        for (const char *w : {"bk_f_sin", "bk_f_cos", "bk_f_tan", "bk_f_asin(", "bk_f_acos(", "bk_f_atan", "bk_f_exp(", "bk_f_log", "bk_pow(", "bk_host_angle_half("})
+            if (text.find(w) != std::string::npos) sp.worth = true;
+    }
+    int axes(std::initializer_list<std::string> operands) const
+    {
+        int ax = AX_CONST;
+        for (const std::string &o : operands) ax |= axis_of(o);
+        return ax;
+    }
+
+    std::string pure_value(Fn &f, const std::string &call, std::initializer_list<std::string> operands)
     {
         auto hit = pure.find(call);
         if (hit != pure.end() && hit->second.epoch == epoch) return hit->second.name;
         const std::string t = tmp();
-        line(f, "bkv " + t + " = " + call + ";");
+        define(f, "bkv " + t + " = " + call + ";", {t}, axes(operands));
         pure.insert_or_assign(call, Pure{t, epoch});
         return t;
     }
@@ -286,7 +329,7 @@
         if (it != const_tables.end()) return it->second;
         if (!t->nhash.empty() || !t->shash.empty())
             unsupported(f.chunk, at.line, "table '" + hint + "' with non-array keys");
-        std::string name = "GT" + std::to_string(++uid) + "_" + sanitize(hint);
+        std::string name = gp + "GT" + std::to_string(++uid) + "_" + sanitize(hint);
         int n = (int)t->arr.size();
         table_code << "static __device__ const bkv " << name << "[" << n + 1 << "] = {{0.0, 0.0, BK_TNIL}";
         for (const Value &v : t->arr) {
@@ -424,9 +467,9 @@
                 unsupported(f.chunk, e.line, "the length operator on this expression");
             }
             std::string a = emit_expr(f, *e.a), t = tmp();
-            if (e.str == "not") line(f, "bkv " + t + " = bk_not(" + a + ");");
+            if (e.str == "not") define(f, "bkv " + t + " = bk_not(" + a + ");", {t}, axis_of(a));
             else {
-                line(f, "bkv " + t + " = bk_unm(S, " + a + ");");
+                define(f, "bkv " + t + " = bk_unm(S, " + a + ");", {t}, axis_of(a));
                 if (ad_active && d_of(a) != "0.0") ad_note(f, t, "-" + d_of(a));
             }
             return t;
@@ -439,6 +482,7 @@
                 line(f, std::string("if (") + (op == "and" ? "" : "!") + "bk_truthy(" + t + ")) {");
                 f.indent++;
                 ++epoch;
+                Nest nest(sp);
                 std::string b = emit_expr(f, *e.b);
                 line(f, t + " = " + b + ";");
                 f.indent--;
@@ -463,7 +507,7 @@
             else if (op == ">") call = "bk_lt(S, " + b + ", " + a + ")";
             else if (op == ">=") call = "bk_le(S, " + b + ", " + a + ")";
             else unsupported(f.chunk, e.line, "operator '" + op + "'");
-            if (!ad_active) return pure_value(f, call);
+            if (!ad_active) return pure_value(f, call, {a, b});
             line(f, "bkv " + t + " = " + call + ";");
             if (ad_active && (d_of(a) != "0.0" || d_of(b) != "0.0")) {
                 const std::string da = d_of(a), db = d_of(b);
@@ -632,7 +676,7 @@
             auto hit = sincos.find(operand);
             if (hit == sincos.end() || hit->second.epoch != epoch) {
                 SinCos sc{tmp("sn"), tmp("cs"), epoch};
-                line(f, "bkv " + sc.s + ", " + sc.c + "; bk_f_sincos(S, " + operand + ", &" + sc.s + ", &" + sc.c + ");");
+                define(f, "bkv " + sc.s + ", " + sc.c + "; bk_f_sincos(S, " + operand + ", &" + sc.s + ", &" + sc.c + ");", {sc.s, sc.c}, axis_of(operand));
                 hit = sincos.insert_or_assign(operand, sc).first;
             }
             single(bn == "math.sin" ? hit->second.s : hit->second.c);
@@ -642,7 +686,7 @@
         }
         auto u = unary.find(bn);
         if (u != unary.end()) {
-            if (!ad_active) { single(pure_value(f, u->second + "(S, " + A(0) + ")")); return; }
+            if (!ad_active) { single(pure_value(f, u->second + "(S, " + A(0) + ")", {A(0)})); return; }
             single(u->second + "(S, " + A(0) + ")");
             if (ad_active && d_of(A(0)) != "0.0") {
                 const std::string x = A(0) + ".n", r = *arr + "[0].n", d = d_of(A(0));
@@ -659,7 +703,7 @@
             return;
         }
         if (bn == "math.atan2") {
-            if (!ad_active) { single(pure_value(f, "bk_f_atan2(S, " + A(0) + ", " + A(1) + ")")); return; }
+            if (!ad_active) { single(pure_value(f, "bk_f_atan2(S, " + A(0) + ", " + A(1) + ")", {A(0), A(1)})); return; }
             single("bk_f_atan2(S, " + A(0) + ", " + A(1) + ")");
             if (ad_active && (d_of(A(0)) != "0.0" || d_of(A(1)) != "0.0")) {
                 const std::string y = A(0) + ".n", x = A(1) + ".n";
@@ -713,6 +757,16 @@
         }
         if (bn == "type") { single("bk_typeof(" + A(0) + ")"); return; }
         if (bn == "latlon_to_ray") {
+            const int ax[2] = {axis_of(A(0)), axis_of(A(1))};
+            if (hoist_ok(f) && (ax[0] == AX_X) != (ax[1] == AX_X) && ax[0] != AX_CONST && ax[1] != AX_CONST) {
+                std::string h[2];
+                for (int k = 0; k < 2; ++k) {
+                    h[k] = tmp("h");
+                    define(f, "BkHalf " + h[k] + "; bk_host_angle_half(S, " + A((size_t)k) + ", &" + h[k] + ");", {h[k]}, ax[k], "BkHalf");
+                }
+                line(f, "bkv " + *arr + "[3]; const int " + *cnt + " = bk_host_ray_from_halves(S, " + h[0] + ", " + h[1] + ", " + *arr + ");");
+                return;
+            }
             line(f, "bkv " + *arr + "[3]; const int " + *cnt + " = bk_host_latlon_to_ray(S, " + A(0) + ", " + A(1) + ", " + *arr + ");");
             return;
         }
@@ -801,6 +855,7 @@
     void emit_block(Fn &f, const Block &b)
     {
         ++epoch;
+        Nest nest(sp);
         for (const StmtP &s : b) emit_stmt(f, *s);
         ++epoch;
     }
@@ -811,7 +866,7 @@
         std::vector<std::string> v;
         for (size_t i = 0; i < want; ++i) {
             std::string t = tmp();
-            line(f, "const bkv " + t + " = " + arg_at(a, i) + ";");
+            define(f, "const bkv " + t + " = " + arg_at(a, i) + ";", {t}, axis_of(arg_at(a, i)));
             if (ad_active && d_of(arg_at(a, i)) != "0.0") ad_note(f, t, d_of(arg_at(a, i)));
             v.push_back(t);
         }
@@ -836,6 +891,7 @@
                 if (o->is_table(slot)) unsupported(f.chunk, target.line, "re-assigning table '" + target.str + "'");
                 if (o->fn_slots.count(slot)) unsupported(f.chunk, target.line, "re-assigning function '" + target.str + "'");
                 line(f, o->lp + std::to_string(slot) + " = " + val + ";");
+                if (sp.on && o == sp.fn) sp.axis[o->lp + std::to_string(slot)] = AX_MIXED;
                 forget(o->lp + std::to_string(slot));
                 if (ad_active && o == ad_fn && ad_slot.count(slot)) line(f, ad_slot[slot] + " = " + d_of(val) + ";");
             } else if (target.var == VarKind::Global) {
@@ -900,6 +956,8 @@
         const FuncProto *p = s.exprs[0]->proto;
         const int slot = s.slots[0];
         if (f.fn_slots.count(slot) || f.is_table(slot)) unsupported(f.chunk, s.line, "re-declaring '" + s.names[0] + "'");
+        if (sp.on && sp.declined.empty()) sp.declined = "a function defined inside lens_inverse";
+        Nest nest(sp);
         const std::string id = std::to_string(++uid);
         Fn g;
         g.proto = p;
@@ -999,7 +1057,12 @@
             }
             auto v = emit_values(f, s.exprs, s.slots.size());
             for (size_t i = 0; i < s.slots.size(); ++i) {
-                line(f, f.lp + std::to_string(s.slots[i]) + " = " + v[i] + ";");
+                const std::string var = f.lp + std::to_string(s.slots[i]);
+                if (hoist_ok(f) && slot_is_constant(f.proto, s.slots[i]) && !sp.axis.count(var)) define(f, var + " = " + v[i] + ";", {var}, axis_of(v[i]), "local");
+                else {
+                    line(f, var + " = " + v[i] + ";");
+                    if (sp.on && &f == sp.fn) sp.axis[var] = AX_MIXED;
+                }
                 forget(f.lp + std::to_string(s.slots[i]));
                 if (ad_active && &f == ad_fn && ad_slot.count(s.slots[i])) line(f, ad_slot[s.slots[i]] + " = " + d_of(v[i]) + ";");
             }
@@ -1029,6 +1092,7 @@
             line(f, "}");
             return;
         case Stmt::While: {
+            Nest nest(sp);
             line(f, "for (;;) {");
             f.indent++;
             line(f, "if (!bk_tick(S)) break;");
@@ -1040,6 +1104,7 @@
             return;
         }
         case Stmt::Repeat: {
+            Nest nest(sp);
             line(f, "for (;;) {");
             f.indent++;
             line(f, "if (!bk_tick(S)) break;");
@@ -1052,6 +1117,8 @@
         }
         case Stmt::If: {
             int opened = 0;
+            sp.if_axis = AX_CONST;
+            int cond_axis = AX_CONST;
             for (size_t i = 0; i < s.clauses.size(); ++i) {
                 const auto &c = s.clauses[i];
                 if (!c.first) {
@@ -1059,6 +1126,7 @@
                     break;
                 }
                 std::string cv = emit_expr(f, *c.first);
+                cond_axis |= axis_of(cv);
                 line(f, "if (bk_truthy(" + cv + ")) {");
                 f.indent++;
                 emit_block(f, c.second);
@@ -1067,9 +1135,11 @@
                     line(f, "} else {");
                     f.indent++;
                     opened++;
+                    ++sp.depth;
                 } else line(f, "}");
             }
-            for (int k = 0; k < opened; ++k) { f.indent--; line(f, "}"); }
+            for (int k = 0; k < opened; ++k) { f.indent--; line(f, "}"); --sp.depth; }
+            sp.if_axis = cond_axis;
             return;
         }
         case Stmt::NumFor: {
@@ -1079,6 +1149,7 @@
             line(f, "bk_need_exact(S, " + start + "); bk_need_exact(S, " + stop + "); bk_need_exact(S, " + step + ");");
             line(f, "const double " + st + " = bk_tonum(S, " + step + "), " + lim + " = bk_tonum(S, " + stop + ");");
             line(f, "double " + idx + " = bk_tonum(S, " + start + ") - " + st + ";");
+            Nest nest(sp);
             line(f, "for (;;) {");
             f.indent++;
             line(f, idx + " = " + idx + " + " + st + ";");
@@ -1138,6 +1209,7 @@
                 n = ct.second;
             }
             std::string gi = tmp("gi"), gv = tmp("gv");
+            Nest nest(sp);
             line(f, "for (int " + gi + " = 1; " + gi + " <= " + std::to_string(n) + "; ++" + gi + ") {");
             f.indent++;
             line(f, "if (!bk_tick(S)) break;");
@@ -1197,7 +1269,7 @@
         if (fi.emitting) unsupported(from_chunk, line_no, "recursion ('" + cl->proto->name + "')");
         fi.proto = cl->proto;
         fi.cl = cl;
-        fi.cname = "LF" + std::to_string(++uid) + "_" + sanitize(cl->proto->name);
+        fi.cname = gp + "LF" + std::to_string(++uid) + "_" + sanitize(cl->proto->name);
         fi.emitting = true;
 
         Fn f;
@@ -1222,6 +1294,79 @@
         fi.emitting = false;
         fi.done = true;
         return fi;
+    }
+
+    static bool can_return(const Stmt &s)
+    {
+        if (s.kind == Stmt::Return) return true;
+        for (const StmtP &b : s.body) if (can_return(*b)) return true;
+        for (auto &c : s.clauses) for (const StmtP &b : c.second) if (can_return(*b)) return true;
+        return false;
+    }
+
+    bool emit_split_pair(const Closure *cl, std::string *col_name, std::string *px_name)
+    {
+        if (!mutable_globals.empty() || !mutable_cells.empty()) { sp.declined = "the callbacks assign script globals (carried state, a keyed cache)"; return false; }
+        if (cl->proto->is_vararg || cl->proto->nparams < 2) { sp.declined = "lens_inverse does not name its two parameters"; return false; }
+        Fn f;
+        f.proto = cl->proto;
+        f.cl = cl;
+        f.chunk = cl->chunk->name;
+        sp.on = true;
+        sp.fn = &f;
+        sp.axis[f.lp + "0"] = AX_X;
+        sp.axis[f.lp + "1"] = AX_Y;
+        ++epoch;
+        for (const StmtP &stp : cl->proto->body) {
+            const Stmt &s = *stp;
+            emit_stmt(f, s);
+            if (s.kind != Stmt::Return && can_return(s)) {
+                if (s.kind == Stmt::If && !(sp.if_axis & AX_Y)) sp.declined = "a return that depends on x alone";
+                sp.open = false;
+            }
+            if (!sp.declined.empty()) break;
+        }
+        ++epoch;
+        sp.on = false;
+        sp.fn = nullptr;
+        if (!sp.declined.empty()) return false;
+        const std::string px = f.out.str();
+        std::vector<std::pair<std::string, std::string>> live;
+        const auto used = [&px](const std::string &name) {
+            const auto word = [](char c) { return c == '_' || isalnum((unsigned char)c); };
+            for (size_t at = px.find(name); at != std::string::npos; at = px.find(name, at + 1))
+                if ((at == 0 || !word(px[at - 1])) && (at + name.size() >= px.size() || !word(px[at + name.size()]))) return true;
+            return false;
+        };
+        for (auto &fl : sp.fields) if (used(fl.second)) live.push_back(fl);
+        if (!sp.worth || live.empty()) { sp.declined = "nothing worth evaluating once per column (no libm call depends on x alone)"; return false; }
+        const std::string base = gp + "LF" + std::to_string(++uid) + "_" + sanitize(cl->proto->name);
+        *col_name = base + "_col";
+        *px_name = base + "_px";
+        std::ostringstream o;
+        o << "/* " << f.chunk << ":" << cl->proto->line << "  function " << cl->proto->name << ": what depends on x alone, once per column strip */\n";
+        o << "struct BkCol {\n";
+        for (auto &fl : live) o << "    " << (fl.first == "local" ? "bkv" : fl.first) << " " << fl.second << ";\n";
+        o << "};\n";
+        o << "BK_DEV void " << *col_name << "(BkState &S, bkv x, BkCol &C)\n{\n";
+        o << "    const bkv a[1] = {x};\n    const int na = 1;\n";
+        declare_locals(o, f, "    ");
+        o << "    (void)a; (void)na;\n";
+        o << sp.col.str();
+        for (auto &fl : live) o << "    C." << fl.second << " = " << fl.second << ";\n";
+        o << "}\n\n";
+        o << "/* ... and the rest, once per pixel, from a copy of the state the column part left */\n";
+        o << "BK_DEV int " << *px_name << "(BkState &S, const bkv *a, int na, bkv *r, const BkCol &C)\n{\n";
+        declare_locals(o, f, "    ");
+        o << "    (void)a; (void)na; (void)r;\n";
+        for (auto &fl : live) {
+            if (fl.first == "local") o << "    " << fl.second << " = C." << fl.second << ";\n";
+            else o << "    const " << fl.first << " " << fl.second << " = C." << fl.second << ";\n";
+        }
+        o << px;
+        o << "    return 0;\n}\n\n";
+        fn_code.push_back(o.str());
+        return true;
     }
 };
 
@@ -1571,6 +1716,26 @@
     }
     src << "\n";
     if (!names[0].empty()) src << "#define BK_HAS_INVERSE 1\n#define LF_lens_inverse " << names[0] << "\n";
+    if (!names[0].empty() && req.axis_split) {
+        Emitter em2(*req.interp);
+        em2.gp = "C";
+        em2.strings = em.strings;
+        std::set<const FuncProto *> seen2;
+        for (const Value *v : roots)
+            if (v->t == Value::FUNC && !seen2.count(v->fn()->proto)) {
+                seen2.insert(v->fn()->proto);
+                em2.scan_closure(v->fn(), seen2);
+            }
+        std::string col, px;
+        bool pair = false;
+        try { pair = em2.emit_split_pair(roots[0]->fn(), &col, &px); } catch (const LuaError &) { pair = false; }
+        if (pair && em2.strings.size() == em.strings.size()) {
+            src << em2.table_code.str() << "\n";
+            for (const std::string &c : em2.fn_code) src << c;
+            src << "#define BK_HAS_INVERSE_SPLIT 1\n#define LF_lens_inverse_col " << col << "\n#define LF_lens_inverse_px " << px << "\n";
+        }
+        if (req.split_declined) *req.split_declined = pair ? std::string() : em2.sp.declined.empty() ? std::string("not translated") : em2.sp.declined;
+    }
     if (!names[1].empty()) src << "#define BK_HAS_FORWARD 1\n#define LF_lens_forward " << names[1] << "\n";
     if (!names[2].empty()) src << "#define BK_HAS_GLOBE_PLATE 1\n#define LF_globe_plate " << names[2] << "\n";
     src << "#include \"bk_build_kernels.h\"\n";
diff --git a/blinky_amd/csrc/bk_emit.h b/blinky_amd/csrc/bk_emit.h
--- a/blinky_amd/csrc/bk_emit.h
+++ b/blinky_amd/csrc/bk_emit.h
@@ -11,6 +11,8 @@
     bklua::Value lens_inverse;
     bklua::Value lens_forward;
     bklua::Value globe_plate;
+    bool axis_split = true;
+    std::string *split_declined = nullptr;
 };
 
 std::string emit_build_source(const EmitRequest &req);
diff --git a/blinky_amd/csrc/bk_internal.h b/blinky_amd/csrc/bk_internal.h
--- a/blinky_amd/csrc/bk_internal.h
+++ b/blinky_amd/csrc/bk_internal.h
@@ -20,7 +20,7 @@
 
 namespace bk {
 
-struct DebugOptions { int no_memcache = 0, libm_rel_log2 = 0, print_model = 0, host_module = 0, no_direct_submit = 0, forward_careful = 0; };
+struct DebugOptions { int no_memcache = 0, libm_rel_log2 = 0, print_model = 0, host_module = 0, no_direct_submit = 0, forward_careful = 0, no_axis_split = 0, axis_strip_rows = 0; };
 extern DebugOptions g_debug;
 
 struct Range {
@@ -119,6 +119,7 @@
 
     int apply_variant = -1;
     int num_cus = 256;
+    int last_strip_rows = 0;
     int apply_flags = 0;
     int apply_block_cost = -1;
     int apply_lds_kb = 0;
diff --git a/blinky_amd/csrc/bk_lens.cpp b/blinky_amd/csrc/bk_lens.cpp
--- a/blinky_amd/csrc/bk_lens.cpp
+++ b/blinky_amd/csrc/bk_lens.cpp
@@ -305,7 +305,7 @@
 {
     if (cr.rc != BK_OK) return ctx->fail(cr.rc, "%s", cr.log.c_str());
     if (P->module) { (void)hipModuleUnload(P->module); P->module = nullptr; }
-    P->k_inverse = P->k_corners = P->k_quads = P->k_resolve = P->k_tiles = nullptr;
+    P->k_inverse = P->k_inverse_strip = P->k_corners = P->k_quads = P->k_resolve = P->k_tiles = nullptr;
     P->module_from_cache = cr.from_disk;
     if (ctx->device < 0) {
         P->module_source = source;
@@ -313,6 +313,7 @@
     }
     BK_HIP(ctx, hipModuleLoadData(&P->module, cr.code->data()));
     (void)hipModuleGetFunction(&P->k_inverse, P->module, "bk_build_inverse");
+    if (hipModuleGetFunction(&P->k_inverse_strip, P->module, "bk_build_inverse_strip") != hipSuccess) P->k_inverse_strip = nullptr;
     (void)hipModuleGetFunction(&P->k_corners, P->module, "bk_forward_corners");
     (void)hipModuleGetFunction(&P->k_quads, P->module, "bk_forward_quads");
     (void)hipModuleGetFunction(&P->k_resolve, P->module, "bk_forward_resolve");
@@ -354,7 +355,8 @@
     std::string psrc;
     bk::EmitRequest rq;
     rq.interp = &P->interp; rq.lens_inverse = P->lens_inverse; rq.lens_forward = P->lens_forward; rq.globe_plate = P->globe_plate;
-    if (P->emitted.valid && P->emitted.activity == P->interp.activity && P->emitted.libm_rel == bk::g_debug.libm_rel_log2) {
+    rq.axis_split = !bk::g_debug.no_axis_split;
+    if (P->emitted.valid && P->emitted.activity == P->interp.activity && P->emitted.libm_rel == bk::g_debug.libm_rel_log2 && P->emitted.no_axis_split == bk::g_debug.no_axis_split) {
         if (!P->emitted.refused.empty()) return BK_OK;
         psrc = P->emitted.src;
     } else
@@ -380,8 +382,9 @@
     rq.lens_inverse = P->lens_inverse;
     rq.lens_forward = P->lens_forward;
     rq.globe_plate = P->globe_plate;
+    rq.axis_split = !bk::g_debug.no_axis_split;
     if (refused) refused->clear();
-    if (P->emitted.valid && P->emitted.activity == P->interp.activity && P->emitted.libm_rel == bk::g_debug.libm_rel_log2 &&
+    if (P->emitted.valid && P->emitted.activity == P->interp.activity && P->emitted.libm_rel == bk::g_debug.libm_rel_log2 && P->emitted.no_axis_split == bk::g_debug.no_axis_split &&
         (refused || P->emitted.refused.empty())) {
         *out = P->emitted.src;
         if (refused) *refused = P->emitted.refused;
@@ -390,7 +393,7 @@
     P->emitted.valid = false;
     const auto remember = [&](const std::string &src, const std::string &why) {
         P->emitted.src = src; P->emitted.refused = why;
-        P->emitted.activity = P->interp.activity; P->emitted.libm_rel = bk::g_debug.libm_rel_log2;
+        P->emitted.activity = P->interp.activity; P->emitted.libm_rel = bk::g_debug.libm_rel_log2; P->emitted.no_axis_split = bk::g_debug.no_axis_split;
         try { std::string which; P->emitted.stateless = !bk::callbacks_carry_state(rq, &which); } catch (const LuaError &) { P->emitted.stateless = false; }
         P->emitted.valid = true;
     };
diff --git a/blinky_amd/csrc/bk_lens_priv.h b/blinky_amd/csrc/bk_lens_priv.h
--- a/blinky_amd/csrc/bk_lens_priv.h
+++ b/blinky_amd/csrc/bk_lens_priv.h
@@ -23,10 +23,10 @@
     std::string module_source;
     hipModule_t module = nullptr;
     bool module_from_cache = false;
-    hipFunction_t k_inverse = nullptr, k_corners = nullptr, k_quads = nullptr, k_resolve = nullptr, k_tiles = nullptr;
+    hipFunction_t k_inverse = nullptr, k_inverse_strip = nullptr, k_corners = nullptr, k_quads = nullptr, k_resolve = nullptr, k_tiles = nullptr;
     std::shared_future<::CodeResult> pending;
     std::string pending_source;
-    struct { bool valid = false; unsigned long long activity = 0; int libm_rel = 0; bool stateless = false; std::string src, refused; } emitted;
+    struct { bool valid = false; unsigned long long activity = 0; int libm_rel = 0; int no_axis_split = 0; bool stateless = false; std::string src, refused; } emitted;
     bool fwd_needs_host = false;
     std::string last_source;
     std::string console;
diff --git a/blinky_amd/ffi.py b/blinky_amd/ffi.py
--- a/blinky_amd/ffi.py
+++ b/blinky_amd/ffi.py
@@ -61,6 +61,7 @@
     "bk_last_build_bad_key": (C.c_uint, [_vp]),
     "bk_set_sequential_build": (_i, [_vp, _i]),
     "bk_last_build_path": (_i, [_vp, C.c_char_p, _sz]),
+    "bk_last_build_axis_split": (_i, [_vp, C.POINTER(_i)]),
     "bk_lens_carries_state": (_i, [_vp, C.c_char_p, _sz]),
     "bk_truncate_build": (_i, [_vp, C.c_uint, C.POINTER(_i)]),
     "bk_set_cache_dir": (_i, [C.c_char_p]),
@@ -327,6 +328,13 @@
             self._chk(rc)
         return rc, buf.value.decode(errors="replace")
 
+    def last_build_axis_split(self):
+        rows = _i()
+        rc = lib.bk_last_build_axis_split(self._h, C.byref(rows))
+        if rc < 0:
+            self._chk(rc)
+        return bool(rc), rows.value
+
     def set_sequential_build(self, mode):
         self._chk(lib.bk_set_sequential_build(self._h, int(mode)))
 
diff --git a/include/blinky_hip.h b/include/blinky_hip.h
--- a/include/blinky_hip.h
+++ b/include/blinky_hip.h
@@ -64,6 +64,7 @@
 
 int bk_build(bk_ctx *ctx, int display_out[BK_MAX_PLATES], double *scale_out);
 int bk_last_build_path(const bk_ctx *ctx, char *why , size_t cap);
+int bk_last_build_axis_split(const bk_ctx *ctx, int *rows );
 int bk_set_sequential_build(bk_ctx *ctx, int mode);
 int bk_lens_carries_state(bk_ctx *ctx, char *global_name , size_t cap);
 unsigned int bk_last_build_bad_key(const bk_ctx *ctx);
```

Result: no change. 2.631 million Mpixels/s, median of 3 (+0.1%).
